# AnthonyMadia/lodestar

Hardware: AMD Instinct MI355X
Metric: verified signature sets/sec (node) at 8192-set batches (higher is better)
Workload: dtype u32 (28-bit-limb Montgomery Fp, v_mad_u64_u32)

## Files before the change

### lodestar_amd/csrc/bgv_api.cpp

```cpp
#include <hip/hip_runtime.h>
#include <stdio.h>
#include <stdlib.h>
#include <string.h>
#include <sys/mman.h>
#include <sys/random.h>

#include <algorithm>
#include <atomic>
#include <chrono>
#include <condition_variable>
#include <unordered_map>
#include <deque>
#include <map>
#include <memory>
#include <mutex>
#include <shared_mutex>
#include <unordered_set>
#include <thread>
#include <vector>

#include "../../include/blsgpu.h"
#include "bgv_launch.h"
#include "bgv_retry_plan.h"
#include "bls_field.h"

#define BGV_MAX_BATCH_SLOTS 131072
#define BGV_DISPATCHERS 2

static size_t max_batch_slots() {
  static const size_t v = env_size("BGV_MAX_BATCH_SLOTS", BGV_MAX_BATCH_SLOTS, BGV_WAVE);
  return v;
}
#define BGV_COALESCE_US 500
static size_t coalesce_us() {
  static const size_t v = env_size("BGV_COALESCE_US", BGV_COALESCE_US, 0);
  return v;
}
#define BGV_IDLE_COALESCE_US 50
static size_t idle_coalesce_us() {
  static const size_t v = env_size("BGV_IDLE_COALESCE_US", BGV_IDLE_COALESCE_US, 0);
  return v;
}
#define BGV_SPLIT_MIN_SETS 4096
static size_t split_min_env() {
  static const size_t v = env_size("BGV_SPLIT_MIN", BGV_SPLIT_MIN_SETS, 0);
  return v == 1 ? 2 : v;
}
static int dispatchers_per_device() {
  static const int v = (int)env_size("BGV_DISPATCHERS", BGV_DISPATCHERS, 1);
  return v;
}
static int execs_per_device() {
  static const int v = (int)env_size("BGV_EXECS", 2 * BGV_DISPATCHERS, 1);
  return std::max(v, dispatchers_per_device());
}

static size_t retry_hold_max() {
  static const size_t v = env_size("BGV_RETRY_HOLD", 1, 1);
  return v;
}
static int retry_threads_per_device() {
  static const int v = (int)env_size("BGV_RETRY_THREADS", 1, 1);
  return v;
}

extern "C" int bgv_device_count(void) {
  int n = 0;
  if (hipGetDeviceCount(&n) != hipSuccess) return 0;
  return n;
}

namespace {

template <class T>
struct Pinned {
  T* p = nullptr;
  size_t cap = 0;
  hipError_t reserve(size_t n) {
    if (n <= cap) return hipSuccess;
    release();
    n = std::max(n, 2 * cap);
    hipError_t e = hipHostMalloc(reinterpret_cast<void**>(&p), std::max<size_t>(n, 1) * sizeof(T), 0);
    if (e != hipSuccess) {
      p = nullptr;
      return e;
    }
    cap = n;
    return hipSuccess;
  }
  void release() {
    if (p) (void)hipHostFree(p);
    p = nullptr;
    cap = 0;
  }
};

struct Exec {
  hipStream_t main = nullptr;
  hipStream_t close = nullptr;
  hipEvent_t ev0 = nullptr, ev1 = nullptr, ev_prep = nullptr, ev_sets = nullptr;
  hipEvent_t kev[2 * BGV_NKERNELS] = {};
  void* slot_mem = nullptr;
  uint32_t slot_cap = 0;
  void* group_mem = nullptr;
  uint32_t group_cap = 0;
  bgv_dslot* d_slots = nullptr;
  bgv_dgroup* d_groups = nullptr;
  uint32_t* d_idx = nullptr;
  size_t idx_cap = 0;
  uint8_t* d_pkb = nullptr;
  size_t pkb_cap = 0;
  Pinned<bgv_dslot> h_slots;
  Pinned<bgv_dgroup> h_groups;
  Pinned<uint32_t> h_idx;
  Pinned<uint8_t> h_pkb;
  Pinned<int32_t> h_ss, h_ps, h_verdict;
  fp12_t* d_gu1 = nullptr;
  size_t gu1_cap = 0;
  void* d_pscratch = nullptr;
  size_t pscratch_cap = 0;
  uint8_t* d_pout = nullptr;
  size_t pout_cap = 0;
  uint32_t* d_lines = nullptr;
  uint32_t lines_cap = 0;
};

struct FinalScratch {
  uint8_t* din = nullptr;
  void* vals = nullptr;
  void* one = nullptr;
  bgv_dgroup* dg = nullptr;
  int32_t* dst = nullptr;
  int32_t* dv = nullptr;
  size_t cap = 0;
};

static const uint32_t kComHandles = 2 * BGV_MAX_COMMITTEES;
static const size_t kComPoolInit = size_t(1) << 20;
struct ComPool {
  std::mutex mu;
  std::vector<uint32_t> free_handles;
  std::map<uint32_t, uint32_t> free_ranges;
  size_t cap = 0;
  bool alloc(uint32_t n, uint32_t* handle, uint32_t* off) {
    if (free_handles.empty()) return false;
    for (auto it = free_ranges.begin(); it != free_ranges.end(); ++it)
      if (it->second >= n) {
        *off = it->first;
        const uint32_t rest = it->second - n;
        free_ranges.erase(it);
        if (rest) free_ranges.emplace(*off + n, rest);
        *handle = free_handles.back();
        free_handles.pop_back();
        return true;
      }
    return false;
  }
  void add_range(uint32_t off, uint32_t n) {
    auto nx = free_ranges.lower_bound(off);
    if (nx != free_ranges.begin()) {
      auto pv = std::prev(nx);
      if (pv->first + pv->second == off) {
        off = pv->first;
        n += pv->second;
        free_ranges.erase(pv);
      }
    }
    if (nx != free_ranges.end() && off + n == nx->first) {
      n += nx->second;
      free_ranges.erase(nx);
    }
    free_ranges.emplace(off, n);
  }
};
struct CommitteeRec {
  uint32_t handle = 0, off = 0;
  std::vector<uint32_t> idx;
  bool bad = false;
  std::shared_ptr<ComPool> pool;
  ~CommitteeRec() {
    if (!pool) return;
    std::lock_guard<std::mutex> lk(pool->mu);
    pool->free_handles.push_back(handle);
    pool->add_range(off, (uint32_t)idx.size());
  }
};

struct Call;
struct BatchState {
  std::chrono::steady_clock::time_point tb;
  double t_merge = 0, t_tok = 0, t_sets = 0, t_pass1 = 0, t_post = 0;
  uint32_t nslots = 0, ngroups = 0;
  std::vector<uint32_t> call_gb;
  bool want_gu = false;
  bool uniform = false;
  bool prof = false;
};
struct RetryJob {
  std::vector<Call*> calls;
  Exec* x = nullptr;
  std::shared_ptr<BatchState> st;
};
struct DevSched {
  std::mutex mu;
  std::condition_variable cv;
  std::deque<Exec*> free;
  std::deque<RetryJob> rq;
  bool stop = false;
  std::vector<std::thread> retry_threads;
  std::vector<hipStream_t> retries;
  std::vector<hipStream_t> dstreams;
};

struct Device {
  int id = 0;
  std::unique_ptr<DevSched> sched = std::make_unique<DevSched>();
  FinalScratch final_scratch;
  hipStream_t stream = nullptr;
  bgv_cache_entry* cache = nullptr;
  size_t cache_cap = 0;
  bgv_dcommittee* com_dir = nullptr;
  uint32_t* com_pool = nullptr;
  uint32_t* com_list = nullptr;
  std::vector<Exec*> execs;
  std::unique_ptr<std::mutex> compute_mu = std::make_unique<std::mutex>();
};

struct Call : CallPlan {
  const bgv_set* sets = nullptr;
  const bgv_pkbits* pkbits = nullptr;
  std::vector<SetCommittee> setcom;
  std::vector<std::shared_ptr<CommitteeRec>> com_refs;
  int32_t* out = nullptr;
  bgv_stats* stats_out = nullptr;
  bgv_done_fn done = nullptr;
  void* user = nullptr;
  bool owned = false;
  std::chrono::steady_clock::time_point t0;
  int dev = -1;
  bgv_job pjob{};
  int32_t pcode = 0;
  int rc = BGV_OK;
  std::mutex mu;
  std::condition_variable cv;
  bool finished = false;
};

}

struct bgv_ctx {
  std::vector<Device> devs;
  std::atomic<size_t> n_pubkeys{0};
  std::mutex put_mu;
  std::unordered_set<uint32_t> bad_pk;
  std::atomic<bool> closed{false};
  std::mutex rng_mu;
  uint64_t rng_seed = 0, rng_state = 0;
  std::shared_mutex cache_mu;
  std::mutex util_mu;
  std::shared_mutex com_mu;
  std::unordered_map<uint32_t, std::shared_ptr<CommitteeRec>> committees;
  std::vector<std::weak_ptr<CommitteeRec>> retired;
  std::shared_ptr<ComPool> com_pool = std::make_shared<ComPool>();
  std::mutex prof_mu;
  bool profile = false;
  bool fault_inject = false;
  std::atomic<uint32_t> max_slots{BGV_MAX_BATCH_SLOTS};
  std::atomic<uint32_t> coalesce{BGV_COALESCE_US};
  std::atomic<uint32_t> idle_coalesce{BGV_IDLE_COALESCE_US};
  std::atomic<int> running{0};
  std::atomic<uint32_t> split_min{BGV_SPLIT_MIN_SETS};
  int split_inflight = 0;
  bool split_closing = false;
  std::mutex split_mu;
  std::condition_variable split_cv;
  double kernel_ms[BGV_NKERNELS] = {};
  uint64_t kernel_launches = 0;
  std::vector<std::thread> dispatchers;
  std::mutex qmu;
  std::condition_variable qcv;
  std::deque<Call*> queue;
  bool stop = false;
};

#define HIPCHK(x)                               \
  do {                                          \
    hipError_t e_ = (x);                        \
    if (e_ != hipSuccess) return -BGV_E_DEVICE; \
  } while (0)

static uint64_t splitmix64(uint64_t* s) {
  uint64_t z = (*s += 0x9E3779B97F4A7C15ull);
  z = (z ^ (z >> 30)) * 0xBF58476D1CE4E5B9ull;
  z = (z ^ (z >> 27)) * 0x94D049BB133111EBull;
  return z ^ (z >> 31);
}

static void fill_scalars(bgv_ctx* c, uint64_t* out, size_t n) {
  {
    std::lock_guard<std::mutex> lk(c->rng_mu);
    if (c->rng_seed) {
      for (size_t i = 0; i < n; ++i) {
        uint64_t v;
        do v = splitmix64(&c->rng_state);
        while (v == 0);
        out[i] = v;
      }
      return;
    }
  }
  par_ranges(n, [out](size_t lo, size_t hi) {
    size_t got = 0;
    uint8_t* p = reinterpret_cast<uint8_t*>(out + lo);
    while (got < (hi - lo) * 8) {
      const ssize_t r = getrandom(p + got, (hi - lo) * 8 - got, 0);
      if (r > 0) got += (size_t)r;
    }
    for (size_t i = lo; i < hi; ++i)
      if (out[i] == 0) out[i] = 1;
  });
}

template <class T>
static int grow(T** p, size_t* cap, size_t want) {
  if (want <= *cap) return BGV_OK;
  size_t n = std::max(want, *cap * 2);
  if (*p) (void)hipFree(*p);
  *p = nullptr;
  HIPCHK(hipMalloc(reinterpret_cast<void**>(p), n * sizeof(T)));
  *cap = n;
  return BGV_OK;
}

static int exec_reserve_slots(Exec& x, uint32_t slots) {
  if (slots <= x.slot_cap) return BGV_OK;
  uint32_t n = std::max<uint32_t>(slots, x.slot_cap * 2);
  if (x.slot_mem) (void)hipFree(x.slot_mem);
  if (x.d_slots) (void)hipFree(x.d_slots);
  x.slot_mem = nullptr;
  x.d_slots = nullptr;
  HIPCHK(hipMalloc(&x.slot_mem, bgv_slot_mem_bytes(n)));
  HIPCHK(hipMalloc(reinterpret_cast<void**>(&x.d_slots), sizeof(bgv_dslot) * n));
  x.slot_cap = n;
  return BGV_OK;
}

static int exec_reserve_groups(Exec& x, uint32_t groups) {
  if (groups <= x.group_cap) return BGV_OK;
  uint32_t n = std::max<uint32_t>(groups, x.group_cap * 2);
  if (x.group_mem) (void)hipFree(x.group_mem);
  if (x.d_groups) (void)hipFree(x.d_groups);
  x.group_mem = nullptr;
  x.d_groups = nullptr;
  HIPCHK(hipMalloc(&x.group_mem, bgv_group_bytes() * n));
  HIPCHK(hipMalloc(reinterpret_cast<void**>(&x.d_groups), sizeof(bgv_dgroup) * n));
  x.group_cap = n;
  return BGV_OK;
}

static uint32_t lines_keep_pairs(size_t slots) {
  return (uint32_t)((slots + slots / BGV_WAVE + 16383u) & ~(size_t)16383u);
}
static void exec_trim_lines(Exec& x, size_t max_slots) {
  if (x.lines_cap <= lines_keep_pairs(max_slots)) return;
  (void)hipFree(x.d_lines);
  x.d_lines = nullptr;
  x.lines_cap = 0;
}
static int exec_reserve_lines(Exec& x, bgv_dev_batch& b) {
  const uint32_t need = bgv_lines_pairs(b);
  if (need > x.lines_cap) {
    const uint32_t cap = (need + 16383u) & ~16383u;
    if (x.d_lines) (void)hipFree(x.d_lines);
    x.d_lines = nullptr;
    x.lines_cap = 0;
    HIPCHK(hipMalloc(reinterpret_cast<void**>(&x.d_lines), bgv_line_record_bytes() * cap));
    x.lines_cap = cap;
  }
  b.lines = x.d_lines;
  b.lines_cap = x.lines_cap;
  return BGV_OK;
}

static int exec_create(Exec* x) {
  HIPCHK(hipEventCreate(&x->ev0));
  HIPCHK(hipEventCreate(&x->ev1));
  HIPCHK(hipEventCreateWithFlags(&x->ev_sets, hipEventDisableTiming));
  HIPCHK(hipEventCreateWithFlags(&x->ev_prep, hipEventDisableTiming));
  for (auto& e : x->kev) HIPCHK(hipEventCreate(&e));
  return BGV_OK;
}

static void exec_destroy(Exec* x) {
  if (x->main) (void)hipStreamSynchronize(x->main);
  void* ptrs[] = {x->slot_mem, x->group_mem, x->d_slots,    x->d_groups, x->d_idx,
                  x->d_pkb,      x->d_pscratch, x->d_pout, x->d_lines};
  for (void* p : ptrs)
    if (p) (void)hipFree(p);
  x->h_slots.release();
  x->h_groups.release();
  x->h_idx.release();
  x->h_pkb.release();
  x->h_ss.release();
  x->h_ps.release();
  x->h_verdict.release();
  if (x->d_gu1) (void)hipFree(x->d_gu1);
  if (x->ev0) (void)hipEventDestroy(x->ev0);
  if (x->ev1) (void)hipEventDestroy(x->ev1);
  if (x->ev_sets) (void)hipEventDestroy(x->ev_sets);
  if (x->ev_prep) (void)hipEventDestroy(x->ev_prep);
  for (auto& e : x->kev)
    if (e) (void)hipEventDestroy(e);
  if (x->close) (void)hipStreamSynchronize(x->close);
  delete x;
}

static void prof_add(bgv_ctx* c, Exec& x, bool sets, bool groups) {
  std::lock_guard<std::mutex> lk(c->prof_mu);
  if (!c->profile) return;
  for (int k = 0; k < BGV_NKERNELS; ++k) {
    const bool is_set_kernel = k < BGV_NSETKERNELS;
    if ((is_set_kernel && !sets) || (!is_set_kernel && !groups)) continue;
    float km = 0;
    if (hipEventElapsedTime(&km, x.kev[2 * k], x.kev[2 * k + 1]) == hipSuccess) c->kernel_ms[k] += km;
  }
  if (sets) c->kernel_launches++;
}

static bgv_dev_batch make_batch(Device& d, Exec& x, uint32_t nslots, uint32_t ngroups) {
  bgv_dev_batch b;
  memset(&b, 0, sizeof(b));
  b.nslots = nslots;
  b.ngroups = ngroups;
  b.slots = x.d_slots;
  b.groups = x.d_groups;
  b.pk_idx = x.d_idx;
  b.cache_opaque = d.cache;
  b.pk_bytes = x.d_pkb;
  b.com_dir = d.com_dir;
  b.com_pool = d.com_pool;
  bgv_carve(&b, x.slot_mem, x.slot_cap, x.group_mem, x.group_cap);
  return b;
}

static void call_finish(Call* call) {
  for (size_t j = 0; j < call->njobs; ++j) call->out[j] = call->code[j] == 2 ? -BGV_E_DEVICE : call->code[j];
  call->st.wall_ms =
      std::chrono::duration<double, std::milli>(std::chrono::steady_clock::now() - call->t0).count();
  if (call->stats_out) *call->stats_out = call->st;
  if (call->done) call->done(call->user, call->rc);
  if (call->owned) {
    delete call;
    return;
  }
  {
    std::lock_guard<std::mutex> lk(call->mu);
    call->finished = true;
  }
  call->cv.notify_all();
}

static void call_fail(Call* call, int rc) {
  call->rc = rc;
  for (auto& x : call->code)
    if (x == 2) x = -BGV_E_DEVICE;
  call_finish(call);
}

static int host_job_code(bgv_ctx* c, const bgv_job& jb, const bgv_set* sets, int32_t* code,
                         const bgv_pkbits* pkbits = nullptr, Call* call = nullptr) {
  *code = 2;
  if (jb.n_sets == 0) {
    *code = -BGV_E_EMPTY_SET;
    return BGV_OK;
  }
  for (uint32_t k = 0; k < jb.n_sets && *code == 2; ++k) {
    const bgv_set& s = sets[jb.first_set + k];
    if (pkbits && pkbits[jb.first_set + k].committee != BGV_NO_COMMITTEE) {
      const bgv_pkbits& pb = pkbits[jb.first_set + k];
      if (!s.msg || (!s.sig && s.sig_len) || (!pb.bits && pb.n_bits)) return -BGV_E_ARG;
      const auto it = c->committees.find(pb.committee);
      const CommitteeRec* rec = it != c->committees.end() ? it->second.get() : nullptr;
      CommitteeInfo ci{};
      if (rec) ci = CommitteeInfo{rec->handle, (uint32_t)rec->idx.size(), rec->bad};
      SetCommittee sc;
      *code = committee_set_check(rec ? &ci : nullptr, pb, &sc);
      if (*code == 2 && call) {
        call->setcom[jb.first_set + k] = sc;
        if (call->com_refs.empty() || call->com_refs.back().get() != rec) call->com_refs.push_back(it->second);
      }
      continue;
    }
    if (s.n_pk == 0)
      *code = -BGV_E_EMPTY_AGGREGATE;
    else if (!s.msg || (!s.sig && s.sig_len) || (!s.pk_indices && !s.pk_bytes))
      return -BGV_E_ARG;
    else if (s.pk_indices)
      for (uint32_t q = 0; q < s.n_pk; ++q)
        if (s.pk_indices[q] >= c->n_pubkeys || (!c->bad_pk.empty() && c->bad_pk.count(s.pk_indices[q]))) {
          *code = -BGV_E_BAD_INDEX;
          break;
        }
  }
  return BGV_OK;
}

static void advise_huge(void* p, size_t bytes) {
  const uintptr_t a = ((uintptr_t)p + (2u << 20) - 1) & ~(uintptr_t)((2u << 20) - 1);
  const uintptr_t e = ((uintptr_t)p + bytes) & ~(uintptr_t)((2u << 20) - 1);
  if (e > a) (void)madvise(reinterpret_cast<void*>(a), e - a, MADV_HUGEPAGE);
}

static int call_submit(bgv_ctx* c, Call* call, const bgv_job* jobs, size_t njobs, const bgv_set* sets, size_t nsets,
                       int mode, int32_t* out, bgv_stats* stats, bgv_done_fn done, void* user, int dev = -1,
                       const bgv_pkbits* pkbits = nullptr) {
  call->t0 = std::chrono::steady_clock::now();
  call->dev = dev;
  if (c->closed) return -BGV_E_CLOSED;
  if ((njobs && (!jobs || !out)) || (nsets && !sets)) return -BGV_E_ARG;
  if (mode != BGV_MODE_WORKER && mode != BGV_MODE_PER_JOB) return -BGV_E_ARG;
  call->jobs = jobs;
  call->njobs = njobs;
  call->sets = sets;
  call->nsets = nsets;
  call->mode = mode;
  call->out = out;
  call->stats_out = stats;
  call->done = done;
  call->user = user;
  call->code.assign(njobs, 2);
  call->pkbits = pkbits;
  if (pkbits) call->setcom.assign(nsets, SetCommittee{});
  {
    std::shared_lock<std::shared_mutex> clk(c->cache_mu);
    std::shared_lock<std::shared_mutex> mlk(c->com_mu, std::defer_lock);
    if (pkbits) mlk.lock();
    for (size_t j = 0; j < njobs; ++j) {
      if ((size_t)jobs[j].first_set + jobs[j].n_sets > nsets) return -BGV_E_ARG;
      if (host_job_code(c, jobs[j], sets, &call->code[j], pkbits, call) != BGV_OK) return -BGV_E_ARG;
    }
  }
  const auto is_com = [pkbits](size_t i) { return pkbits && pkbits[i].committee != BGV_NO_COMMITTEE; };
  Layout& L = call->L;
  {
    size_t npk = 0;
    for (size_t i = 0; i < nsets; ++i)
      if (is_com(i))
        npk += 1 + pkb_nwords(call->setcom[i].n);
      else if (sets[i].pk_indices)
        npk += sets[i].n_pk;
    const size_t cap = nsets + nsets / 8 + BGV_WAVE;
    L.slots.reserve(cap);
    L.slot_set.reserve(cap);
    L.idx.reserve(npk);
    if (nsets >= (1u << 17)) {
      advise_huge(L.slots.data(), sizeof(bgv_dslot) * cap);
      advise_huge(L.slot_set.data(), 4 * cap);
      advise_huge(L.idx.data(), 4 * npk);
    }
  }
  layout_call(L, call->todo, jobs, njobs, sets, mode, call->code, pkbits ? call->setcom.data() : nullptr);
  call->set_sig.assign(nsets, 0);
  call->set_pk.assign(nsets, 0);
  if (L.slots.empty()) {
    call_finish(call);
    return BGV_OK;
  }
  {
    std::lock_guard<std::mutex> lk(c->qmu);
    if (c->stop) return -BGV_E_CLOSED;
    c->queue.push_back(call);
  }
  if (dev < 0)
    c->qcv.notify_one();
  else
    c->qcv.notify_all();
  return BGV_OK;
}

static double ms_since(std::chrono::steady_clock::time_point t) {
  return std::chrono::duration<double, std::milli>(std::chrono::steady_clock::now() - t).count();
}

static bool needs_retry(const std::vector<Call*>& calls) {
  for (const Call* call : calls)
    if (!call->units.empty()) return true;
  return false;
}

static int run_pass1(bgv_ctx* c, Device& d, Exec& x, std::vector<Call*>& calls, BatchState& bs) {
  const auto tb = std::chrono::steady_clock::now();
  bs.tb = tb;
  double t_merge = 0, t_tok = 0, t_sets = 0, t_pass1 = 0, t_post = 0;
  uint32_t nslots = 0, ngroups = 0;
  size_t nidx = 0, npkb = 0, nuniq = 0, ncom_team = 0, ncom_wave = 0;
  bool any_uniform = false;
  for (Call* call : calls) {
    call->slot_base = nslots;
    nslots += (uint32_t)call->L.slots.size();
    ngroups += (uint32_t)call->L.groups.size();
    nidx += call->L.idx.size();
    npkb += call->L.pkb.size();
    nuniq += call->L.uniq.size();
    ncom_team += call->L.com_team.size();
    ncom_wave += call->L.com_wave.size();
    for (char u : call->L.group_uniform) any_uniform = any_uniform || u;
  }
  const size_t ncom = ncom_team + ncom_wave, nlist = nuniq + ncom;
  const bool bulk = nslots + ngroups > bgv_fold_pairs_max();
  const bool uniform = uniform_enabled() && any_uniform && bulk && !bgv_single_pass_miller();
  HIPCHK(hipSetDevice(d.id));
  int rc;
  if ((rc = exec_reserve_slots(x, nslots)) || (rc = exec_reserve_groups(x, ngroups)) ||
      (rc = grow(&x.d_idx, &x.idx_cap, std::max<size_t>(nidx + nlist, 1))) ||
      (rc = grow(&x.d_pkb, &x.pkb_cap, std::max<size_t>(npkb, 1))))
    return rc;
  HIPCHK(x.h_slots.reserve(nslots));
  HIPCHK(x.h_groups.reserve(std::max<size_t>(ngroups, 1)));
  HIPCHK(x.h_idx.reserve(nidx + nlist));
  HIPCHK(x.h_pkb.reserve(npkb));
  HIPCHK(x.h_ss.reserve(nslots));
  HIPCHK(x.h_ps.reserve(nslots));
  HIPCHK(x.h_verdict.reserve(std::max<size_t>(ngroups, 1)));
  bgv_dslot* slots = x.h_slots.p;
  bgv_dgroup* groups = x.h_groups.p;
  uint32_t max_npk = 0;
  {
    size_t ns = 0, ng = 0, ni = 0, npb = 0;
    for (Call* call : calls) {
      const uint32_t ib = (uint32_t)ni, pb = (uint32_t)(npb / 96), gb = (uint32_t)ng;
      if (ns == 0 && ib == 0 && pb == 0 && gb == 0) {
        const bgv_dslot* src = call->L.slots.data();
        std::atomic<uint32_t> mx{0};
        par_ranges(call->L.slots.size(), [&](size_t lo, size_t hi) {
          memcpy(slots + lo, src + lo, sizeof(bgv_dslot) * (hi - lo));
          uint32_t m = 0;
          for (size_t i = lo; i < hi; ++i)
            if (!(src[i].flags & BGV_SLOT_PK_COMMITTEE)) m = std::max(m, src[i].n_pk);
          uint32_t cur = mx.load();
          while (m > cur && !mx.compare_exchange_weak(cur, m)) {
          }
        });
        max_npk = std::max(max_npk, mx.load());
        ns = call->L.slots.size();
      } else {
        for (const bgv_dslot& s0 : call->L.slots) {
          const bgv_dslot s = rebase_slot(s0, call->slot_base, ib, pb, gb);
          if (!(s.flags & BGV_SLOT_PK_COMMITTEE)) max_npk = std::max(max_npk, s.n_pk);
          slots[ns++] = s;
        }
      }
      for (size_t gi = 0; gi < call->L.groups.size(); ++gi) {
        const bgv_dgroup& g = call->L.groups[gi];
        groups[ng++] = bgv_dgroup{g.first_slot + call->slot_base, g.n_slots, g.mask, 0,
                                  uniform && call->L.group_uniform[gi] ? BGV_GROUP_UNIFORM : 0u};
      }
      if (!call->L.idx.empty()) memcpy(x.h_idx.p + ni, call->L.idx.data(), 4 * call->L.idx.size());
      ni += call->L.idx.size();
      if (!call->L.pkb.empty()) memcpy(x.h_pkb.p + npb, call->L.pkb.data(), call->L.pkb.size());
      npb += call->L.pkb.size();
    }
    uint32_t* u = x.h_idx.p + nidx;
    for (Call* call : calls)
      for (uint32_t v : call->L.uniq) *u++ = v + call->slot_base;
    for (Call* call : calls)
      for (uint32_t v : call->L.com_team) *u++ = v + call->slot_base;
    for (Call* call : calls)
      for (uint32_t v : call->L.com_wave) *u++ = v + call->slot_base;
  }
  std::vector<uint64_t> sc(nslots);
  fill_scalars(c, sc.data(), nslots);
  par_ranges(nslots, [&](size_t lo, size_t hi) {
    for (size_t i = lo; i < hi; ++i) slots[i].scalar = sc[i];
  });

  bool prof;
  {
    std::lock_guard<std::mutex> lk(c->prof_mu);
    prof = c->profile;
  }
  t_merge = ms_since(tb);
  if (c->fault_inject) HIPCHK(hipErrorLaunchFailure);
  HIPCHK(hipMemcpyAsync(x.d_slots, slots, sizeof(bgv_dslot) * nslots, hipMemcpyHostToDevice, x.main));
  HIPCHK(hipMemcpyAsync(x.d_groups, groups, sizeof(bgv_dgroup) * ngroups, hipMemcpyHostToDevice, x.main));
  if (nidx + nlist) HIPCHK(hipMemcpyAsync(x.d_idx, x.h_idx.p, 4 * (nidx + nlist), hipMemcpyHostToDevice, x.main));
  if (npkb) HIPCHK(hipMemcpyAsync(x.d_pkb, x.h_pkb.p, npkb, hipMemcpyHostToDevice, x.main));
  bgv_dev_batch b = make_batch(d, x, nslots, ngroups);
  b.max_npk = max_npk;
  b.uniform = uniform;
  bs.uniform = uniform;
  b.uniq = x.d_idx + nidx;
  b.nuniq = (uint32_t)nuniq;
  b.com = x.d_idx + nidx + nuniq;
  b.ncom_team = (uint32_t)ncom_team;
  b.ncom_wave = (uint32_t)ncom_wave;
  if (int lrc = exec_reserve_lines(x, b)) return lrc;
  bgv_streams S{x.main, prof ? x.kev : nullptr};
  int32_t *ss = x.h_ss.p, *ps = x.h_ps.p, *verdict = x.h_verdict.p;
  {
    const auto tt = std::chrono::steady_clock::now();
    std::unique_lock<std::mutex> tok(*d.compute_mu);
    t_tok = ms_since(tt);
    HIPCHK(hipEventRecord(x.ev0, x.main));
    HIPCHK(bgv_launch_prep(b, S));
    HIPCHK(hipEventRecord(x.ev_prep, x.main));
    HIPCHK(bgv_launch_miller(b, S));
    HIPCHK(hipEventRecord(x.ev_sets, x.main));
    HIPCHK(hipEventSynchronize(x.ev_prep));
    t_sets = ms_since(tt) - t_tok;
  }
  const auto tg = std::chrono::steady_clock::now();
  HIPCHK(bgv_launch_groups(b, S, false));
  HIPCHK(hipEventRecord(x.ev1, x.main));
  HIPCHK(hipMemcpyAsync(ss, b.sig_status, 4ull * nslots, hipMemcpyDeviceToHost, x.main));
  HIPCHK(hipMemcpyAsync(ps, b.pk_status, 4ull * nslots, hipMemcpyDeviceToHost, x.main));
  HIPCHK(hipMemcpyAsync(verdict, b.verdict, 4ull * ngroups, hipMemcpyDeviceToHost, x.main));
  HIPCHK(hipStreamSynchronize(x.main));
  float ms = 0;
  HIPCHK(hipEventElapsedTime(&ms, x.ev0, x.ev1));
  exec_trim_lines(x, c->max_slots.load());
  if (prof) prof_add(c, x, true, true);
  t_pass1 = ms_since(tg);
  const auto tp = std::chrono::steady_clock::now();
  std::vector<uint32_t>& call_gb = bs.call_gb;
  bool& want_gu = bs.want_gu;
  {
    uint32_t gb = 0;
    for (Call* call : calls) {
      call->st.device_ms += ms;
      call->after_pass1(ss + call->slot_base, ps + call->slot_base, verdict + gb);
      call_gb.push_back(gb);
      gb += (uint32_t)call->L.groups.size();
      want_gu = want_gu || call->any_pattern_eligible();
    }
  }
  if (want_gu) {
    if ((rc = grow(&x.d_gu1, &x.gu1_cap, ngroups))) return rc;
    HIPCHK(hipMemcpyAsync(x.d_gu1, b.gu, sizeof(fp12_t) * ngroups, hipMemcpyDeviceToDevice, x.main));
  }
  {
    uint32_t gb = 0, np = 0, maxg = 0;
    for (Call* call : calls) {
      if (call->partial_out) {
        ++np;
        maxg = std::max<uint32_t>(maxg, (uint32_t)call->L.groups.size());
      }
    }
    if (np) {
      if ((rc = grow(reinterpret_cast<uint8_t**>(&x.d_pscratch), &x.pscratch_cap,
                     bgv_fp12_bytes() * (maxg / 32 + 4))) ||
          (rc = grow(&x.d_pout, &x.pout_cap, 576)))
        return rc;
      for (Call* call : calls) {
        const uint32_t ng = (uint32_t)call->L.groups.size();
        if (call->partial_out) {
          HIPCHK(bgv_launch_partial(b, gb, ng, x.d_pscratch, x.d_pout, x.main));
          HIPCHK(hipMemcpyAsync(call->partial_out, x.d_pout, 576, hipMemcpyDeviceToHost, x.main));
          HIPCHK(hipStreamSynchronize(x.main));
        }
        gb += ng;
      }
    }
  }
  HIPCHK(hipStreamSynchronize(x.main));
  t_post = ms_since(tp);
  bs.t_merge = t_merge;
  bs.t_tok = t_tok;
  bs.t_sets = t_sets;
  bs.t_pass1 = t_pass1;
  bs.t_post = t_post;
  bs.nslots = nslots;
  bs.ngroups = ngroups;
  bs.prof = prof;
  if (trace_on() && !needs_retry(calls))
    fprintf(stderr,
            "[bgv] dev %d calls %zu slots %u groups %u | submit..dispatch %.1f | merge %.1f tokwait %.1f sets %.1f "
            "groups %.1f post %.1f total %.1f ms\n",
            d.id, calls.size(), nslots, ngroups,
            std::chrono::duration<double, std::milli>(tb - calls.front()->t0).count(), t_merge, t_tok, t_sets,
            t_pass1, t_post, ms_since(tb));
  return BGV_OK;
}

struct RetryRun {
  RetryJob job;
  int rounds = 0;
  uint32_t nrg = 0;
  double t_build = 0;
  std::chrono::steady_clock::time_point tr;
};

static int retry_launch(Device& d, RetryRun& r, bool* more) {
  Exec& x = *r.job.x;
  std::vector<Call*>& calls = r.job.calls;
  BatchState& bs = *r.job.st;
  const auto th = std::chrono::steady_clock::now();
  std::vector<bgv_dgroup> rg;
  for (size_t k = 0; k < calls.size(); ++k)
    calls[k]->build_parts(rg, bs.want_gu ? (int64_t)bs.call_gb[k] : -1, bs.uniform);
  *more = !rg.empty();
  r.nrg = 0;
  if (rg.empty()) return BGV_OK;
  ++r.rounds;
  const uint32_t nrg = (uint32_t)rg.size();
  std::vector<uint32_t> upk;
  if (bs.uniform)
    for (uint32_t t = 0; t < nrg; ++t)
      if (rg[t].flags & BGV_GROUP_UNIFORM) upk.push_back(t);
  const uint32_t per = (uint32_t)(sizeof(bgv_dgroup) / sizeof(uint32_t));
  const uint32_t nlist = ((uint32_t)upk.size() + per - 1) / per;
  int rc;
  if ((rc = exec_reserve_groups(x, nrg + nlist))) return rc;
  HIPCHK(x.h_groups.reserve(nrg + nlist));
  HIPCHK(x.h_verdict.reserve(nrg));
  memcpy(x.h_groups.p, rg.data(), sizeof(bgv_dgroup) * nrg);
  if (!upk.empty()) memcpy(x.h_groups.p + nrg, upk.data(), 4 * upk.size());
  HIPCHK(hipMemcpyAsync(x.d_groups, x.h_groups.p, sizeof(bgv_dgroup) * (nrg + nlist), hipMemcpyHostToDevice,
                        x.close));
  bgv_dev_batch b = make_batch(d, x, bs.nslots, nrg);
  b.uniform = !upk.empty();
  b.upk = reinterpret_cast<const uint32_t*>(b.groups + nrg);
  b.npk = (uint32_t)upk.size();
  for (const bgv_dgroup& t : rg) b.weighted = b.weighted || (t.flags & BGV_GROUP_WEIGHTED);
  bool pattern = false;
  for (Call* call : calls) pattern = pattern || !call->punits.empty();
  if (pattern) b.gu1 = x.d_gu1;
  r.t_build = ms_since(th);
  bgv_streams SC{x.close, bs.prof ? x.kev : nullptr};
  HIPCHK(hipEventRecord(x.ev0, x.close));
  HIPCHK(bgv_launch_groups(b, SC, true));
  HIPCHK(hipEventRecord(x.ev1, x.close));
  HIPCHK(hipMemcpyAsync(x.h_verdict.p, b.verdict, 4ull * nrg, hipMemcpyDeviceToHost, x.close));
  r.nrg = nrg;
  return BGV_OK;
}

static int retry_complete(bgv_ctx* c, RetryRun& r, double t_wait) {
  Exec& x = *r.job.x;
  float ms = 0;
  HIPCHK(hipEventElapsedTime(&ms, x.ev0, x.ev1));
  if (r.job.st->prof) prof_add(c, x, false, true);
  if (trace_on()) {
    size_t npt = 0;
    for (Call* call : r.job.calls)
      for (const PatternUnit& pu : call->punits) npt += pu.tests.size();
    fprintf(stderr,
            "[bgv]  round %d: %u groups (%zu tests with a reference), host %.2f, launch..verdicts %.2f, device %.2f ms, "
            "since round start %.1f ms\n",
            r.rounds, r.nrg, npt, r.t_build, t_wait, ms, ms_since(r.tr));
  }
  for (Call* call : r.job.calls) {
    call->st.device_ms += ms;
    call->after_round(x.h_verdict.p);
  }
  r.nrg = 0;
  return BGV_OK;
}

static void retry_trace_done(const Device& d, const RetryRun& r) {
  if (!trace_on()) return;
  const BatchState& bs = *r.job.st;
  fprintf(stderr,
          "[bgv] dev %d calls %zu slots %u groups %u | merge %.1f tokwait %.1f sets %.1f groups %.1f post %.1f "
          "retry(%d) %.1f total %.1f ms\n",
          d.id, r.job.calls.size(), bs.nslots, bs.ngroups, bs.t_merge, bs.t_tok, bs.t_sets, bs.t_pass1, bs.t_post,
          r.rounds, ms_since(r.tr), ms_since(bs.tb));
}

static Exec* exec_acquire(Device& d) {
  DevSched& s = *d.sched;
  std::unique_lock<std::mutex> lk(s.mu);
  s.cv.wait(lk, [&s] { return !s.free.empty(); });
  Exec* x = s.free.back();
  s.free.pop_back();
  return x;
}

static void exec_release(Device& d, Exec* x) {
  DevSched& s = *d.sched;
  {
    std::lock_guard<std::mutex> lk(s.mu);
    s.free.push_back(x);
  }
  s.cv.notify_all();
}

static void finish_calls(std::vector<Call*>& calls, int rc) {
  for (Call* call : calls) {
    if (rc != BGV_OK)
      call_fail(call, rc);
    else
      call_finish(call);
  }
}

static void retry_loop(bgv_ctx* c, Device* d, int k) {
  DevSched& s = *d->sched;
  (void)hipSetDevice(d->id);
  hipStream_t st = s.retries[k];
  std::vector<RetryRun> held;
  auto leave = [&](size_t i, int rc) {
    finish_calls(held[i].job.calls, rc);
    exec_release(*d, held[i].job.x);
    c->running.fetch_sub(1);
    held.erase(held.begin() + (std::ptrdiff_t)i);
  };
  for (;;) {
    {
      std::unique_lock<std::mutex> lk(s.mu);
      if (held.empty()) s.cv.wait(lk, [&s] { return s.stop || !s.rq.empty(); });
      if (held.empty() && s.rq.empty()) return;
      while (!s.rq.empty() && held.size() < retry_hold_max()) {
        RetryRun r;
        r.job = std::move(s.rq.front());
        s.rq.pop_front();
        r.job.x->close = st;
        r.tr = std::chrono::steady_clock::now();
        c->running.fetch_add(1);
        held.push_back(std::move(r));
      }
    }
    (void)hipSetDevice(d->id);
    for (size_t i = 0; i < held.size();) {
      bool more = false;
      const int rc = retry_launch(*d, held[i], &more);
      if (rc != BGV_OK) {
        (void)hipStreamSynchronize(st);
        leave(i, rc);
      } else if (!more) {
        retry_trace_done(*d, held[i]);
        leave(i, BGV_OK);
      } else {
        ++i;
      }
    }
    if (held.empty()) continue;
    const auto tl = std::chrono::steady_clock::now();
    const hipError_t e = hipStreamSynchronize(st);
    const double t_wait = ms_since(tl);
    for (size_t i = 0; i < held.size();) {
      const int rc = e == hipSuccess ? retry_complete(c, held[i], t_wait) : -BGV_E_DEVICE;
      if (rc != BGV_OK)
        leave(i, rc);
      else
        ++i;
    }
  }
}

static void dispatcher_loop(bgv_ctx* c, Device* d, hipStream_t stream) {
  (void)hipSetDevice(d->id);
  const int di = (int)(d - c->devs.data());
  auto mine = [di](const Call* q) { return q->dev < 0 || q->dev == di; };
  auto any_mine = [c, &mine] {
    for (Call* q : c->queue)
      if (mine(q)) return true;
    return false;
  };
  for (;;) {
    std::vector<Call*> calls;
    {
      std::unique_lock<std::mutex> lk(c->qmu);
      c->qcv.wait(lk, [c, &any_mine] { return c->stop || any_mine(); });
      if (!any_mine()) return;
      auto queued_slots = [c, &mine] {
        size_t n = 0;
        for (Call* q : c->queue)
          if (mine(q)) n += q->L.slots.size();
        return n;
      };
      const size_t cap = c->max_slots.load();
      const size_t win = c->running.load() > 0 ? c->coalesce.load()
                                               : std::min<size_t>(c->coalesce.load(), c->idle_coalesce.load());
      const auto until = std::chrono::steady_clock::now() + std::chrono::microseconds(win);
      while (!c->stop && queued_slots() < cap &&
             c->qcv.wait_until(lk, until) != std::cv_status::timeout) {
      }
      if (!any_mine()) continue;
      size_t slots = 0;
      for (auto it = c->queue.begin(); it != c->queue.end();) {
        Call* call = *it;
        if (!mine(call)) {
          ++it;
          continue;
        }
        const size_t n = call->L.slots.size();
        if (!calls.empty() && slots + n > cap) break;
        calls.push_back(call);
        slots += n;
        it = c->queue.erase(it);
      }
      if (!c->queue.empty()) c->qcv.notify_all();
    }
    Exec* x = exec_acquire(*d);
    x->main = stream;
    auto bs = std::make_shared<BatchState>();
    int rc;
    {
      std::shared_lock<std::shared_mutex> clk(c->cache_mu);
      c->running.fetch_add(1);
      rc = run_pass1(c, *d, *x, calls, *bs);
      c->running.fetch_sub(1);
    }
    if (rc == BGV_OK && needs_retry(calls)) {
      DevSched& s = *d->sched;
      {
        std::lock_guard<std::mutex> lk(s.mu);
        s.rq.push_back(RetryJob{std::move(calls), x, bs});
      }
      s.cv.notify_all();
      continue;
    }
    finish_calls(calls, rc);
    exec_release(*d, x);
  }
}

extern "C" {

static void ctx_free_devices(bgv_ctx* c) {
  for (Device& d : c->devs) {
    if (!d.stream) continue;
    (void)hipSetDevice(d.id);
    for (Exec* x : d.execs) exec_destroy(x);
    d.execs.clear();
    d.sched->free.clear();
    for (hipStream_t st : d.sched->dstreams) (void)hipStreamDestroy(st);
    d.sched->dstreams.clear();
    for (hipStream_t st : d.sched->retries) (void)hipStreamDestroy(st);
    d.sched->retries.clear();
    if (d.stream) (void)hipStreamSynchronize(d.stream);
    if (d.cache) (void)hipFree(d.cache);
    d.cache = nullptr;
    {
      void* cbufs[] = {d.com_dir, d.com_pool, d.com_list};
      for (void* q : cbufs)
        if (q) (void)hipFree(q);
      d.com_dir = nullptr;
      d.com_pool = nullptr;
      d.com_list = nullptr;
    }
    {
      FinalScratch& fs = d.final_scratch;
      void* bufs[] = {fs.din, fs.vals, fs.one, fs.dg, fs.dst, fs.dv};
      for (void* q : bufs)
        if (q) (void)hipFree(q);
      fs = FinalScratch{};
    }
    if (d.stream) (void)hipStreamDestroy(d.stream);
    d.stream = nullptr;
  }
}

int bgv_init(const int* devices, int ndev, bgv_ctx** out) {
  if (!out) return -BGV_E_ARG;
  *out = nullptr;
  int avail = bgv_device_count();
  if (avail <= 0) return -BGV_E_DEVICE;
  bgv_ctx* c = new bgv_ctx();
  {
    const char* fi = getenv("BGV_FAULT_INJECT");
    c->fault_inject = fi && atoi(fi) > 0;
  }
  c->max_slots = (uint32_t)max_batch_slots();
  c->coalesce = (uint32_t)coalesce_us();
  c->idle_coalesce = (uint32_t)idle_coalesce_us();
  c->split_min = (uint32_t)split_min_env();
  const int n = (devices && ndev > 0) ? ndev : 1;
  c->devs.resize(n);
  for (int i = 0; i < n; ++i) {
    Device& d = c->devs[i];
    d.id = (devices && ndev > 0) ? devices[i] : 0;
    bool ok = d.id >= 0 && d.id < avail && hipSetDevice(d.id) == hipSuccess &&
              hipStreamCreateWithFlags(&d.stream, hipStreamNonBlocking) == hipSuccess;
    int least = 0, greatest = 0;
    ok = ok && hipDeviceGetStreamPriorityRange(&least, &greatest) == hipSuccess;
    for (int k = 0; ok && k < retry_threads_per_device(); ++k) {
      hipStream_t st = nullptr;
      ok = hipStreamCreateWithPriority(&st, hipStreamNonBlocking, greatest) == hipSuccess;
      if (ok) d.sched->retries.push_back(st);
    }
    for (int k = 0; ok && k < dispatchers_per_device(); ++k) {
      hipStream_t st = nullptr;
      ok = hipStreamCreateWithFlags(&st, hipStreamNonBlocking) == hipSuccess;
      if (ok) d.sched->dstreams.push_back(st);
    }
    ok = ok && hipMalloc(reinterpret_cast<void**>(&d.com_dir), sizeof(bgv_dcommittee) * kComHandles) == hipSuccess &&
         hipMalloc(reinterpret_cast<void**>(&d.com_pool), 4 * kComPoolInit) == hipSuccess &&
         hipMalloc(reinterpret_cast<void**>(&d.com_list), 4 * (size_t)kComHandles) == hipSuccess;
    for (int k = 0; ok && k < execs_per_device(); ++k) {
      Exec* x = new Exec();
      d.execs.push_back(x);
      ok = exec_create(x) == BGV_OK;
      if (ok) d.sched->free.push_back(x);
    }
    if (!ok) {
      ctx_free_devices(c);
      delete c;
      (void)hipGetLastError();
      return d.id < 0 || d.id >= avail ? -BGV_E_ARG : -BGV_E_DEVICE;
    }
  }
  c->com_pool->cap = kComPoolInit;
  c->com_pool->free_ranges.emplace(0u, (uint32_t)kComPoolInit);
  for (uint32_t h = kComHandles; h-- > 0;) c->com_pool->free_handles.push_back(h);
  for (Device& d : c->devs) {
    for (hipStream_t st : d.sched->dstreams) c->dispatchers.emplace_back(dispatcher_loop, c, &d, st);
    for (int k = 0; k < (int)d.sched->retries.size(); ++k) d.sched->retry_threads.emplace_back(retry_loop, c, &d, k);
  }
  *out = c;
  return BGV_OK;
}

int bgv_close(bgv_ctx* c) {
  if (!c) return -BGV_E_ARG;
  {
    std::unique_lock<std::mutex> lk(c->split_mu);
    c->split_closing = true;
    c->split_cv.wait(lk, [c] { return c->split_inflight == 0; });
  }
  {
    std::lock_guard<std::mutex> lk(c->qmu);
    c->stop = true;
  }
  c->qcv.notify_all();
  for (auto& w : c->dispatchers)
    if (w.joinable()) w.join();
  c->dispatchers.clear();
  for (Device& d : c->devs) {
    {
      std::lock_guard<std::mutex> lk(d.sched->mu);
      d.sched->stop = true;
    }
    d.sched->cv.notify_all();
    for (auto& t : d.sched->retry_threads)
      if (t.joinable()) t.join();
    d.sched->retry_threads.clear();
  }
  std::unique_lock<std::shared_mutex> lk(c->cache_mu);
  if (c->closed.exchange(true)) return BGV_OK;
  ctx_free_devices(c);
  return BGV_OK;
}

int bgv_destroy(bgv_ctx* c) {
  if (!c) return -BGV_E_ARG;
  bgv_close(c);
  delete c;
  return BGV_OK;
}

int bgv_set_batching(bgv_ctx* c, uint32_t max_batch_slots, uint32_t coalesce_us, uint32_t idle_coalesce_us) {
  if (!c) return -BGV_E_ARG;
  if (max_batch_slots) c->max_slots = std::max<uint32_t>(max_batch_slots, BGV_WAVE);
  if (coalesce_us != UINT32_MAX) c->coalesce = coalesce_us;
  if (idle_coalesce_us != UINT32_MAX) c->idle_coalesce = idle_coalesce_us;
  return BGV_OK;
}

int bgv_set_rng_seed(bgv_ctx* c, uint64_t seed) {
  if (!c) return -BGV_E_ARG;
  std::lock_guard<std::mutex> lk(c->rng_mu);
  c->rng_seed = seed;
  c->rng_state = seed;
  return BGV_OK;
}

size_t bgv_pubkeys_count(const bgv_ctx* c) { return c ? c->n_pubkeys.load() : 0; }

static int cache_reserve(bgv_ctx* c, size_t need) {
  const size_t esz = bgv_cache_entry_bytes();
  for (Device& d : c->devs) {
    HIPCHK(hipSetDevice(d.id));
    if (need <= d.cache_cap) continue;
    size_t cap = std::max(need, d.cache_cap * 2);
    void* p = nullptr;
    HIPCHK(hipMalloc(&p, esz * cap));
    if (d.cache) {
      HIPCHK(hipMemcpyAsync(p, d.cache, esz * c->n_pubkeys, hipMemcpyDeviceToDevice, d.stream));
      HIPCHK(hipStreamSynchronize(d.stream));
      HIPCHK(hipFree(d.cache));
    }
    d.cache = static_cast<bgv_cache_entry*>(p);
    d.cache_cap = cap;
  }
  return BGV_OK;
}

static int committee_totals(bgv_ctx* c, const std::vector<uint32_t>& handles) {
  if (handles.empty()) return BGV_OK;
  for (Device& d : c->devs) {
    HIPCHK(hipSetDevice(d.id));
    HIPCHK(hipMemcpyAsync(d.com_list, handles.data(), 4 * handles.size(), hipMemcpyHostToDevice, d.stream));
    HIPCHK(bgv_launch_committee_totals(d.com_dir, d.com_list, (uint32_t)handles.size(), d.com_pool, d.cache, d.stream));
    HIPCHK(hipStreamSynchronize(d.stream));
  }
  return BGV_OK;
}

static int committees_refresh(bgv_ctx* c, uint32_t first, size_t n) {
  std::vector<uint32_t> handles;
  {
    std::unique_lock<std::shared_mutex> lk(c->com_mu);
    std::vector<std::shared_ptr<CommitteeRec>> recs;
    for (auto& kv : c->committees) recs.push_back(kv.second);
    for (auto& w : c->retired)
      if (auto sp = w.lock()) recs.push_back(std::move(sp));
    for (auto& sp : recs) {
      CommitteeRec& r = *sp;
      bool touched = false, bad = false;
      for (uint32_t i : r.idx) {
        touched = touched || (i >= first && (size_t)i < (size_t)first + n);
        bad = bad || (!c->bad_pk.empty() && c->bad_pk.count(i));
      }
      if (!touched) continue;
      r.bad = bad;
      handles.push_back(r.handle);
    }
  }
  return committee_totals(c, handles);
}

static int com_pool_grow(bgv_ctx* c, size_t need) {
  ComPool& P = *c->com_pool;
  const size_t old = P.cap, cap = std::max(2 * old, old + need);
  if (cap > (size_t)UINT32_MAX) return -BGV_E_NOMEM;
  for (Device& d : c->devs) {
    HIPCHK(hipSetDevice(d.id));
    uint32_t* p = nullptr;
    HIPCHK(hipMalloc(reinterpret_cast<void**>(&p), 4 * cap));
    HIPCHK(hipMemcpyAsync(p, d.com_pool, 4 * old, hipMemcpyDeviceToDevice, d.stream));
    HIPCHK(hipStreamSynchronize(d.stream));
    HIPCHK(hipFree(d.com_pool));
    d.com_pool = p;
  }
  std::lock_guard<std::mutex> lk(P.mu);
  P.add_range((uint32_t)old, (uint32_t)(cap - old));
  P.cap = cap;
  return BGV_OK;
}

int bgv_committee_put(bgv_ctx* c, uint32_t id, const uint32_t* indices, size_t n) {
  if (!c || id >= BGV_MAX_COMMITTEES || !indices || n < 1 || n > 65536) return -BGV_E_ARG;
  std::lock_guard<std::mutex> plk(c->put_mu);
  auto rec = std::make_shared<CommitteeRec>();
  auto checks = [&]() -> int {
    if (c->closed) return -BGV_E_CLOSED;
    {
      std::shared_lock<std::shared_mutex> lk(c->com_mu);
      if (c->committees.count(id)) return -BGV_E_ARG;
    }
    for (size_t i = 0; i < n; ++i)
      if (indices[i] >= c->n_pubkeys || (!c->bad_pk.empty() && c->bad_pk.count(indices[i]))) return -BGV_E_BAD_INDEX;
    return BGV_OK;
  };
  auto take = [&]() -> bool {
    std::lock_guard<std::mutex> lk(c->com_pool->mu);
    if (!c->com_pool->alloc((uint32_t)n, &rec->handle, &rec->off)) return false;
    rec->pool = c->com_pool;
    return true;
  };
  auto upload = [&]() -> int {
    rec->idx.assign(indices, indices + n);
    const bgv_dcommittee head{rec->off, (uint32_t)n, {}};
    std::lock_guard<std::mutex> ulk(c->util_mu);
    for (Device& d : c->devs) {
      HIPCHK(hipSetDevice(d.id));
      HIPCHK(hipMemcpyAsync(d.com_pool + rec->off, indices, 4 * n, hipMemcpyHostToDevice, d.stream));
      HIPCHK(hipMemcpyAsync(d.com_dir + rec->handle, &head, sizeof(head), hipMemcpyHostToDevice, d.stream));
      HIPCHK(hipStreamSynchronize(d.stream));
    }
    const int rc = committee_totals(c, {rec->handle});
    if (rc) return rc;
    std::unique_lock<std::shared_mutex> lk(c->com_mu);
    c->committees.emplace(id, rec);
    return BGV_OK;
  };
  {
    std::shared_lock<std::shared_mutex> clk(c->cache_mu);
    if (int rc = checks()) return rc;
    if (take()) return upload();
    std::lock_guard<std::mutex> lk(c->com_pool->mu);
    if (c->com_pool->free_handles.empty()) return -BGV_E_NOMEM;
  }
  std::unique_lock<std::shared_mutex> clk(c->cache_mu);
  if (int rc = checks()) return rc;
  {
    std::lock_guard<std::mutex> ulk(c->util_mu);
    if (int rc = com_pool_grow(c, n)) return rc;
  }
  if (!take()) return -BGV_E_NOMEM;
  return upload();
}

int bgv_committee_drop(bgv_ctx* c, uint32_t id) {
  if (!c) return -BGV_E_ARG;
  std::lock_guard<std::mutex> plk(c->put_mu);
  if (c->closed) return -BGV_E_CLOSED;
  std::shared_ptr<CommitteeRec> rec;
  std::unique_lock<std::shared_mutex> lk(c->com_mu);
  auto it = c->committees.find(id);
  if (it == c->committees.end()) return -BGV_E_BAD_INDEX;
  rec = std::move(it->second);
  c->committees.erase(it);
  c->retired.erase(std::remove_if(c->retired.begin(), c->retired.end(),
                                  [](const std::weak_ptr<CommitteeRec>& w) { return w.expired(); }),
                   c->retired.end());
  c->retired.push_back(rec);
  return BGV_OK;
}

int bgv_pubkeys_put(bgv_ctx* c, uint32_t first, const uint8_t* keys, size_t n, int fmt) {
  if (!c || (n && !keys) || (fmt != BGV_PK_COMPRESSED && fmt != BGV_PK_UNCOMPRESSED)) return -BGV_E_ARG;
  std::lock_guard<std::mutex> plk(c->put_mu);
  const size_t esz = bgv_cache_entry_bytes();
  std::vector<void*> staged(c->devs.size(), nullptr);
  std::vector<int32_t> status(n, 0);
  auto free_staged = [&] {
    for (size_t di = 0; di < staged.size(); ++di)
      if (staged[di]) {
        (void)hipSetDevice(c->devs[di].id);
        (void)hipFree(staged[di]);
      }
  };
  {
    std::shared_lock<std::shared_mutex> clk(c->cache_mu);
    if (c->closed) return -BGV_E_CLOSED;
    if ((size_t)first > c->n_pubkeys) return -BGV_E_ARG;
    if (n == 0) return BGV_OK;
    std::lock_guard<std::mutex> ulk(c->util_mu);
    for (size_t di = 0; di < c->devs.size(); ++di) {
      Device& d = c->devs[di];
      if (hipSetDevice(d.id) != hipSuccess || hipMalloc(&staged[di], esz * n) != hipSuccess ||
          hipMemsetAsync(staged[di], 0, esz * n, d.stream) != hipSuccess) {
        free_staged();
        return -BGV_E_DEVICE;
      }
      const size_t chunk = 1 << 20;
      uint8_t* dk = nullptr;
      int32_t* dst = nullptr;
      int rc = BGV_OK;
      if (hipMalloc(reinterpret_cast<void**>(&dk), (size_t)fmt * std::min(n, chunk) + 1) != hipSuccess ||
          hipMalloc(reinterpret_cast<void**>(&dst), 4 * std::min(n, chunk) + 4) != hipSuccess)
        rc = -BGV_E_DEVICE;
      for (size_t off = 0; rc == BGV_OK && off < n; off += chunk) {
        const size_t m = std::min(chunk, n - off);
        bgv_cache_entry* out =
            reinterpret_cast<bgv_cache_entry*>(static_cast<uint8_t*>(staged[di]) + esz * off);
        if (hipMemcpyAsync(dk, keys + (size_t)fmt * off, (size_t)fmt * m, hipMemcpyHostToDevice, d.stream) !=
                hipSuccess ||
            bgv_launch_cache_put(dk, (uint32_t)m, fmt, out, dst, d.stream) != hipSuccess ||
            (di == 0 && hipMemcpyAsync(status.data() + off, dst, 4 * m, hipMemcpyDeviceToHost, d.stream) !=
                            hipSuccess) ||
            hipStreamSynchronize(d.stream) != hipSuccess)
          rc = -BGV_E_DEVICE;
      }
      if (dk) (void)hipFree(dk);
      if (dst) (void)hipFree(dst);
      if (rc) {
        free_staged();
        return rc;
      }
    }
  }
  int first_err = BGV_OK;
  std::vector<uint32_t> bad;
  for (size_t i = 0; i < n; ++i)
    if (status[i]) {
      if (first_err == BGV_OK) first_err = status[i];
      bad.push_back(first + (uint32_t)i);
    }
  const size_t need = (size_t)first + n;
  auto copy_in = [&]() -> int {
    for (size_t di = 0; di < c->devs.size(); ++di) {
      Device& d = c->devs[di];
      HIPCHK(hipSetDevice(d.id));
      HIPCHK(hipMemcpyAsync(reinterpret_cast<uint8_t*>(d.cache) + esz * first, staged[di], esz * n,
                            hipMemcpyDeviceToDevice, d.stream));
      HIPCHK(hipStreamSynchronize(d.stream));
    }
    return BGV_OK;
  };
  int rc = BGV_OK;
  bool done = false;
  {
    std::shared_lock<std::shared_mutex> clk(c->cache_mu);
    if (c->closed) {
      rc = -BGV_E_CLOSED;
      done = true;
    } else if (first == c->n_pubkeys && bad.empty()) {
      bool fits = true;
      for (const Device& d : c->devs) fits = fits && need <= d.cache_cap;
      if (fits) {
        std::lock_guard<std::mutex> ulk(c->util_mu);
        rc = copy_in();
        if (rc == BGV_OK) c->n_pubkeys.store(need);
        done = true;
      }
    }
  }
  if (!done) {
    std::unique_lock<std::shared_mutex> clk(c->cache_mu);
    if (c->closed) {
      rc = -BGV_E_CLOSED;
    } else {
      std::lock_guard<std::mutex> ulk(c->util_mu);
      rc = cache_reserve(c, need);
      const uint32_t old_n = (uint32_t)c->n_pubkeys.load();
      for (size_t di = 0; rc == BGV_OK && di < c->devs.size(); ++di) {
        Device& d = c->devs[di];
        if (hipSetDevice(d.id) != hipSuccess) rc = -BGV_E_DEVICE;
        for (uint32_t i : bad)
          if (rc == BGV_OK && i < old_n &&
              hipMemcpyAsync(static_cast<uint8_t*>(staged[di]) + esz * (i - first),
                             reinterpret_cast<const uint8_t*>(d.cache) + esz * i, esz, hipMemcpyDeviceToDevice,
                             d.stream) != hipSuccess)
            rc = -BGV_E_DEVICE;
      }
      if (rc == BGV_OK) rc = copy_in();
      if (rc == BGV_OK) {
        for (uint32_t i = first; i < need; ++i) c->bad_pk.erase(i);
        for (uint32_t i : bad) c->bad_pk.insert(i);
        c->n_pubkeys.store(std::max(c->n_pubkeys.load(), need));
        if (first < old_n) rc = committees_refresh(c, first, n);
      }
    }
  }
  free_staged();
  if (rc) return rc;
  return first_err ? -first_err : BGV_OK;
}

static void fp12_one_bytes(uint8_t out[576]) {
  memset(out, 0, 576);
  out[47] = 1;
}

static int partial_submit(bgv_ctx* c, Call* call, const bgv_set* sets, size_t nsets, uint8_t* out576,
                          int32_t* out_codes, int dev, const bgv_pkbits* pkbits = nullptr) {
  out_codes[0] = out_codes[1] = 0;
  fp12_one_bytes(out576);
  call->partial_out = out576;
  call->partial_codes = out_codes;
  call->pjob = bgv_job{0, (uint32_t)nsets, 0};
  return call_submit(c, call, &call->pjob, 1, sets, nsets, BGV_MODE_PER_JOB, &call->pcode, nullptr, nullptr, nullptr,
                     dev, pkbits);
}

static int call_wait(Call* call) {
  std::unique_lock<std::mutex> lk(call->mu);
  call->cv.wait(lk, [call] { return call->finished; });
  return call->rc;
}

static int partial_finish(Call* call, int rc, int32_t* out_codes) {
  if (rc == BGV_OK) rc = call_wait(call);
  if (rc == BGV_OK && call->pcode < 0 && call->pcode != -BGV_E_DEVICE) out_codes[0] = call->pcode;
  return rc;
}

static size_t split_min_sets(const bgv_ctx* c) {
  return c->split_min.load();
}

static void stats_add(bgv_stats* a, const bgv_stats& b) {
  a->batch_retries += b.batch_retries;
  a->batch_sigs_success += b.batch_sigs_success;
  a->device_groups += b.device_groups;
  a->sets_verified += b.sets_verified;
  a->device_ms = std::max(a->device_ms, b.device_ms);
}

static bool split_wanted(const bgv_ctx* c, size_t nsets) {
  return c->devs.size() > 1 && split_min_sets(c) > 0 && nsets >= split_min_sets(c);
}

static bool split_enter(bgv_ctx* c) {
  std::lock_guard<std::mutex> lk(c->split_mu);
  if (c->split_closing) return false;
  ++c->split_inflight;
  return true;
}

static void split_leave(bgv_ctx* c) {
  std::lock_guard<std::mutex> lk(c->split_mu);
  --c->split_inflight;
  c->split_cv.notify_all();
}

static int verify_split(bgv_ctx* c, const bgv_job* jobs, size_t njobs, const bgv_set* sets, size_t nsets,
                        const bgv_pkbits* pkbits, int mode, int32_t* out, bgv_stats* stats) {
  const auto t0 = std::chrono::steady_clock::now();
  const size_t K = c->devs.size(), big = split_min_sets(c);
  struct Shard {
    Call call;
    size_t job;
    uint8_t part[576];
    int32_t codes[2] = {0, 0};
    int rc = BGV_OK;
  };
  struct Child {
    Call call;
    std::vector<bgv_job> jobs;
    std::vector<int32_t> out;
    bgv_stats st{};
    size_t j0 = 0;
    int rc = BGV_OK;
  };
  std::vector<std::unique_ptr<Shard>> shards;
  std::vector<std::unique_ptr<Child>> kids;
  std::vector<size_t> small;
  size_t small_sets = 0;
  std::vector<int32_t> pre(njobs, 2);
  {
    std::shared_lock<std::shared_mutex> clk(c->cache_mu);
    std::shared_lock<std::shared_mutex> mlk(c->com_mu, std::defer_lock);
    if (pkbits) mlk.lock();
    for (size_t j = 0; j < njobs; ++j) {
      if ((size_t)jobs[j].first_set + jobs[j].n_sets > nsets) return -BGV_E_ARG;
      if (jobs[j].n_sets >= big && host_job_code(c, jobs[j], sets, &pre[j], pkbits) != BGV_OK) return -BGV_E_ARG;
    }
  }
  for (size_t j = 0; j < njobs; ++j) {
    if (jobs[j].n_sets >= big) continue;
    small.push_back(j);
    small_sets += jobs[j].n_sets;
  }
  int rc = BGV_OK;
  {
    size_t i = 0, acc = 0;
    for (size_t d = 0; d < K && i < small.size(); ++d) {
      const size_t target = (small_sets * (d + 1) + K - 1) / K;
      auto kid = std::make_unique<Child>();
      kid->j0 = i;
      while (i < small.size() && (acc < target || kid->jobs.empty())) {
        kid->jobs.push_back(jobs[small[i]]);
        acc += jobs[small[i]].n_sets;
        ++i;
      }
      if (d == K - 1)
        while (i < small.size()) {
          kid->jobs.push_back(jobs[small[i]]);
          ++i;
        }
      kid->out.assign(kid->jobs.size(), 0);
      kid->rc = call_submit(c, &kid->call, kid->jobs.data(), kid->jobs.size(), sets, nsets, mode, kid->out.data(),
                            &kid->st, nullptr, nullptr, (int)d, pkbits);
      if (kid->rc != BGV_OK && rc == BGV_OK) rc = kid->rc;
      kids.push_back(std::move(kid));
    }
  }
  for (size_t j = 0; j < njobs; ++j) {
    const uint32_t n = jobs[j].n_sets;
    if (n < big || pre[j] != 2) continue;
    for (size_t d = 0; d < K; ++d) {
      const size_t lo = n * d / K, hi = n * (d + 1) / K;
      if (hi <= lo) continue;
      auto sh = std::make_unique<Shard>();
      sh->job = j;
      sh->rc = partial_submit(c, &sh->call, sets + jobs[j].first_set + lo, hi - lo, sh->part, sh->codes, (int)d,
                              pkbits ? pkbits + jobs[j].first_set + lo : nullptr);
      if (sh->rc != BGV_OK && rc == BGV_OK) rc = sh->rc;
      shards.push_back(std::move(sh));
    }
  }
  for (auto& k : kids)
    if (k->rc == BGV_OK) {
      k->rc = call_wait(&k->call);
      if (k->rc != BGV_OK && rc == BGV_OK) rc = k->rc;
    }
  for (auto& sh : shards)
    if (sh->rc == BGV_OK) {
      sh->rc = partial_finish(&sh->call, BGV_OK, sh->codes);
      if (sh->rc != BGV_OK && rc == BGV_OK) rc = sh->rc;
    }
  if (rc != BGV_OK) return rc;
  bgv_stats st{};
  for (auto& k : kids) {
    for (size_t q = 0; q < k->jobs.size(); ++q) out[small[k->j0 + q]] = k->out[q];
    stats_add(&st, k->st);
  }
  for (size_t j = 0; j < njobs; ++j) {
    if (jobs[j].n_sets < big) continue;
    if (pre[j] != 2) {
      out[j] = pre[j];
      continue;
    }
    int32_t code = 0;
    bool decided = false;
    std::vector<uint8_t> parts;
    for (auto& sh : shards)
      if (sh->job == j && sh->codes[0] && !decided) {
        code = sh->codes[0];
        decided = true;
      }
    for (auto& sh : shards)
      if (sh->job == j && sh->codes[1] && !decided) {
        code = sh->codes[1] == 1 ? -BGV_BLST_PK_IS_INFINITY : sh->codes[1];
        decided = true;
      }
    if (!decided) {
      for (auto& sh : shards)
        if (sh->job == j) parts.insert(parts.end(), sh->part, sh->part + 576);
      int32_t v = 0;
      const int frc = bgv_final_verify(c, parts.data(), parts.size() / 576, &v);
      if (frc != BGV_OK) return frc;
      code = v ? 1 : 0;
    }
    out[j] = code;
    st.sets_verified += jobs[j].n_sets;
    st.device_groups += 1;
  }
  st.wall_ms = std::chrono::duration<double, std::milli>(std::chrono::steady_clock::now() - t0).count();
  if (stats) *stats = st;
  return BGV_OK;
}

int bgv_set_split(bgv_ctx* c, uint32_t min_sets) {
  if (!c) return -BGV_E_ARG;
  c->split_min = min_sets == 1 ? 2 : min_sets;
  return BGV_OK;
}

int bgv_verify(bgv_ctx* c, const bgv_job* jobs, size_t njobs, const bgv_set* sets, size_t nsets, int mode,
               int32_t* out, bgv_stats* stats) {
  return bgv_verify_bits(c, jobs, njobs, sets, nsets, nullptr, mode, out, stats);
}

int bgv_verify_async(bgv_ctx* c, const bgv_job* jobs, size_t njobs, const bgv_set* sets, size_t nsets, int mode,
                     int32_t* out, bgv_stats* stats, bgv_done_fn done, void* user) {
  return bgv_verify_bits_async(c, jobs, njobs, sets, nsets, nullptr, mode, out, stats, done, user);
}

int bgv_verify_bits(bgv_ctx* c, const bgv_job* jobs, size_t njobs, const bgv_set* sets, size_t nsets,
                    const bgv_pkbits* pkbits, int mode, int32_t* out, bgv_stats* stats) {
  if (!c) return -BGV_E_ARG;
  if (split_wanted(c, nsets)) {
    if (c->closed) return -BGV_E_CLOSED;
    if ((njobs && (!jobs || !out)) || (nsets && !sets)) return -BGV_E_ARG;
    if (mode != BGV_MODE_WORKER && mode != BGV_MODE_PER_JOB) return -BGV_E_ARG;
    if (!split_enter(c)) return -BGV_E_CLOSED;
    const int rc = verify_split(c, jobs, njobs, sets, nsets, pkbits, mode, out, stats);
    split_leave(c);
    return rc;
  }
  Call* call = new Call();
  int rc = call_submit(c, call, jobs, njobs, sets, nsets, mode, out, stats, nullptr, nullptr, -1, pkbits);
  if (rc == BGV_OK) {
    std::unique_lock<std::mutex> lk(call->mu);
    call->cv.wait(lk, [call] { return call->finished; });
    rc = call->rc;
  }
  delete call;
  return rc;
}

int bgv_verify_bits_async(bgv_ctx* c, const bgv_job* jobs, size_t njobs, const bgv_set* sets, size_t nsets,
                          const bgv_pkbits* pkbits, int mode, int32_t* out, bgv_stats* stats, bgv_done_fn done,
                          void* user) {
  if (!c) return -BGV_E_ARG;
  if (split_wanted(c, nsets)) {
    if (c->closed) return -BGV_E_CLOSED;
    if ((njobs && (!jobs || !out)) || (nsets && !sets)) return -BGV_E_ARG;
    if (mode != BGV_MODE_WORKER && mode != BGV_MODE_PER_JOB) return -BGV_E_ARG;
    if (!split_enter(c)) return -BGV_E_CLOSED;
    std::thread([=] {
      const int rc = verify_split(c, jobs, njobs, sets, nsets, pkbits, mode, out, stats);
      if (done) done(user, rc);
      split_leave(c);
    }).detach();
    return BGV_OK;
  }
  Call* call = new Call();
  call->owned = true;
  int rc = call_submit(c, call, jobs, njobs, sets, nsets, mode, out, stats, done, user, -1, pkbits);
  if (rc != BGV_OK) delete call;
  return rc;
}

int bgv_verify_partial(bgv_ctx* c, const bgv_set* sets, size_t nsets, uint8_t out576[576], int32_t out_codes[2]) {
  if (!c || !out576 || !out_codes || (nsets && !sets)) return -BGV_E_ARG;
  out_codes[0] = out_codes[1] = 0;
  fp12_one_bytes(out576);
  if (nsets == 0) return c->closed ? -BGV_E_CLOSED : BGV_OK;
  Call* call = new Call();
  const int rc = partial_finish(call, partial_submit(c, call, sets, nsets, out576, out_codes, -1), out_codes);
  delete call;
  return rc;
}

int bgv_final_verify(bgv_ctx* c, const uint8_t* partials, size_t n, int32_t* out_verdict) {
  if (!c || !out_verdict || (n && !partials) || n > (1u << 20)) return -BGV_E_ARG;
  std::shared_lock<std::shared_mutex> clk(c->cache_mu);
  if (c->closed) return -BGV_E_CLOSED;
  std::lock_guard<std::mutex> lk(c->util_mu);
  Device& d = c->devs[0];
  HIPCHK(hipSetDevice(d.id));
  const size_t m = std::max<size_t>(n, 1);
  std::vector<uint8_t> in(576 * m);
  if (n) memcpy(in.data(), partials, 576 * n);
  else fp12_one_bytes(in.data());
  FinalScratch& fs = d.final_scratch;
  if (m > fs.cap) {
    void* bufs[] = {fs.din, fs.vals, fs.one, fs.dg, fs.dst, fs.dv};
    for (void* q : bufs)
      if (q) (void)hipFree(q);
    fs = FinalScratch{};
    const size_t cap = std::max<size_t>(m, 8);
    HIPCHK(hipMalloc(reinterpret_cast<void**>(&fs.din), 576 * cap));
    HIPCHK(hipMalloc(&fs.vals, bgv_fp12_bytes() * cap));
    HIPCHK(hipMalloc(&fs.one, bgv_fp12_bytes()));
    HIPCHK(hipMalloc(reinterpret_cast<void**>(&fs.dg), sizeof(bgv_dgroup)));
    HIPCHK(hipMalloc(reinterpret_cast<void**>(&fs.dst), 4 * cap));
    HIPCHK(hipMalloc(reinterpret_cast<void**>(&fs.dv), 4));
    fs.cap = cap;
  }
  const bgv_dgroup g{0, (uint32_t)m, BGV_ALL_SLOTS};
  HIPCHK(hipMemcpyAsync(fs.din, in.data(), 576 * m, hipMemcpyHostToDevice, d.stream));
  HIPCHK(hipMemcpyAsync(fs.dg, &g, sizeof(g), hipMemcpyHostToDevice, d.stream));
  HIPCHK(bgv_launch_final_verify(fs.din, (uint32_t)m, fs.vals, fs.one, fs.dg, fs.dst, fs.dv, d.stream));
  std::vector<int32_t> st(m);
  int32_t v = 0;
  HIPCHK(hipMemcpyAsync(st.data(), fs.dst, 4 * m, hipMemcpyDeviceToHost, d.stream));
  HIPCHK(hipMemcpyAsync(&v, fs.dv, 4, hipMemcpyDeviceToHost, d.stream));
  HIPCHK(hipStreamSynchronize(d.stream));
  for (int32_t x : st)
    if (x) return -BGV_E_ARG;
  *out_verdict = v;
  return BGV_OK;
}

int bgv_debug_prepare(bgv_ctx* c, const bgv_set* sets, size_t nsets, int path, uint64_t seed, uint8_t* out_h192,
                      uint8_t* out_f576, int32_t* out_status) {
  if (!c || (nsets && (!sets || !out_h192 || !out_f576 || !out_status)) ||
      (path != BGV_PATH_BULK && path != BGV_PATH_LATENCY))
    return -BGV_E_ARG;
  if (nsets == 0) return BGV_OK;
  std::shared_lock<std::shared_mutex> clk(c->cache_mu);
  if (c->closed) return -BGV_E_CLOSED;
  std::vector<bgv_dslot> slots;
  std::vector<bgv_dgroup> groups;
  std::vector<uint32_t> idx;
  uint64_t state = seed;
  uint32_t max_npk = 0;
  for (size_t i = 0; i < nsets; ++i) {
    const bgv_set& st = sets[i];
    if (!st.pk_indices || st.n_pk == 0 || !st.msg || (st.sig_len && !st.sig)) return -BGV_E_ARG;
    for (uint32_t q = 0; q < st.n_pk; ++q)
      if (st.pk_indices[q] >= c->n_pubkeys || c->bad_pk.count(st.pk_indices[q])) return -BGV_E_BAD_INDEX;
    bgv_dslot s;
    memset(&s, 0, sizeof(s));
    s.flags = BGV_SLOT_PK_CACHED;
    s.n_pk = st.n_pk;
    s.sig_len = st.sig_len;
    s.pk_off = (uint32_t)idx.size();
    idx.insert(idx.end(), st.pk_indices, st.pk_indices + st.n_pk);
    memcpy(s.msg, st.msg, 32);
    if (st.sig_len == 96) memcpy(s.sig, st.sig, 96);
    s.group = (uint32_t)(i / BGV_WAVE);
    s.hsrc = (uint32_t)i;
    do s.scalar = splitmix64(&state);
    while (s.scalar == 0);
    max_npk = std::max(max_npk, st.n_pk);
    slots.push_back(s);
  }
  while (slots.size() % BGV_WAVE) {
    bgv_dslot s;
    memset(&s, 0, sizeof(s));
    s.flags = BGV_SLOT_PAD;
    s.hsrc = (uint32_t)slots.size();
    slots.push_back(s);
  }
  for (size_t g = 0; g * BGV_WAVE < nsets; ++g)
    groups.push_back(bgv_dgroup{(uint32_t)(g * BGV_WAVE), (uint32_t)std::min<size_t>(BGV_WAVE, nsets - g * BGV_WAVE),
                                BGV_ALL_SLOTS});
  const uint32_t nslots = (uint32_t)slots.size(), ngroups = (uint32_t)groups.size();
  std::lock_guard<std::mutex> lk(c->util_mu);
  Device& d = c->devs[0];
  HIPCHK(hipSetDevice(d.id));
  Exec* x = new Exec();
  uint8_t *dh = nullptr, *df = nullptr;
  int rc = exec_create(x);
  hipStream_t dstream = nullptr;
  if (!rc && hipStreamCreateWithFlags(&dstream, hipStreamNonBlocking) != hipSuccess) rc = -BGV_E_DEVICE;
  x->main = dstream;
  if (!rc) rc = exec_reserve_slots(*x, nslots);
  if (!rc) rc = exec_reserve_groups(*x, ngroups);
  if (!rc) rc = grow(&x->d_idx, &x->idx_cap, idx.size());
  if (!rc && (hipMalloc(reinterpret_cast<void**>(&dh), 192ull * nslots) != hipSuccess ||
              hipMalloc(reinterpret_cast<void**>(&df), 576ull * nslots) != hipSuccess))
    rc = -BGV_E_DEVICE;
  std::vector<int32_t> ss(nslots), ps(nslots);
  if (!rc) {
    bgv_dev_batch b = make_batch(d, *x, nslots, ngroups);
    b.max_npk = max_npk;
    b.path = path;
    rc = exec_reserve_lines(*x, b);
    bgv_streams S{x->main, nullptr};
    const bool ok = rc == BGV_OK &&
        hipMemcpyAsync(x->d_slots, slots.data(), sizeof(bgv_dslot) * nslots, hipMemcpyHostToDevice, x->main) ==
            hipSuccess &&
        hipMemcpyAsync(x->d_groups, groups.data(), sizeof(bgv_dgroup) * ngroups, hipMemcpyHostToDevice, x->main) ==
            hipSuccess &&
        hipMemcpyAsync(x->d_idx, idx.data(), 4 * idx.size(), hipMemcpyHostToDevice, x->main) == hipSuccess &&
        bgv_launch_sets(b, S) == hipSuccess && bgv_launch_debug_out(b, dh, df, x->main) == hipSuccess &&
        hipMemcpyAsync(out_h192, dh, 192 * nsets, hipMemcpyDeviceToHost, x->main) == hipSuccess &&
        hipMemcpyAsync(out_f576, df, 576 * nsets, hipMemcpyDeviceToHost, x->main) == hipSuccess &&
        hipMemcpyAsync(ss.data(), b.sig_status, 4ull * nslots, hipMemcpyDeviceToHost, x->main) == hipSuccess &&
        hipMemcpyAsync(ps.data(), b.pk_status, 4ull * nslots, hipMemcpyDeviceToHost, x->main) == hipSuccess &&
        hipStreamSynchronize(x->main) == hipSuccess;
    if (!ok) rc = -BGV_E_DEVICE;
  }
  if (dh) (void)hipFree(dh);
  if (df) (void)hipFree(df);
  exec_destroy(x);
  if (dstream) (void)hipStreamDestroy(dstream);
  if (rc) return rc;
  for (size_t i = 0; i < nsets; ++i) {
    out_status[2 * i] = ss[i];
    out_status[2 * i + 1] = ps[i];
  }
  return BGV_OK;
}

int bgv_debug_uniform(bgv_ctx* c, const bgv_set* sets, size_t nsets, uint64_t seed, const uint64_t* test_masks,
                      const uint32_t* test_weighted, size_t ntests, uint8_t* out_first576, uint8_t* out_pk576,
                      uint8_t* out_sig576) {
  if (!c || nsets < 2 || nsets > BGV_WAVE || !sets || !out_first576 || ntests > BGV_WAVE ||
      (ntests && (!test_masks || !test_weighted || !out_pk576 || !out_sig576)))
    return -BGV_E_ARG;
  std::shared_lock<std::shared_mutex> clk(c->cache_mu);
  if (c->closed) return -BGV_E_CLOSED;
  std::vector<bgv_dslot> slots;
  std::vector<uint32_t> idx;
  uint64_t state = seed;
  uint32_t max_npk = 0;
  for (size_t i = 0; i < nsets; ++i) {
    const bgv_set& st = sets[i];
    if (!st.pk_indices || st.n_pk == 0 || !st.msg || st.sig_len != 96 || !st.sig ||
        memcmp(st.msg, sets[0].msg, 32) != 0)
      return -BGV_E_ARG;
    for (uint32_t q = 0; q < st.n_pk; ++q)
      if (st.pk_indices[q] >= c->n_pubkeys || c->bad_pk.count(st.pk_indices[q])) return -BGV_E_BAD_INDEX;
    bgv_dslot s;
    memset(&s, 0, sizeof(s));
    s.flags = BGV_SLOT_PK_CACHED;
    s.n_pk = st.n_pk;
    s.sig_len = st.sig_len;
    s.pk_off = (uint32_t)idx.size();
    idx.insert(idx.end(), st.pk_indices, st.pk_indices + st.n_pk);
    memcpy(s.msg, st.msg, 32);
    memcpy(s.sig, st.sig, 96);
    s.group = 0;
    s.hsrc = 0;
    do s.scalar = splitmix64(&state);
    while (s.scalar == 0);
    max_npk = std::max(max_npk, st.n_pk);
    slots.push_back(s);
  }
  while (slots.size() % BGV_WAVE) {
    bgv_dslot s;
    memset(&s, 0, sizeof(s));
    s.flags = BGV_SLOT_PAD;
    s.hsrc = (uint32_t)slots.size();
    slots.push_back(s);
  }
  const uint32_t nslots = (uint32_t)slots.size(), nt = (uint32_t)ntests;
  const bgv_dgroup first{0u, (uint32_t)nsets, BGV_ALL_SLOTS, 0u, BGV_GROUP_UNIFORM};
  const uint32_t per = (uint32_t)(sizeof(bgv_dgroup) / sizeof(uint32_t));
  const uint32_t nlist = (nt + per - 1) / per;
  std::vector<bgv_dgroup> tg(nt + nlist);
  bool weighted = false;
  for (uint32_t t = 0; t < nt; ++t) {
    tg[t] = bgv_dgroup{0u, (uint32_t)nsets, test_masks[t], 0u,
                       BGV_GROUP_UNIFORM | (test_weighted[t] ? BGV_GROUP_WEIGHTED : 0u)};
    weighted = weighted || test_weighted[t];
    reinterpret_cast<uint32_t*>(tg.data() + nt)[t] = t;
  }
  std::lock_guard<std::mutex> lk(c->util_mu);
  Device& d = c->devs[0];
  HIPCHK(hipSetDevice(d.id));
  Exec* x = new Exec();
  uint8_t* dout = nullptr;
  int rc = exec_create(x);
  hipStream_t dstream = nullptr;
  if (!rc && hipStreamCreateWithFlags(&dstream, hipStreamNonBlocking) != hipSuccess) rc = -BGV_E_DEVICE;
  x->main = dstream;
  if (!rc) rc = exec_reserve_slots(*x, nslots);
  if (!rc) rc = exec_reserve_groups(*x, std::max<uint32_t>(1, nt + nlist));
  if (!rc) rc = grow(&x->d_idx, &x->idx_cap, idx.size());
  if (!rc && hipMalloc(reinterpret_cast<void**>(&dout), 576ull * (1 + 2 * nt)) != hipSuccess) rc = -BGV_E_DEVICE;
  if (!rc) {
    bgv_dev_batch b = make_batch(d, *x, nslots, 1);
    b.max_npk = max_npk;
    b.path = BGV_PATH_BULK;
    b.uniform = true;
    rc = exec_reserve_lines(*x, b);
    bgv_streams S{x->main, nullptr};
    bool ok = rc == BGV_OK &&
        hipMemcpyAsync(x->d_slots, slots.data(), sizeof(bgv_dslot) * nslots, hipMemcpyHostToDevice, x->main) ==
            hipSuccess &&
        hipMemcpyAsync(x->d_groups, &first, sizeof(bgv_dgroup), hipMemcpyHostToDevice, x->main) == hipSuccess &&
        hipMemcpyAsync(x->d_idx, idx.data(), 4 * idx.size(), hipMemcpyHostToDevice, x->main) == hipSuccess &&
        bgv_launch_sets(b, S) == hipSuccess &&
        bgv_launch_fp12_bytes(b.gpkp, 1, dout, x->main) == hipSuccess;
    if (ok && nt) {
      bgv_dev_batch t = make_batch(d, *x, nslots, nt);
      t.max_npk = max_npk;
      t.path = BGV_PATH_BULK;
      t.uniform = true;
      t.upk = reinterpret_cast<const uint32_t*>(t.groups + nt);
      t.npk = nt;
      t.weighted = weighted;
      ok = hipMemcpyAsync(x->d_groups, tg.data(), sizeof(bgv_dgroup) * tg.size(), hipMemcpyHostToDevice, x->main) ==
               hipSuccess &&
           bgv_launch_gpairs(t, x->main) == hipSuccess &&
           bgv_launch_fp12_bytes(t.gpkp, nt, dout + 576, x->main) == hipSuccess &&
           bgv_launch_fp12_bytes(t.gpair, nt, dout + 576ull * (1 + nt), x->main) == hipSuccess &&
           hipMemcpyAsync(out_pk576, dout + 576, 576ull * nt, hipMemcpyDeviceToHost, x->main) == hipSuccess &&
           hipMemcpyAsync(out_sig576, dout + 576ull * (1 + nt), 576ull * nt, hipMemcpyDeviceToHost, x->main) ==
               hipSuccess;
    }
    ok = ok && hipMemcpyAsync(out_first576, dout, 576, hipMemcpyDeviceToHost, x->main) == hipSuccess &&
         hipStreamSynchronize(x->main) == hipSuccess;
    if (!ok) rc = -BGV_E_DEVICE;
  }
  if (dout) (void)hipFree(dout);
  exec_destroy(x);
  if (dstream) (void)hipStreamDestroy(dstream);
  return rc;
}

int bgv_aggregate_pubkeys(bgv_ctx* c, const uint32_t* idx, size_t n, uint8_t out96[96]) {
  if (!c || !out96 || (n && !idx)) return -BGV_E_ARG;
  if (n == 0) return -BGV_E_EMPTY_AGGREGATE;
  std::shared_lock<std::shared_mutex> clk(c->cache_mu);
  if (c->closed) return -BGV_E_CLOSED;
  for (size_t i = 0; i < n; ++i)
    if (idx[i] >= c->n_pubkeys || c->bad_pk.count(idx[i])) return -BGV_E_BAD_INDEX;
  std::lock_guard<std::mutex> lk(c->util_mu);
  Device& d = c->devs[0];
  HIPCHK(hipSetDevice(d.id));
  bgv_dslot s;
  memset(&s, 0, sizeof(s));
  s.flags = BGV_SLOT_PK_CACHED;
  s.n_pk = (uint32_t)n;
  uint32_t* di = nullptr;
  uint8_t* dout = nullptr;
  bgv_dslot* ds = nullptr;
  void* dagg = nullptr;
  HIPCHK(hipMalloc(reinterpret_cast<void**>(&di), 4 * n));
  HIPCHK(hipMalloc(reinterpret_cast<void**>(&dout), 96));
  HIPCHK(hipMalloc(reinterpret_cast<void**>(&ds), sizeof(bgv_dslot)));
  HIPCHK(hipMalloc(&dagg, bgv_g1_point_bytes()));
  HIPCHK(hipMemcpyAsync(di, idx, 4 * n, hipMemcpyHostToDevice, d.stream));
  HIPCHK(hipMemcpyAsync(ds, &s, sizeof(s), hipMemcpyHostToDevice, d.stream));
  HIPCHK(bgv_launch_aggregate(ds, di, (uint32_t)n, d.cache, dagg, dout, d.stream));
  HIPCHK(hipMemcpyAsync(out96, dout, 96, hipMemcpyDeviceToHost, d.stream));
  HIPCHK(hipStreamSynchronize(d.stream));
  void* bufs[] = {di, dout, ds, dagg};
  for (void* p : bufs) (void)hipFree(p);
  return BGV_OK;
}

int bgv_aggregate_committee_bits(bgv_ctx* c, uint32_t id, const uint8_t* bits, uint32_t n_bits, uint8_t out96[96]) {
  if (!c || !out96 || (n_bits && !bits)) return -BGV_E_ARG;
  std::shared_lock<std::shared_mutex> clk(c->cache_mu);
  if (c->closed) return -BGV_E_CLOSED;
  const uint8_t zero[96] = {0};
  bgv_set st{};
  st.sig_len = 96;
  st.msg = zero;
  st.sig = zero;
  const bgv_pkbits pb{id, n_bits, bits};
  const bgv_job jb{0, 1, 0};
  Call call;
  call.setcom.assign(1, SetCommittee{});
  int32_t code = 2;
  {
    std::shared_lock<std::shared_mutex> mlk(c->com_mu);
    if (host_job_code(c, jb, &st, &code, &pb, &call) != BGV_OK) return -BGV_E_ARG;
  }
  if (code != 2) return code;
  Layout L;
  std::vector<size_t> todo;
  layout_call(L, todo, &jb, 1, &st, BGV_MODE_PER_JOB, {2}, call.setcom.data());
  const uint32_t list = 0;
  std::lock_guard<std::mutex> lk(c->util_mu);
  Device& d = c->devs[0];
  HIPCHK(hipSetDevice(d.id));
  uint32_t* di = nullptr;
  uint8_t* dout = nullptr;
  bgv_dslot* ds = nullptr;
  void* dagg = nullptr;
  const bool ok =
      hipMalloc(reinterpret_cast<void**>(&di), 4 * (L.idx.size() + 1)) == hipSuccess &&
      hipMalloc(reinterpret_cast<void**>(&dout), 96) == hipSuccess &&
      hipMalloc(reinterpret_cast<void**>(&ds), sizeof(bgv_dslot)) == hipSuccess &&
      hipMalloc(&dagg, bgv_g1_point_bytes()) == hipSuccess &&
      hipMemcpyAsync(di, L.idx.data(), 4 * L.idx.size(), hipMemcpyHostToDevice, d.stream) == hipSuccess &&
      hipMemcpyAsync(di + L.idx.size(), &list, 4, hipMemcpyHostToDevice, d.stream) == hipSuccess &&
      hipMemcpyAsync(ds, L.slots.data(), sizeof(bgv_dslot), hipMemcpyHostToDevice, d.stream) == hipSuccess &&
      bgv_launch_aggregate_bits(ds, di, di + L.idx.size(), !L.com_team.empty(), d.com_dir, d.com_pool, d.cache, dagg,
                                dout, d.stream) == hipSuccess &&
      hipMemcpyAsync(out96, dout, 96, hipMemcpyDeviceToHost, d.stream) == hipSuccess;
  const bool done = hipStreamSynchronize(d.stream) == hipSuccess;
  void* bufs[] = {di, dout, ds, dagg};
  for (void* p : bufs)
    if (p) (void)hipFree(p);
  return ok && done ? BGV_OK : -BGV_E_DEVICE;
}

int bgv_hash_to_g2(bgv_ctx* c, const uint8_t* msgs, const uint32_t* lens, size_t n, uint8_t* out192) {
  if (!c || (n && (!lens || !out192))) return -BGV_E_ARG;
  std::shared_lock<std::shared_mutex> clk(c->cache_mu);
  if (c->closed) return -BGV_E_CLOSED;
  if (n == 0) return BGV_OK;
  std::vector<uint32_t> offs(n);
  size_t tot = 0;
  for (size_t i = 0; i < n; ++i) {
    if (lens[i] > 1024) return -BGV_E_ARG;
    offs[i] = (uint32_t)tot;
    tot += lens[i];
  }
  if (tot && !msgs) return -BGV_E_ARG;
  std::lock_guard<std::mutex> lk(c->util_mu);
  Device& d = c->devs[0];
  HIPCHK(hipSetDevice(d.id));
  uint8_t *dm = nullptr, *dout = nullptr;
  uint32_t *doff = nullptr, *dlen = nullptr;
  HIPCHK(hipMalloc(reinterpret_cast<void**>(&dm), tot + 1));
  HIPCHK(hipMalloc(reinterpret_cast<void**>(&doff), 4 * n));
  HIPCHK(hipMalloc(reinterpret_cast<void**>(&dlen), 4 * n));
  HIPCHK(hipMalloc(reinterpret_cast<void**>(&dout), 192 * n));
  if (tot) HIPCHK(hipMemcpyAsync(dm, msgs, tot, hipMemcpyHostToDevice, d.stream));
  HIPCHK(hipMemcpyAsync(doff, offs.data(), 4 * n, hipMemcpyHostToDevice, d.stream));
  HIPCHK(hipMemcpyAsync(dlen, lens, 4 * n, hipMemcpyHostToDevice, d.stream));
  HIPCHK(bgv_launch_hash(dm, doff, dlen, (uint32_t)n, dout, d.stream));
  HIPCHK(hipMemcpyAsync(out192, dout, 192 * n, hipMemcpyDeviceToHost, d.stream));
  HIPCHK(hipStreamSynchronize(d.stream));
  (void)hipFree(dm);
  (void)hipFree(doff);
  (void)hipFree(dlen);
  (void)hipFree(dout);
  return BGV_OK;
}

int bgv_pubkeys_validate(bgv_ctx* c, const uint8_t* keys48, size_t n, int32_t* out_status, uint8_t* out96) {
  if (!c || (n && (!keys48 || !out_status))) return -BGV_E_ARG;
  std::shared_lock<std::shared_mutex> clk(c->cache_mu);
  if (c->closed) return -BGV_E_CLOSED;
  if (n == 0) return BGV_OK;
  std::lock_guard<std::mutex> lk(c->util_mu);
  Device& d = c->devs[0];
  HIPCHK(hipSetDevice(d.id));
  uint8_t *dk = nullptr, *dout = nullptr;
  int32_t* dst = nullptr;
  HIPCHK(hipMalloc(reinterpret_cast<void**>(&dk), 48 * n));
  HIPCHK(hipMalloc(reinterpret_cast<void**>(&dout), 96 * n));
  HIPCHK(hipMalloc(reinterpret_cast<void**>(&dst), 4 * n));
  HIPCHK(hipMemcpyAsync(dk, keys48, 48 * n, hipMemcpyHostToDevice, d.stream));
  HIPCHK(bgv_launch_pk_validate(dk, (uint32_t)n, dst, dout, d.stream));
  HIPCHK(hipMemcpyAsync(out_status, dst, 4 * n, hipMemcpyDeviceToHost, d.stream));
  if (out96) HIPCHK(hipMemcpyAsync(out96, dout, 96 * n, hipMemcpyDeviceToHost, d.stream));
  HIPCHK(hipStreamSynchronize(d.stream));
  (void)hipFree(dk);
  (void)hipFree(dout);
  (void)hipFree(dst);
  for (size_t i = 0; i < n; ++i) out_status[i] = -out_status[i];
  return BGV_OK;
}

int bgv_aggregate_signatures(bgv_ctx* c, const uint8_t* sigs96, const uint32_t* lens, const uint32_t* counts,
                             size_t naggs, uint8_t* out96, int32_t* out_status) {
  if (!c || (naggs && (!counts || !out96 || !out_status))) return -BGV_E_ARG;
  std::shared_lock<std::shared_mutex> clk(c->cache_mu);
  if (c->closed) return -BGV_E_CLOSED;
  if (naggs == 0) return BGV_OK;
  std::vector<uint32_t> first(naggs);
  size_t n = 0;
  for (size_t a = 0; a < naggs; ++a) {
    first[a] = (uint32_t)n;
    n += counts[a];
  }
  if (n && (!sigs96 || !lens)) return -BGV_E_ARG;
  std::vector<int32_t> st(n);
  std::lock_guard<std::mutex> lk(c->util_mu);
  Device& d = c->devs[0];
  HIPCHK(hipSetDevice(d.id));
  uint8_t *ds = nullptr, *dout = nullptr;
  uint32_t *dl = nullptr, *df = nullptr, *dc = nullptr;
  int32_t* dst = nullptr;
  void* pts = nullptr;
  HIPCHK(hipMalloc(reinterpret_cast<void**>(&ds), 96 * n + 1));
  HIPCHK(hipMalloc(reinterpret_cast<void**>(&dl), 4 * n + 4));
  HIPCHK(hipMalloc(reinterpret_cast<void**>(&dst), 4 * n + 4));
  HIPCHK(hipMalloc(&pts, bgv_g2_point_bytes() * n + 1));
  HIPCHK(hipMalloc(reinterpret_cast<void**>(&df), 4 * naggs));
  HIPCHK(hipMalloc(reinterpret_cast<void**>(&dc), 4 * naggs));
  HIPCHK(hipMalloc(reinterpret_cast<void**>(&dout), 96 * naggs));
  if (n) {
    HIPCHK(hipMemcpyAsync(ds, sigs96, 96 * n, hipMemcpyHostToDevice, d.stream));
    HIPCHK(hipMemcpyAsync(dl, lens, 4 * n, hipMemcpyHostToDevice, d.stream));
  }
  HIPCHK(hipMemcpyAsync(df, first.data(), 4 * naggs, hipMemcpyHostToDevice, d.stream));
  HIPCHK(hipMemcpyAsync(dc, counts, 4 * naggs, hipMemcpyHostToDevice, d.stream));
  HIPCHK(bgv_launch_sig_aggregate(ds, dl, (uint32_t)n, df, dc, (uint32_t)naggs, pts, dst, dout, d.stream));
  if (n) HIPCHK(hipMemcpyAsync(st.data(), dst, 4 * n, hipMemcpyDeviceToHost, d.stream));
  HIPCHK(hipMemcpyAsync(out96, dout, 96 * naggs, hipMemcpyDeviceToHost, d.stream));
  HIPCHK(hipStreamSynchronize(d.stream));
  void* bufs[] = {ds, dl, dst, pts, df, dc, dout};
  for (void* b : bufs) (void)hipFree(b);
  for (size_t a = 0; a < naggs; ++a) {
    int32_t code = counts[a] ? BGV_OK : -BGV_E_EMPTY_AGGREGATE;
    for (uint32_t k = 0; k < counts[a] && code == BGV_OK; ++k)
      if (st[first[a] + k] != BGV_OK) code = -st[first[a] + k];
    out_status[a] = code;
    if (code != BGV_OK) memset(out96 + 96 * a, 0, 96);
  }
  return BGV_OK;
}

int bgv_deposits_verify(bgv_ctx* c, const uint8_t* keys48, const uint8_t* msgs32, const uint8_t* sigs96, size_t n,
                        int32_t* out_valid) {
  if (!c || (n && (!keys48 || !msgs32 || !sigs96 || !out_valid))) return -BGV_E_ARG;
  if (n == 0) return BGV_OK;
  std::vector<int32_t> ks(n);
  std::vector<uint8_t> pk96(96 * n);
  int rc = bgv_pubkeys_validate(c, keys48, n, ks.data(), pk96.data());
  if (rc) return rc;
  std::vector<bgv_set> sets;
  std::vector<bgv_job> jobs;
  std::vector<size_t> which;
  for (size_t i = 0; i < n; ++i) {
    out_valid[i] = 0;
    if (ks[i] != BGV_OK) continue;
    bgv_set st{};
    st.n_pk = 1;
    st.sig_len = 96;
    st.pk_bytes = pk96.data() + 96 * i;
    st.msg = msgs32 + 32 * i;
    st.sig = sigs96 + 96 * i;
    jobs.push_back(bgv_job{(uint32_t)sets.size(), 1, 0});
    sets.push_back(st);
    which.push_back(i);
  }
  if (jobs.empty()) return BGV_OK;
  std::vector<int32_t> codes(jobs.size());
  rc = bgv_verify(c, jobs.data(), jobs.size(), sets.data(), sets.size(), BGV_MODE_PER_JOB, codes.data(), nullptr);
  if (rc) return rc;
  for (size_t k = 0; k < which.size(); ++k) out_valid[which[k]] = codes[k] == 1 ? 1 : 0;
  return BGV_OK;
}

int bgv_keygen(bgv_ctx* c, const uint8_t* sks, size_t n, int64_t cache_first, uint8_t* out48) {
  if (!c || (n && !sks)) return -BGV_E_ARG;
  std::lock_guard<std::mutex> plk(c->put_mu);
  std::unique_lock<std::shared_mutex> clk(c->cache_mu);
  if (c->closed) return -BGV_E_CLOSED;
  if (cache_first > (int64_t)c->n_pubkeys) return -BGV_E_ARG;
  if (n == 0) return BGV_OK;
  if (cache_first >= 0) {
    int rc = cache_reserve(c, (size_t)cache_first + n);
    if (rc) return rc;
  }
  const size_t esz = bgv_cache_entry_bytes();
  for (size_t di = 0; di < c->devs.size(); ++di) {
    Device& d = c->devs[di];
    if (cache_first < 0 && di > 0) break;
    HIPCHK(hipSetDevice(d.id));
    uint8_t *dsk = nullptr, *dout = nullptr;
    HIPCHK(hipMalloc(reinterpret_cast<void**>(&dsk), 32 * n));
    HIPCHK(hipMalloc(reinterpret_cast<void**>(&dout), 48 * n));
    HIPCHK(hipMemcpyAsync(dsk, sks, 32 * n, hipMemcpyHostToDevice, d.stream));
    bgv_cache_entry* dst =
        cache_first >= 0 ? reinterpret_cast<bgv_cache_entry*>(reinterpret_cast<uint8_t*>(d.cache) + esz * cache_first)
                         : nullptr;
    HIPCHK(bgv_launch_keygen(dsk, (uint32_t)n, dst, dout, d.stream));
    if (out48 && di == 0) HIPCHK(hipMemcpyAsync(out48, dout, 48 * n, hipMemcpyDeviceToHost, d.stream));
    HIPCHK(hipStreamSynchronize(d.stream));
    (void)hipFree(dsk);
    (void)hipFree(dout);
  }
  if (cache_first >= 0) {
    const size_t old_n = c->n_pubkeys.load();
    for (size_t i = 0; i < n; ++i) c->bad_pk.erase((uint32_t)(cache_first + i));
    c->n_pubkeys.store(std::max(old_n, (size_t)cache_first + n));
    if ((size_t)cache_first < old_n) return committees_refresh(c, (uint32_t)cache_first, n);
  }
  return BGV_OK;
}

int bgv_sign(bgv_ctx* c, const uint8_t* sks, const uint8_t* msgs, size_t n, uint8_t* out96) {
  if (!c || (n && (!sks || !msgs || !out96))) return -BGV_E_ARG;
  std::shared_lock<std::shared_mutex> clk(c->cache_mu);
  if (c->closed) return -BGV_E_CLOSED;
  if (n == 0) return BGV_OK;
  std::lock_guard<std::mutex> lk(c->util_mu);
  Device& d = c->devs[0];
  HIPCHK(hipSetDevice(d.id));
  uint8_t *dsk = nullptr, *dm = nullptr, *dout = nullptr;
  HIPCHK(hipMalloc(reinterpret_cast<void**>(&dsk), 32 * n));
  HIPCHK(hipMalloc(reinterpret_cast<void**>(&dm), 32 * n));
  HIPCHK(hipMalloc(reinterpret_cast<void**>(&dout), 96 * n));
  HIPCHK(hipMemcpyAsync(dsk, sks, 32 * n, hipMemcpyHostToDevice, d.stream));
  HIPCHK(hipMemcpyAsync(dm, msgs, 32 * n, hipMemcpyHostToDevice, d.stream));
  HIPCHK(bgv_launch_sign(dsk, dm, (uint32_t)n, dout, d.stream));
  HIPCHK(hipMemcpyAsync(out96, dout, 96 * n, hipMemcpyDeviceToHost, d.stream));
  HIPCHK(hipStreamSynchronize(d.stream));
  (void)hipFree(dsk);
  (void)hipFree(dm);
  (void)hipFree(dout);
  return BGV_OK;
}

int bgv_profile(bgv_ctx* c, int enable, double* kernel_ms, const char** names, int n, uint64_t* launches) {
  if (!c) return -BGV_E_ARG;
  std::lock_guard<std::mutex> lk(c->prof_mu);
  for (int k = 0; k < n && k < BGV_NKERNELS; ++k) {
    if (kernel_ms) kernel_ms[k] = c->kernel_ms[k];
    if (names) names[k] = BGV_KERNEL_NAMES[k];
  }
  if (launches) *launches = c->kernel_launches;
  if (enable >= 0) {
    c->profile = enable != 0;
    for (double& v : c->kernel_ms) v = 0;
    c->kernel_launches = 0;
  }
  return BGV_NKERNELS;
}

const char* bgv_strerror(int code) {
  if (code < 0) code = -code;
  switch (code) {
    case BGV_OK: return "BLST_SUCCESS";
    case BGV_BLST_BAD_ENCODING: return "BLST_BAD_ENCODING";
    case BGV_BLST_POINT_NOT_ON_CURVE: return "BLST_POINT_NOT_ON_CURVE";
    case BGV_BLST_POINT_NOT_IN_GROUP: return "BLST_POINT_NOT_IN_GROUP";
    case BGV_BLST_AGGR_TYPE_MISMATCH: return "BLST_AGGR_TYPE_MISMATCH";
    case BGV_BLST_VERIFY_FAIL: return "BLST_VERIFY_FAIL";
    case BGV_BLST_PK_IS_INFINITY: return "BLST_PK_IS_INFINITY";
    case BGV_BLST_BAD_SCALAR: return "BLST_BAD_SCALAR";
    case BGV_BLST_INVALID_SIZE: return "BLST_INVALID_SIZE";
    case BGV_E_EMPTY_AGGREGATE: return "EMPTY_AGGREGATE_ARRAY";
    case BGV_E_EMPTY_SET: return "Empty signature set";
    case BGV_E_BAD_INDEX: return "BGV_E_BAD_INDEX: validator index not in the device pubkey cache";
    case BGV_E_ARG: return "BGV_E_ARG: invalid argument";
    case BGV_E_DEVICE: return "BGV_E_DEVICE: HIP device error";
    case BGV_E_NOMEM: return "BGV_E_NOMEM";
    case BGV_E_CLOSED: return "QUEUE_ABORTED";
    default: return "BGV_E_UNKNOWN";
  }
}

}
```

### lodestar_amd/csrc/bgv_device.h

```cpp
#pragma once
#include <stdlib.h>
#include "bgv_layout.h"
#define BGV_KERNEL_SIDE 1
#include "bls_hash.h"
#include "bls_pairing.h"
#include "bls_team.h"

#ifndef BGV_WPE
#define BGV_WPE 1
#endif
#ifndef BGV_WPE_PREP
#define BGV_WPE_PREP 1
#endif
#ifndef BGV_PK_TREE_MIN
#define BGV_PK_TREE_MIN 16
#endif
#ifndef BGV_PK_TEAM_MAX
#define BGV_PK_TEAM_MAX 256
#endif
#define BGV_KATTR __launch_bounds__(64) __attribute__((amdgpu_waves_per_eu(BGV_WPE, BGV_WPE)))
#define BGV_KATTR_PREP __launch_bounds__(64) __attribute__((amdgpu_waves_per_eu(BGV_WPE_PREP, BGV_WPE_PREP)))

template <int M>
__device__ __forceinline__ uint32_t lane_xor(uint32_t v) {
  if constexpr (M == 32)
    return (uint32_t)__builtin_amdgcn_ds_bpermute((int)((threadIdx.x ^ 32u) << 2), (int)v);
  else
    return (uint32_t)__builtin_amdgcn_ds_swizzle((int)v, 0x1f | (M << 10));
}

template <int M, class P>
__device__ __forceinline__ P point_xor(const P& p) {
  constexpr int W = (int)(sizeof(P) / 4);
  P r;
  const uint32_t* a = reinterpret_cast<const uint32_t*>(&p);
  uint32_t* o = reinterpret_cast<uint32_t*>(&r);
  BGV_UNROLL for (int i = 0; i < W; ++i) o[i] = lane_xor<M>(a[i]);
  return r;
}



__device__ __forceinline__ bool grp_has(const bgv_dgroup& g, uint32_t k) {
  return k < g.n_slots && (k >= 64 || ((g.mask >> k) & 1));
}

__device__ __forceinline__ bool slot_live(const bgv_dslot& d, int32_t ss, int32_t ps) {
  return !(d.flags & BGV_SLOT_PAD) && (ss == BGV_ST_OK || ss == BGV_ST_INFINITY) && ps == BGV_ST_OK;
}

#include "bgv_launch.h"

static inline unsigned nblk(uint32_t n, unsigned t) { return (n + t - 1) / t; }

#define BGV_PREP_WIDE_MAX 340
#define BGV_MILLER_WIDE_MAX 1024

static inline uint32_t bgv_latency_max() {
  static const uint32_t v = [] {
    const char* e = getenv("BGV_LATENCY_MAX");
    return e ? (uint32_t)strtoul(e, nullptr, 10) : 16384u;
  }();
  return v;
}

static inline bool bgv_use_latency(const bgv_dev_batch& b, uint32_t pairs) {
  return b.path == BGV_PATH_LATENCY || (b.path == BGV_PATH_AUTO && pairs <= bgv_latency_max());
}

#define BGV_MARK(i) \
  if (s.kev) (void)hipEventRecord(s.kev[i], s.main)
```

### lodestar_amd/csrc/bgv_k_final.hip

```cpp
#include "bgv_device.h"

#include "bgv_team_dev.h"
#include "bgv_rns.h"


template <class O>
__device__ int32_t verdict_bits(O& o, const fp_t& u, const bgv_dgroup& g, const fp12_t* __restrict__ gu1, int fi) {
  int32_t v = o.is_fp6(u) ? 1 : 0;
  if (gu1) {
    const fp_t ur = g.ref1 ? reinterpret_cast<const fp_t*>(gu1 + (g.ref1 - 1))[fi] : u;
    if (o.is_fp6(o.mul(ur, o.conj(u))) && g.ref1) v |= 2;
  }
  return v;
}

extern "C" {

__global__ void BGV_KATTR k_final(const bgv_dgroup* __restrict__ groups, uint32_t ngroups,
                                  const fp12_t* __restrict__ f, const fp12_t* __restrict__ gpair,
                                  int32_t* __restrict__ verdict, fp12_t* __restrict__ gprod,
                                  fp12_t* __restrict__ gu, const fp12_t* __restrict__ gu1) {
  __shared__ fp_t lds[BGV_FINAL_TEAMS][2 * BGV_TEAM_COMPS];
  __shared__ uint32_t lens[BGV_FINAL_TEAMS];
  const int team = threadIdx.x / BGV_TEAM, c = threadIdx.x % BGV_TEAM;
  const int cc = c < BGV_TEAM_COMPS ? c : c - 4;
  const uint32_t gi = blockIdx.x * BGV_FINAL_TEAMS + team;
  const uint32_t gg = gi < ngroups ? gi : ngroups - 1;
  const bgv_dgroup g = groups[gg];
  if (c == 0) lens[team] = g.n_slots;
  __syncthreads();
  uint32_t nmax = 0;
  BGV_UNROLL for (int t = 0; t < BGV_FINAL_TEAMS; ++t) nmax = lens[t] > nmax ? lens[t] : nmax;
  const int fi = tm_fp_index(cc);
  const fp_t one_c = cc == 0 ? fp_one() : fp_zero();
  tm_dev_ops o{lds[team], lds[team] + BGV_TEAM_COMPS, c, cc};
  const fp_t* fs = reinterpret_cast<const fp_t*>(f + g.first_slot);
  constexpr int kFp12 = (int)(sizeof(fp12_t) / sizeof(fp_t));
  fp_t x = reinterpret_cast<const fp_t*>(gpair + gg)[fi];
  fp_t y = grp_has(g, 0) ? fs[fi] : one_c;
  BGV_NO_UNROLL for (uint32_t k = 0; k < nmax; ++k) {
    const fp_t yn = grp_has(g, k + 1) ? fs[kFp12 * (k + 1) + fi] : one_c;
    x = o.mul(x, y);
    y = yn;
  }
  if (gprod && gi < ngroups && c < BGV_TEAM_COMPS) reinterpret_cast<fp_t*>(gprod + gi)[fi] = x;
  const fp_t u = tm_final_exp_u(o, x);
  if (gu && gi < ngroups && c < BGV_TEAM_COMPS) reinterpret_cast<fp_t*>(gu + gi)[fi] = u;
  const int32_t v = verdict_bits(o, u, g, gu1, fi);
  if (gi < ngroups && c == 0) verdict[gi] = v;
}

#define BGV_FINAL12_TEAMS 5
#define BGV_FINAL12_ARGS                                                                                     \
  const bgv_dgroup *__restrict__ groups, uint32_t ngroups, const fp12_t *__restrict__ f,                     \
      const fp12_t *__restrict__ gpair, int32_t *__restrict__ verdict, fp12_t *__restrict__ gprod,          \
      fp12_t *__restrict__ gu, const fp12_t *__restrict__ gu1, const fp12_t *__restrict__ gpkp
}
__device__ __forceinline__ void final12_body(BGV_FINAL12_ARGS) {
  __shared__ fp_t lds[BGV_FINAL12_TEAMS + 1][2 * BGV_TEAM_COMPS];
  __shared__ uint32_t lens[BGV_FINAL12_TEAMS + 1];
  const int team = threadIdx.x / BGV_TEAM_COMPS, c = threadIdx.x % BGV_TEAM_COMPS;
  const uint32_t gi = blockIdx.x * BGV_FINAL12_TEAMS + team;
  const bool live = team < BGV_FINAL12_TEAMS && gi < ngroups;
  const bgv_dgroup g = groups[live ? gi : ngroups - 1];
  uint64_t m = live ? g.mask & (g.n_slots >= 64 ? ~0ull : ((1ull << g.n_slots) - 1)) : 0;
  const bool uni = gpkp && live && (g.flags & BGV_GROUP_UNIFORM);
  if (uni) m = 0;
  if (c == 0) lens[team] = (uint32_t)__popcll(m);
  __syncthreads();
  uint32_t nmax = 0;
  BGV_UNROLL for (int t = 0; t <= BGV_FINAL12_TEAMS; ++t) nmax = lens[t] > nmax ? lens[t] : nmax;
  const int fi = tm_fp_index(c);
  const fp_t one_c = c == 0 ? fp_one() : fp_zero();
  tm_dev_ops_t<BGV_TEAM_COMPS> o{lds[team], lds[team] + BGV_TEAM_COMPS, c, c};
  const fp_t* fs = reinterpret_cast<const fp_t*>(f + g.first_slot);
  constexpr int kFp12 = (int)(sizeof(fp12_t) / sizeof(fp_t));
  fp_t x = reinterpret_cast<const fp_t*>(gpair + (live ? gi : ngroups - 1))[fi];
  auto next = [&]() {
    if (!m) return one_c;
    const int k = __ffsll((unsigned long long)m) - 1;
    m &= m - 1;
    return fs[kFp12 * k + fi];
  };
  fp_t y = next();
  BGV_NO_UNROLL for (uint32_t k = 0; k < nmax; ++k) {
    const fp_t yn = next();
    x = o.mul(x, y);
    y = yn;
  }
  if (gpkp) x = o.mul(x, uni ? reinterpret_cast<const fp_t*>(gpkp + gi)[fi] : one_c);
  if (gprod && live) reinterpret_cast<fp_t*>(gprod + gi)[fi] = x;
  const fp_t u = tm_final_exp_u(o, x);
  if (gu && live) reinterpret_cast<fp_t*>(gu + gi)[fi] = u;
  const int32_t v = verdict_bits(o, u, g, gu1, fi);
  if (live && c == 0) verdict[gi] = v;
}

extern "C" __global__ void __launch_bounds__(64) k_final_wident(const bgv_dgroup* __restrict__ groups, uint32_t ngroups,
                                                     const fp12_t* __restrict__ gu, const fp12_t* __restrict__ gu1,
                                                     int32_t* __restrict__ verdict) {
  __shared__ fp_t lds[BGV_FINAL12_TEAMS + 1][2 * BGV_TEAM_COMPS];
  __shared__ uint32_t lens[BGV_FINAL12_TEAMS + 1];
  const int team = threadIdx.x / BGV_TEAM_COMPS, c = threadIdx.x % BGV_TEAM_COMPS;
  const uint32_t gi = blockIdx.x * BGV_FINAL12_TEAMS + team;
  const bool live = team < BGV_FINAL12_TEAMS && gi < ngroups;
  const bgv_dgroup g = groups[live ? gi : ngroups - 1];
  const bool wt = live && (g.flags & BGV_GROUP_WEIGHTED) && g.ref1;
  if (c == 0) lens[team] = wt ? g.n_slots : 0u;
  if (!__syncthreads_or(wt ? 1 : 0)) return;
  uint32_t wmax = 0;
  BGV_UNROLL for (int t = 0; t <= BGV_FINAL12_TEAMS; ++t) wmax = lens[t] > wmax ? lens[t] : wmax;
  const int fi = tm_fp_index(c);
  const fp_t one_c = c == 0 ? fp_one() : fp_zero();
  tm_dev_ops_t<BGV_TEAM_COMPS> o{lds[team], lds[team] + BGV_TEAM_COMPS, c, c};
  const fp_t u = wt ? reinterpret_cast<const fp_t*>(gu + gi)[fi] : one_c;
  const fp_t ur = wt ? reinterpret_cast<const fp_t*>(gu1 + (g.ref1 - 1))[fi] : one_c;
  const fp_t cu = o.conj(u);
  fp_t P = ur;
  int32_t found = 0;
  BGV_NO_UNROLL for (uint32_t w = 1; w <= wmax; ++w) {
    const bool hit = o.is_fp6(o.mul(P, cu));
    if (wt && hit && found == 0 && w <= g.n_slots) found = (int32_t)w;
    P = o.mul(P, ur);
  }
  if (wt && c == 0) verdict[gi] = (verdict[gi] & 1) | (found << 8);
}
extern "C" {
__global__ void __launch_bounds__(64) __attribute__((amdgpu_waves_per_eu(2, 2))) k_final12(BGV_FINAL12_ARGS) {
  final12_body(groups, ngroups, f, gpair, verdict, gprod, gu, gu1, gpkp);
}

}
template <bool LEAN>
__device__ auto bgv_fold_ops_pick() {
  if constexpr (LEAN)
    return tm_wide8_lean_ops{};
  else
    return tm_wide_ops_t<false, 8>{};
}
#ifndef BGV_FOLD_TEAMS
#define BGV_FOLD_TEAMS 16
#endif
#define BGV_FOLD_THREADS (BGV_FOLD_TEAMS * BGV_TEAM)
#define BGV_FOLD_RNS_THREADS BGV_RNS_THREADS
static_assert(BGV_FOLD_RNS_THREADS % BGV_TEAM == 0 && BGV_FOLD_RNS_THREADS >= BGV_FOLD_THREADS, "fold block");
template <int ENGINE>
__device__ __forceinline__ void final_fold_body(const bgv_dgroup* __restrict__ groups, uint32_t ngroups,
                                                const fp12_t* __restrict__ f, const fp12_t* __restrict__ gpair,
                                                int32_t* __restrict__ verdict, fp12_t* __restrict__ gprod,
                                                fp12_t* __restrict__ gu, const fp12_t* __restrict__ gu1,
                                                const fp12_t* __restrict__ fsig, const fp12_t* __restrict__ gpkp) {
  constexpr int kTeams = (ENGINE == 2 ? BGV_FOLD_RNS_THREADS : BGV_FOLD_THREADS) / BGV_TEAM;
  __shared__ fp_t lds[kTeams][2 * BGV_TEAM_COMPS];
  __shared__ fp_t part[BGV_FOLD_TEAMS][BGV_TEAM_COMPS];
  __shared__ fp_t W[BGV_TEAM_COMPS], WA[BGV_TEAM_COMPS], WB[BGV_TEAM_COMPS], WP[8 * BGV_TEAM_COMPS];
  const int team = threadIdx.x / BGV_TEAM, c = threadIdx.x % BGV_TEAM;
  const bool fold = team < BGV_FOLD_TEAMS;
  const int cc = c < BGV_TEAM_COMPS ? c : c - 4;
  const uint32_t gi = blockIdx.x;
  const bgv_dgroup g = groups[gi < ngroups ? gi : ngroups - 1];
  const int fi = tm_fp_index(cc);
  const fp_t one_c = cc == 0 ? fp_one() : fp_zero();
  tm_dev_ops o{lds[team], lds[team] + BGV_TEAM_COMPS, c, cc};
  const fp_t* fs = reinterpret_cast<const fp_t*>(f + g.first_slot);
  constexpr int kFp12 = (int)(sizeof(fp12_t) / sizeof(fp_t));
  fp_t x = team == 0 && !fsig ? reinterpret_cast<const fp_t*>(gpair + (gi < ngroups ? gi : ngroups - 1))[fi] : one_c;
  const fp_t* ss = fsig ? reinterpret_cast<const fp_t*>(fsig + g.first_slot) : nullptr;
  const bool uni = gpkp && gi < ngroups && (g.flags & BGV_GROUP_UNIFORM);
  const uint32_t nmax = uni ? 0u : (g.n_slots + BGV_FOLD_TEAMS - 1) / BGV_FOLD_TEAMS;
  BGV_NO_UNROLL for (uint32_t k = 0; k < nmax; ++k) {
    const uint32_t idx = team + BGV_FOLD_TEAMS * k;
    const bool in = fold && grp_has(g, idx);
    const fp_t y = in ? fs[kFp12 * idx + fi] : one_c;
    x = o.mul(x, y);
    if (ss) x = o.mul(x, in ? ss[kFp12 * idx + fi] : one_c);
  }
  BGV_UNROLL for (int w = BGV_FOLD_TEAMS; w > 1; w >>= 1) {
    if (fold && c < BGV_TEAM_COMPS) part[team][cc] = x;
    __syncthreads();
    const int t2 = 2 * (team % (w >> 1));
    x = o.mul(part[t2][cc], part[t2 + 1][cc]);
  }
  if (gpkp) x = o.mul(x, uni && team == 0 ? reinterpret_cast<const fp_t*>(gpkp + gi)[fi] : one_c);
  if (gprod && gi < ngroups && team == 0 && c < BGV_TEAM_COMPS) reinterpret_cast<fp_t*>(gprod + gi)[fi] = x;
  if (team == 0 && c < BGV_TEAM_COMPS) W[cc] = x;
  __syncthreads();
  if constexpr (ENGINE == 2) {
    __shared__ rns_smem RS;
    rns_ops ro;
    ro.init(&RS, threadIdx.x);
    const uint32_t u = tm_final_exp_u(ro, ro.from_fp(W[ro.c]));
    const int rfi = tm_fp_index(ro.c);
    if (gu && gi < ngroups) {
      const fp_t uf = ro.to_fp(u);
      if (ro.i == 0) reinterpret_cast<fp_t*>(gu + gi)[rfi] = uf;
    }
    int32_t v = ro.is_fp6(u) ? 1 : 0;
    if (gu1 && g.ref1) {
      const uint32_t ur = ro.from_fp(reinterpret_cast<const fp_t*>(gu1 + (g.ref1 - 1))[rfi]);
      if (ro.is_fp6(ro.mul(ur, ro.conj(u)))) v |= 2;
    }
    if (gi < ngroups && threadIdx.x == 0) verdict[gi] = v;
  } else {
    const int wc = threadIdx.x % BGV_TEAM_COMPS, wq = threadIdx.x / BGV_TEAM_COMPS;
    using OW = decltype(bgv_fold_ops_pick<ENGINE == 1>());
    OW ow;
    ow.A = WA;
    ow.B = WB;
    ow.P = WP;
    ow.c = wc;
    ow.q = wq;
    if constexpr (ENGINE == 1) tm_sqr_rec8(wc, wq, &ow.rx, &ow.ry);
    const fp_t xw = W[wc];
    const int wfi = tm_fp_index(wc);
    const fp_t u = tm_final_exp_u(ow, xw);
    if (gu && gi < ngroups && wq == 0) reinterpret_cast<fp_t*>(gu + gi)[wfi] = u;
    const int32_t v = verdict_bits(ow, u, g, gu1, wfi);
    if (gi < ngroups && threadIdx.x == 0) verdict[gi] = v;
  }
}
extern "C" {
#define BGV_FOLD_ARGS                                                                                         \
  const bgv_dgroup *__restrict__ groups, uint32_t ngroups, const fp12_t *__restrict__ f,                     \
      const fp12_t *__restrict__ gpair, int32_t *__restrict__ verdict, fp12_t *__restrict__ gprod,          \
      fp12_t *__restrict__ gu, const fp12_t *__restrict__ gu1, const fp12_t *__restrict__ fsig,                \
      const fp12_t *__restrict__ gpkp
__global__ void __launch_bounds__(BGV_FOLD_RNS_THREADS) k_final_fold(BGV_FOLD_ARGS) {
  final_fold_body<2>(groups, ngroups, f, gpair, verdict, gprod, gu, gu1, fsig, gpkp);
}
__global__ void __launch_bounds__(BGV_FOLD_THREADS) k_final_fold_p8(BGV_FOLD_ARGS) {
  final_fold_body<1>(groups, ngroups, f, gpair, verdict, gprod, gu, gu1, fsig, gpkp);
}
__global__ void __launch_bounds__(BGV_FOLD_THREADS) k_final_fold_sel(BGV_FOLD_ARGS) {
  final_fold_body<0>(groups, ngroups, f, gpair, verdict, gprod, gu, gu1, fsig, gpkp);
}

__global__ void BGV_KATTR k_fp12_prod(const fp12_t* __restrict__ in, uint32_t n, uint32_t chunk,
                                      fp12_t* __restrict__ out, uint32_t nout) {
  __shared__ fp_t lds[BGV_FINAL_TEAMS][2 * BGV_TEAM_COMPS];
  const int team = threadIdx.x / BGV_TEAM, c = threadIdx.x % BGV_TEAM;
  const int cc = c < BGV_TEAM_COMPS ? c : c - 4;
  const uint32_t t = blockIdx.x * BGV_FINAL_TEAMS + team;
  const uint32_t lo = t * chunk;
  const uint32_t len = lo < n ? (n - lo < chunk ? n - lo : chunk) : 0;
  const int fi = tm_fp_index(cc);
  const fp_t one_c = cc == 0 ? fp_one() : fp_zero();
  tm_dev_ops o{lds[team], lds[team] + BGV_TEAM_COMPS, c, cc};
  fp_t x = one_c;
  for (uint32_t k = 0; k < chunk; ++k) {
    const fp_t y = k < len ? reinterpret_cast<const fp_t*>(in + lo + k)[fi] : one_c;
    x = o.mul(x, y);
  }
  if (t < nout && c < BGV_TEAM_COMPS) reinterpret_cast<fp_t*>(out + t)[fi] = x;
}

__global__ void k_fp12_to_bytes(const fp12_t* __restrict__ in, uint8_t* __restrict__ out576) {
  if (blockIdx.x != 0 || threadIdx.x != 0) return;
  const fp_t* v = reinterpret_cast<const fp_t*>(in);
  for (int i = 0; i < 12; ++i) {
    uint8_t b[48];
    fp_to_be48(b, fp_from_mont(v[i]));
    for (int q = 0; q < 48; ++q) out576[48 * i + q] = b[q];
  }
}

__global__ void k_fp12_n_to_bytes(const fp12_t* __restrict__ in, uint32_t n, uint8_t* __restrict__ out) {
  const uint32_t i = blockIdx.x * blockDim.x + threadIdx.x;
  if (i >= n) return;
  const fp_t* v = reinterpret_cast<const fp_t*>(in + i);
  for (int k = 0; k < 12; ++k) {
    uint8_t b[48];
    fp_to_be48(b, fp_from_mont(v[k]));
    for (int q = 0; q < 48; ++q) out[576ull * i + 48 * k + q] = b[q];
  }
}

__global__ void k_fp12_from_bytes(const uint8_t* __restrict__ in, uint32_t n, fp12_t* __restrict__ out,
                                  int32_t* __restrict__ status, fp12_t* __restrict__ one) {
  const uint32_t i = blockIdx.x * blockDim.x + threadIdx.x;
  if (i == 0) *one = fp12_one();
  if (i >= n) return;
  fp_t* v = reinterpret_cast<fp_t*>(out + i);
  int32_t st = BGV_OK;
  for (int k = 0; k < 12; ++k) {
    uint8_t b[48];
    for (int q = 0; q < 48; ++q) b[q] = in[576ull * i + 48 * k + q];
    const fp_t r = fp_from_be48(b);
    if (!fp_raw_lt_p(r)) st = BGV_BAD_ENCODING;
    v[k] = fp_to_mont(r);
  }
  status[i] = st;
}

}

uint32_t bgv_fold_pairs_max() { return bgv_latency_max(); }
#ifndef BGV_RETRY_FOLD_MAX
#define BGV_RETRY_FOLD_MAX 512
#endif

hipError_t bgv_launch_groups(const bgv_dev_batch& b, const bgv_streams& s, bool pairs) {
  if (b.ngroups == 0) return hipSuccess;
  BGV_MARK(4);
  if (pairs) {
    const hipError_t e = bgv_launch_gpairs(b, s.main);
    if (e != hipSuccess) return e;
  }
  static const bool lean = [] {
    const char* e = getenv("BGV_FOLD_LEAN");
    return !(e && atoi(e) == 0);
  }();
  static const bool rns = [] {
    const char* e = getenv("BGV_FOLD_RNS");
    return !(e && atoi(e) == 0);
  }();
  if (b.weighted && !b.gu) return hipErrorInvalidValue;
  static const uint32_t retry_fold_max = [] {
    const char* e = getenv("BGV_RETRY_FOLD_MAX");
    return e ? (uint32_t)atoi(e) : (uint32_t)BGV_RETRY_FOLD_MAX;
  }();
  const bool small_retry = pairs && b.uniform && b.ngroups <= retry_fold_max;
  if ((!b.uniform && b.nslots + b.ngroups <= bgv_latency_max()) || small_retry)
    hipLaunchKernelGGL(rns ? k_final_fold : (lean ? k_final_fold_p8 : k_final_fold_sel), dim3(b.ngroups),
                       dim3(rns ? BGV_FOLD_RNS_THREADS : BGV_FOLD_THREADS), 0, s.main, b.groups,
                       b.ngroups, b.f, b.gpair,
                       b.verdict, b.gprod, b.gu, b.gu1,
                       !pairs && bgv_sig_pairs(b) ? static_cast<const fp12_t*>(b.fsig) : nullptr,
                       b.uniform ? static_cast<const fp12_t*>(b.gpkp) : nullptr);
  else
    hipLaunchKernelGGL(k_final12, dim3(nblk(b.ngroups, BGV_FINAL12_TEAMS)), dim3(64), 0, s.main, b.groups,
                       b.ngroups, b.f, b.gpair, b.verdict, b.gprod, b.gu, b.gu1,
                       b.uniform ? static_cast<const fp12_t*>(b.gpkp) : nullptr);
  if (b.weighted)
    hipLaunchKernelGGL(k_final_wident, dim3(nblk(b.ngroups, BGV_FINAL12_TEAMS)), dim3(64), 0, s.main, b.groups,
                       b.ngroups, static_cast<const fp12_t*>(b.gu), b.gu1, b.verdict);
  BGV_MARK(5);
  return hipGetLastError();
}
hipError_t bgv_launch_partial(const bgv_dev_batch& b, uint32_t g0, uint32_t ng, void* scratch, uint8_t* out576,
                              hipStream_t st) {
  fp12_t* tmp = reinterpret_cast<fp12_t*>(scratch);
  const uint32_t chunk = 32, n1 = (ng + chunk - 1) / chunk;
  hipLaunchKernelGGL(k_fp12_prod, dim3(nblk(n1 ? n1 : 1, BGV_FINAL_TEAMS)), dim3(64), 0, st, b.gprod + g0, ng, chunk,
                     tmp + 1, n1);
  hipLaunchKernelGGL(k_fp12_prod, dim3(1), dim3(64), 0, st, tmp + 1, n1, n1 ? n1 : 1, tmp, 1u);
  hipLaunchKernelGGL(k_fp12_to_bytes, dim3(1), dim3(64), 0, st, tmp, out576);
  return hipGetLastError();
}
size_t bgv_fp12_bytes() { return sizeof(fp12_t); }
hipError_t bgv_launch_fp12_bytes(const fp12_t* in, uint32_t n, uint8_t* out576, hipStream_t st) {
  if (n == 0) return hipSuccess;
  hipLaunchKernelGGL(k_fp12_n_to_bytes, dim3(nblk(n, 64)), dim3(64), 0, st, in, n, out576);
  return hipGetLastError();
}

hipError_t bgv_launch_final_verify(const uint8_t* in, uint32_t n, void* vals, void* one, const bgv_dgroup* group,
                                   int32_t* status, int32_t* verdict, hipStream_t st) {
  hipLaunchKernelGGL(k_fp12_from_bytes, dim3(nblk(n, 64)), dim3(64), 0, st, in, n, reinterpret_cast<fp12_t*>(vals),
                     status, reinterpret_cast<fp12_t*>(one));
  hipLaunchKernelGGL(k_final, dim3(1), dim3(64), 0, st, group, 1u, reinterpret_cast<const fp12_t*>(vals),
                     reinterpret_cast<const fp12_t*>(one), verdict, static_cast<fp12_t*>(nullptr),
                     static_cast<fp12_t*>(nullptr), static_cast<const fp12_t*>(nullptr));
  return hipGetLastError();
}
```

### lodestar_amd/csrc/bgv_k_lat.h

```cpp
#pragma once
#include "bgv_k_tasks.h"

static __device__ __forceinline__ g2_jac* split_q1(fp12_t* f, uint32_t s) { return reinterpret_cast<g2_jac*>(f + s); }
static __device__ __forceinline__ g2_aff* split_sig(fp12_t* f, uint32_t s) {
  return reinterpret_cast<g2_aff*>(reinterpret_cast<uint8_t*>(f + s) + sizeof(g2_jac));
}
static_assert(sizeof(g2_jac) + sizeof(g2_aff) <= sizeof(fp12_t), "split intermediates fit in f[s]");

template <class PW>
__device__ __noinline__ void task_map_t(uint32_t s, int which, const bgv_dslot* __restrict__ slots, g2_jac* out,
                                        bool writer) {
  const bgv_dslot& d = slots[s];
  if (d.flags & BGV_SLOT_PAD) return;
  uint8_t msg[32];
  for (int i = 0; i < 32; ++i) msg[i] = d.msg[i];
  fp2_t u0, u1;
  hash_to_field_fp2(&u0, &u1, msg, 32);
  const g2_jac q = sswu_g2_jac_t<PW>(which ? u1 : u0, fp_sqrt_minus5());
  if (writer) *out = q;
}

template <class PW>
__device__ __noinline__ void task_sig_decode_t(uint32_t s, const bgv_dslot* __restrict__ slots, g2_aff* out,
                                               int32_t* __restrict__ sig_status, bool writer) {
  const bgv_dslot& d = slots[s];
  int32_t st = BGV_ST_OK;
  g2_aff a;
  bool fin = false;
  if (d.flags & BGV_SLOT_PAD) {
    st = BGV_ST_INFINITY;
  } else if (d.sig_len != 96) {
    st = BGV_INVALID_SIZE;
  } else {
    uint8_t b[96];
    for (int i = 0; i < 96; ++i) b[i] = d.sig[i];
    bool inf;
    st = g2_decompress_t<PW>(&a, &inf, b);
    if (st == BGV_OK) {
      if (inf)
        st = BGV_ST_INFINITY;
      else
        fin = true;
    }
  }
  if (writer) {
    if (fin) *out = a;
    sig_status[s] = st;
  }
}
```

### lodestar_amd/csrc/bgv_k_prep.hip

```cpp
#include "bgv_k_lat.h"
#include "bgv_pk_bits.h"
#include "bgv_team_dev.h"
#include "bgv_tcurve.h"
#include "bgv_tg1.h"
#include "bgv_tround_dev.h"

static __constant__ uint8_t kTcProg[TCP_TABLE_BYTES] = TCP_TABLE_INIT;
static __constant__ uint8_t kTg1Prog[TG1_TABLE_BYTES] = TG1_TABLE_INIT;

struct tc_dev_engine {
  const uint8_t* prog;
  fp_t* S;
  int c;
  bool bad;
  __device__ void run(int off) {
    int pos = off;
    const int nr = prog[pos++];
    for (int r = 0; r < nr; ++r) {
      const int T = prog[pos], M = prog[pos + 1];
      pos += 2;
      const int rb = tmp_rec_bytes(T, M);
      int out;
      const fp_t v = tmp_lane_any(S, prog + pos + c * rb, T, M, &out);
      S[out] = v;
      __syncthreads();
      pos += BGV_TEAM * rb;
    }
  }
  __device__ void copy(int dst, int src) {
    if (c < 6 && dst != src) S[TCP_BANK(dst) + c] = S[TCP_BANK(src) + c];
    __syncthreads();
  }
  __device__ void neg_y(int b) {
    if (c == 2 || c == 3) S[TCP_BANK(b) + c] = fp_neg(S[TCP_BANK(b) + c]);
    __syncthreads();
  }
  __device__ void check_add() {
    if (c == 0) {
      const auto z2 = [&](int s) { return fp_is_zero(S[s]) && fp_is_zero(S[s + 1]); };
      bad = bad || z2(TC_CHK_A) || z2(TC_CHK_B);
    }
  }
};

#ifndef BGV_WPE_AGG
#define BGV_WPE_AGG 2
#endif

static_assert(sizeof(g1_jac) == sizeof(bgv_dcommittee::total), "bgv_dcommittee keeps a Jacobian G1 point");
template <int T>
__device__ __forceinline__ g1_jac pk_bits_sum(bool act, uint32_t l, const uint32_t* __restrict__ words,
                                              const uint32_t* __restrict__ members, uint32_t n, bool comp,
                                              const g1_aff* __restrict__ cache) {
  g1_jac acc = jac_infinity<fp_t>();
  if (act) {
    pkb_cursor c = pkb_begin(l);
    uint32_t pos;
    if (pkb_next(c, words, n, comp, T, &pos)) {
      acc = jac_from_aff(cache[members[pos]]);
      bool have = pkb_next(c, words, n, comp, T, &pos);
      g1_aff cur = cache[members[have ? pos : 0]];
      while (have) {
        uint32_t pn;
        const bool hn = pkb_next(c, words, n, comp, T, &pn);
        const g1_aff nxt = cache[members[hn ? pn : pos]];
        acc = jac_add_aff(acc, cur);
        cur = nxt;
        pos = hn ? pn : pos;
        have = hn;
      }
    }
  }
  if constexpr (T == 64) {
    acc = jac_add(acc, point_xor<32>(acc));
    acc = jac_add(acc, point_xor<16>(acc));
  }
  acc = jac_add(acc, point_xor<8>(acc));
  acc = jac_add(acc, point_xor<4>(acc));
  acc = jac_add(acc, point_xor<2>(acc));
  acc = jac_add(acc, point_xor<1>(acc));
  return acc;
}

template <int T>
__device__ __forceinline__ void pk_bits_slot(bool act, uint32_t s, uint32_t l, const bgv_dslot* __restrict__ slots,
                                             const uint32_t* __restrict__ pk_idx,
                                             const bgv_dcommittee* __restrict__ dir,
                                             const uint32_t* __restrict__ pool, const g1_aff* __restrict__ cache,
                                             g1_jac* __restrict__ pk_agg, bool writer) {
  const uint32_t* words = nullptr;
  const uint32_t* members = nullptr;
  const bgv_dcommittee* cm = nullptr;
  uint32_t n = 0;
  bool comp = false;
  if (act) {
    const bgv_dslot& d = slots[s];
    cm = dir + pk_idx[d.pk_off];
    words = pk_idx + d.pk_off + 1;
    members = pool + cm->off;
    n = cm->n;
    comp = (d.flags & BGV_SLOT_PK_COMPLEMENT) != 0;
  }
  g1_jac acc = pk_bits_sum<T>(act, l, words, members, n, comp, cache);
  if (act && writer) {
    if (comp) acc = jac_add(*reinterpret_cast<const g1_jac*>(cm->total), jac_neg(acc));
    pk_agg[s] = acc;
  }
}

extern "C" {

__device__ __forceinline__ void pk_aggw_body(const bgv_dslot* __restrict__ slots, uint32_t s,
                                             const uint32_t* __restrict__ pk_idx, const g1_aff* __restrict__ cache,
                                             g1_jac* __restrict__ pk_agg) {
  const bgv_dslot& d = slots[s];
  if ((d.flags & BGV_SLOT_PAD) || !(d.flags & BGV_SLOT_PK_CACHED) || d.n_pk <= BGV_PK_TEAM_MAX) return;
  const uint32_t l = threadIdx.x;
  g1_jac acc = jac_infinity<fp_t>();
  for (uint32_t k = l; k < d.n_pk; k += 64) acc = jac_add_aff(acc, cache[pk_idx[d.pk_off + k]]);
  acc = jac_add(acc, point_xor<32>(acc));
  acc = jac_add(acc, point_xor<16>(acc));
  acc = jac_add(acc, point_xor<8>(acc));
  acc = jac_add(acc, point_xor<4>(acc));
  acc = jac_add(acc, point_xor<2>(acc));
  acc = jac_add(acc, point_xor<1>(acc));
  if (l == 0) pk_agg[s] = acc;
}

__device__ __forceinline__ void pk_agg16_body(const bgv_dslot* __restrict__ slots, uint32_t nslots, uint32_t blk,
                                              const uint32_t* __restrict__ pk_idx, const g1_aff* __restrict__ cache,
                                              g1_jac* __restrict__ pk_agg) {
  const uint32_t s = blk * (64 / 16) + threadIdx.x / 16;
  const uint32_t l = threadIdx.x % 16;
  const bgv_dslot* d = s < nslots ? &slots[s] : nullptr;
  const bool act = d && !(d->flags & BGV_SLOT_PAD) && (d->flags & BGV_SLOT_PK_CACHED) &&
                   d->n_pk >= BGV_PK_TREE_MIN && d->n_pk <= BGV_PK_TEAM_MAX;
  g1_jac acc = jac_infinity<fp_t>();
  if (act) {
    const uint32_t* idx = pk_idx + d->pk_off;
    const uint32_t n = d->n_pk;
    acc = jac_from_aff(cache[idx[l]]);
    uint32_t k = l + 16;
    g1_aff cur = cache[idx[k < n ? k : l]];
    for (; k < n; k += 16) {
      const uint32_t kn = k + 16 < n ? k + 16 : k;
      const g1_aff nxt = cache[idx[kn]];
      acc = jac_add_aff(acc, cur);
      cur = nxt;
    }
  }
  acc = jac_add(acc, point_xor<8>(acc));
  acc = jac_add(acc, point_xor<4>(acc));
  acc = jac_add(acc, point_xor<2>(acc));
  acc = jac_add(acc, point_xor<1>(acc));
  if (act && l == 0) pk_agg[s] = acc;
}

__device__ __forceinline__ void pk_agg_one(const bgv_dslot* __restrict__ slots, uint32_t s,
                                           const uint32_t* __restrict__ pk_idx, const g1_aff* __restrict__ cache,
                                           g1_jac* __restrict__ pk_agg) {
  const bgv_dslot& d = slots[s];
  if ((d.flags & BGV_SLOT_PAD) || !(d.flags & BGV_SLOT_PK_CACHED) || d.n_pk < BGV_PK_TREE_MIN) return;
  if (d.n_pk > BGV_PK_TEAM_MAX) {
    pk_aggw_body(slots, s, pk_idx, cache, pk_agg);
    return;
  }
  const uint32_t l = threadIdx.x % 16;
  const uint32_t* idx = pk_idx + d.pk_off;
  const uint32_t n = d.n_pk;
  g1_jac acc = jac_from_aff(cache[idx[l]]);
  for (uint32_t k = l + 16; k < n; k += 16) acc = jac_add_aff(acc, cache[idx[k]]);
  acc = jac_add(acc, point_xor<8>(acc));
  acc = jac_add(acc, point_xor<4>(acc));
  acc = jac_add(acc, point_xor<2>(acc));
  acc = jac_add(acc, point_xor<1>(acc));
  if (threadIdx.x == 0) pk_agg[s] = acc;
}

#ifndef BGV_WPE_BITS
#define BGV_WPE_BITS 1
#endif
__global__ void __launch_bounds__(64) __attribute__((amdgpu_waves_per_eu(BGV_WPE_BITS, BGV_WPE_BITS)))
k_pk_agg_bits(const bgv_dslot* __restrict__ slots, const uint32_t* __restrict__ com, uint32_t nteam, uint32_t nwave,
              const uint32_t* __restrict__ pk_idx, const bgv_dcommittee* __restrict__ dir,
              const uint32_t* __restrict__ pool, const g1_aff* __restrict__ cache, g1_jac* __restrict__ pk_agg) {
  const uint32_t nb_team = (nteam + 3) / 4;
  if (blockIdx.x < nb_team) {
    const uint32_t q = blockIdx.x * 4 + threadIdx.x / 16, l = threadIdx.x % 16;
    const bool act = q < nteam;
    pk_bits_slot<16>(act, act ? com[q] : 0u, l, slots, pk_idx, dir, pool, cache, pk_agg, l == 0);
  } else {
    const uint32_t q = nteam + (blockIdx.x - nb_team);
    const bool act = q < nteam + nwave;
    pk_bits_slot<64>(act, act ? com[q] : 0u, threadIdx.x, slots, pk_idx, dir, pool, cache, pk_agg, threadIdx.x == 0);
  }
}

#define BGV_PK_ONE_WAVE_MIN 49
__device__ __noinline__ void pk_bits_one(const bgv_dslot* __restrict__ slots, uint32_t s,
                                            const uint32_t* __restrict__ pk_idx,
                                            const bgv_dcommittee* __restrict__ dir,
                                            const uint32_t* __restrict__ pool, const g1_aff* __restrict__ cache,
                                            g1_jac* __restrict__ pk_agg) {
  const bgv_dslot& d = slots[s];
  if ((d.flags & BGV_SLOT_PAD) || !(d.flags & BGV_SLOT_PK_COMMITTEE)) return;
  const uint32_t n = dir[pk_idx[d.pk_off]].n;
  if (pkb_terms(n, d.n_pk, (d.flags & BGV_SLOT_PK_COMPLEMENT) != 0) < BGV_PK_ONE_WAVE_MIN)
    pk_bits_slot<16>(true, s, threadIdx.x % 16, slots, pk_idx, dir, pool, cache, pk_agg, threadIdx.x == 0);
  else
    pk_bits_slot<64>(true, s, threadIdx.x, slots, pk_idx, dir, pool, cache, pk_agg, threadIdx.x == 0);
}

__global__ void __launch_bounds__(64) k_committee_total(bgv_dcommittee* __restrict__ dir,
                                                        const uint32_t* __restrict__ handles, uint32_t nh,
                                                        const uint32_t* __restrict__ pool,
                                                        const g1_aff* __restrict__ cache) {
  if (blockIdx.x >= nh) return;
  bgv_dcommittee* cm = dir + handles[blockIdx.x];
  const g1_jac acc = pk_bits_sum<64>(true, threadIdx.x, nullptr, pool + cm->off, cm->n, false, cache);
  if (threadIdx.x == 0) *reinterpret_cast<g1_jac*>(cm->total) = acc;
}

__global__ void __launch_bounds__(64) k_pk_agg(const bgv_dslot* __restrict__ slots, uint32_t nslots,
                                               const uint32_t* __restrict__ pk_idx,
                                               const g1_aff* __restrict__ cache, g1_jac* __restrict__ pk_agg) {
  if (blockIdx.x < nslots) pk_aggw_body(slots, blockIdx.x, pk_idx, cache, pk_agg);
}

__global__ void BGV_KATTR_PREP k_prep_a(const bgv_dslot* __restrict__ slots, uint32_t nslots, g2_jac* __restrict__ h,
                                        fp12_t* __restrict__ f, int32_t* __restrict__ sig_status,
                                        const uint32_t* __restrict__ pk_idx, const g1_aff* __restrict__ cache,
                                        const uint8_t* __restrict__ pk_bytes, g1_jac* __restrict__ rpk,
                                        int32_t* __restrict__ pk_status, g1_jac* __restrict__ pk_agg) {
  const uint32_t s = blockIdx.x * blockDim.x + threadIdx.x;
  if (s >= nslots) return;
  if (blockIdx.y == 0)
    task_map_t<bgv_pow_lane>(s, 0, slots, h + s, true);
  else if (blockIdx.y == 1)
    task_map_t<bgv_pow_lane>(s, 1, slots, split_q1(f, s), true);
  else if (blockIdx.y == 2)
    task_sig_decode_t<bgv_pow_lane>(s, slots, split_sig(f, s), sig_status, true);
  else
    task_pk(s, slots, pk_idx, cache, pk_bytes, rpk, pk_status, pk_agg);
}

__global__ void __launch_bounds__(64) k_prep_team(const bgv_dslot* __restrict__ slots, uint32_t nslots,
                                                  g2_jac* __restrict__ h, fp12_t* __restrict__ f,
                                                  g2_jac* __restrict__ rsig, int32_t* __restrict__ sig_status) {
  if (blockIdx.y == 2) {
    const uint32_t s = blockIdx.x * blockDim.x + threadIdx.x;
    if (s >= nslots || (slots[s].flags & BGV_SLOT_PAD) || sig_status[s] != BGV_ST_OK) return;
    if (!g2_in_subgroup(jac_from_aff(*split_sig(f, s)))) sig_status[s] = BGV_POINT_NOT_IN_GROUP;
    return;
  }
  __shared__ uint8_t prog[TCP_TABLE_BYTES];
  __shared__ fp_t Sall[BGV_FINAL_TEAMS][TCP_NSLOT];
  __shared__ int flags[BGV_FINAL_TEAMS];
  for (int i = threadIdx.x; i < TCP_TABLE_BYTES; i += 64) prog[i] = kTcProg[i];
  const int team = threadIdx.x / BGV_TEAM, c = threadIdx.x % BGV_TEAM;
  const uint32_t u = blockIdx.x * BGV_FINAL_TEAMS + team;
  const uint32_t uu = u < nslots ? u : nslots - 1;
  const bgv_dslot& d = slots[uu];
  const bool real = u < nslots && !(d.flags & BGV_SLOT_PAD);
  fp_t* S = Sall[team];
  if (c == 6) {
    S[TCP_S_ONE] = fp_one();
  } else if (c >= 7 && c < 11) {
    const fp2_t cx = BGV_PSI_CX, cy = BGV_PSI_CY;
    const fp2_t& v = c < 9 ? cx : cy;
    S[c < 9 ? TCP_S_PSI_CX + (c - 7) : TCP_S_PSI_CY + (c - 9)] = (c & 1) ? v.c0 : v.c1;
  } else if (c == 11) {
    S[TCP_S_PSI2_CX] = fp_t{BGV_PSI2_CX};
  } else if (c == 12) {
    S[TCP_S_PSI2_CY] = fp_t{BGV_PSI2_CY};
  }
  for (int i = c; i < TC_ISO_NCONST; i += BGV_TEAM) S[TCP_S_ISO + i] = tc_iso_const(i);
  tc_dev_engine e{prog, S, c, false};
  if (blockIdx.y == 0) {
    if (c < 6) {
      S[TCP_BANK(1) + c] = reinterpret_cast<const fp_t*>(h + uu)[c];
      S[TCP_BANK(2) + c] = reinterpret_cast<const fp_t*>(split_q1(f, uu))[c];
    }
    __syncthreads();
    tc_clear_cofactor(e);
    if (c == 0) flags[team] = e.bad ? 1 : 0;
    __syncthreads();
    if (real) {
      if (!flags[team]) {
        if (c < 6) reinterpret_cast<fp_t*>(h + uu)[c] = S[TCP_BANK(3) + c];
      } else if (c == 0) {
        h[uu] = g2_clear_cofactor(jac_add(iso_map_g2_jac(h[uu]), iso_map_g2_jac(*split_q1(f, uu))));
      }
    }
  } else {
    const bool ok = sig_status[uu] == BGV_ST_OK;
    if (c < 4)
      S[TCP_BANK(1) + c] = reinterpret_cast<const fp_t*>(split_sig(f, uu))[c];
    else if (c < 6)
      S[TCP_BANK(1) + c] = c == 4 ? fp_one() : fp_zero();
    __syncthreads();
    tc_mul_glv(e, d.scalar);
    if (real && ok && c < 6) reinterpret_cast<fp_t*>(rsig + uu)[c] = S[TCP_BANK(4) + c];
  }
}

struct tc_wide_engine : tr_wide_engine {
  __device__ void copy(int dst, int src) {
    if (q == 0 && c < 6 && dst != src) S[TCP_BANK(dst) + c] = S[TCP_BANK(src) + c];
    __syncthreads();
  }
  __device__ void neg_y(int b) {
    if (q == 0 && (c == 2 || c == 3)) S[TCP_BANK(b) + c] = fp_neg(S[TCP_BANK(b) + c]);
    __syncthreads();
  }
  __device__ void check_add() {
    if (q == 0 && c == 0) {
      const auto z2 = [&](int s) { return fp_is_zero(S[s]) && fp_is_zero(S[s + 1]); };
      bad = bad || z2(TC_CHK_A) || z2(TC_CHK_B);
    }
  }
};

struct tg1_wide_engine : tr_wide_engine {
  __device__ void copy(int dst, int src) {
    if (q == 0 && c < 3 && dst != src) S[TG1_BANK(dst) + c] = S[TG1_BANK(src) + c];
    __syncthreads();
  }
};

__global__ void __launch_bounds__(64) k_prep_wide(const bgv_dslot* __restrict__ slots, uint32_t nslots,
                                                  g2_jac* __restrict__ h, fp12_t* __restrict__ f,
                                                  g2_jac* __restrict__ rsig, int32_t* __restrict__ sig_status,
                                                  const uint32_t* __restrict__ pk_idx,
                                                  const g1_aff* __restrict__ cache, const uint8_t* __restrict__ pk_bytes,
                                                  g1_jac* __restrict__ rpk, int32_t* __restrict__ pk_status,
                                                  g1_jac* __restrict__ pk_agg,
                                                  const bgv_dcommittee* __restrict__ com_dir,
                                                  const uint32_t* __restrict__ com_pool) {
  static_assert(TG1_TABLE_BYTES <= TCP_TABLE_BYTES && TG1_NSLOT <= TCP_NSLOT, "plane 3 reuses the G2 buffers");
  __shared__ uint8_t prog[TCP_TABLE_BYTES];
  __shared__ fp_t S[TCP_NSLOT];
  __shared__ fp_t RP[64];
  __shared__ int flag;
  if (blockIdx.y == 3) {
    const uint32_t s = blockIdx.x;
    if (pk_agg) pk_agg_one(slots, s, pk_idx, cache, pk_agg);
    if (pk_agg) pk_bits_one(slots, s, pk_idx, com_dir, com_pool, cache, pk_agg);
    if (threadIdx.x == 0) {
      g1_jac acc;
      const bool go = task_pk_sum(s, slots, pk_idx, cache, pk_bytes, pk_status, pk_agg, &acc);
      flag = go ? 1 : 0;
      if (go) {
        S[TG1_BANK(1)] = acc.x;
        S[TG1_BANK(1) + 1] = acc.y;
        S[TG1_BANK(1) + 2] = acc.z;
      }
      S[TG1_S_ONE] = fp_one();
      S[TG1_S_BETA] = fp_t{BGV_BETA_MX2};
    }
    for (int i = threadIdx.x; i < TG1_TABLE_BYTES; i += 64) prog[i] = kTg1Prog[i];
    __syncthreads();
    if (!flag) return;
    const int lane = threadIdx.x;
    tg1_wide_engine e{{prog, S, RP, tr_wide_lane_c(lane), tr_wide_lane_q(lane), false}};
    tg1_mul_glv(e, slots[s].scalar);
    if (lane < 3) reinterpret_cast<fp_t*>(rpk + s)[lane] = S[TG1_BANK(4) + lane];
    if (lane == 0) pk_status[s] = BGV_ST_OK;
    return;
  }
  const uint32_t uu = blockIdx.x;
  const int lane = threadIdx.x, c = lane % BGV_TEAM, q = lane / BGV_TEAM;
  const bgv_dslot& d = slots[uu];
  const bool real = !(d.flags & BGV_SLOT_PAD);
  if (blockIdx.y == 2 && (!real || sig_status[uu] != BGV_ST_OK)) return;
  for (int i = lane; i < TCP_TABLE_BYTES; i += 64) prog[i] = kTcProg[i];
  if (q == 0) {
    if (c == 6) {
      S[TCP_S_ONE] = fp_one();
    } else if (c >= 7 && c < 11) {
      const fp2_t cx = BGV_PSI_CX, cy = BGV_PSI_CY;
      const fp2_t& v = c < 9 ? cx : cy;
      S[c < 9 ? TCP_S_PSI_CX + (c - 7) : TCP_S_PSI_CY + (c - 9)] = (c & 1) ? v.c0 : v.c1;
    } else if (c == 11) {
      S[TCP_S_PSI2_CX] = fp_t{BGV_PSI2_CX};
    } else if (c == 12) {
      S[TCP_S_PSI2_CY] = fp_t{BGV_PSI2_CY};
    }
  }
  for (int i = lane; i < TC_ISO_NCONST; i += 64) S[TCP_S_ISO + i] = tc_iso_const(i);
  tc_wide_engine e{{prog, S, RP, tr_wide_lane_c(lane), tr_wide_lane_q(lane), false}};
  if (blockIdx.y == 0) {
    if (q == 0 && c < 6) {
      S[TCP_BANK(1) + c] = reinterpret_cast<const fp_t*>(h + uu)[c];
      S[TCP_BANK(2) + c] = reinterpret_cast<const fp_t*>(split_q1(f, uu))[c];
    }
    __syncthreads();
    tc_clear_cofactor(e);
    if (lane == 0) flag = e.bad ? 1 : 0;
    __syncthreads();
    if (real) {
      if (!flag) {
        if (q == 0 && c < 6) reinterpret_cast<fp_t*>(h + uu)[c] = S[TCP_BANK(3) + c];
      } else if (lane == 0) {
        h[uu] = g2_clear_cofactor(jac_add(iso_map_g2_jac(h[uu]), iso_map_g2_jac(*split_q1(f, uu))));
      }
    }
  } else if (blockIdx.y == 1) {
    const bool ok = sig_status[uu] == BGV_ST_OK;
    if (q == 0) {
      if (c < 4)
        S[TCP_BANK(1) + c] = reinterpret_cast<const fp_t*>(split_sig(f, uu))[c];
      else if (c < 6)
        S[TCP_BANK(1) + c] = c == 4 ? fp_one() : fp_zero();
    }
    __syncthreads();
    tc_mul_glv(e, d.scalar);
    if (real && ok && q == 0 && c < 6) reinterpret_cast<fp_t*>(rsig + uu)[c] = S[TCP_BANK(4) + c];
  } else {
    if (q == 0 && c < 6) {
      const fp_t v = c < 4 ? reinterpret_cast<const fp_t*>(split_sig(f, uu))[c] : (c == 4 ? fp_one() : fp_zero());
      S[TCP_BANK(0) + c] = v;
      S[TCP_BANK(4) + c] = v;
    }
    __syncthreads();
    const int a = tc_to_jac(e, tc_mul_x_abs(e));
    if (lane == 0) {
      const g2_jac p = jac_from_aff(*split_sig(f, uu));
      bool in;
      if (e.bad) {
        in = g2_in_subgroup(p);
      } else {
        const fp_t* B = S + TCP_BANK(a);
        const g2_jac xp = {{B[0], B[1]}, {B[2], B[3]}, {B[4], B[5]}};
        in = jac_eq(g2_psi(p), jac_neg(xp));
      }
      if (!in) sig_status[uu] = BGV_POINT_NOT_IN_GROUP;
    }
  }
}

__global__ void __launch_bounds__(64) __attribute__((amdgpu_waves_per_eu(BGV_WPE_AGG, BGV_WPE_AGG)))
k_pk_agg16(const bgv_dslot* __restrict__ slots, uint32_t nslots, const uint32_t* __restrict__ pk_idx,
           const g1_aff* __restrict__ cache, g1_jac* __restrict__ pk_agg) {
  pk_agg16_body(slots, nslots, blockIdx.x, pk_idx, cache, pk_agg);
}

__global__ void k_pk_sum_out(const bgv_dslot* __restrict__ slot, const uint32_t* __restrict__ idx,
                             const g1_aff* __restrict__ cache, const g1_jac* __restrict__ pk_agg,
                             uint8_t* __restrict__ out96) {
  if (blockIdx.x != 0 || threadIdx.x != 0) return;
  int32_t st = BGV_OK;
  const g1_jac acc = pk_sum(slot[0], idx, cache, nullptr, pk_agg, 0, &st);
  g1_aff a;
  const bool fin = jac_to_aff(&a, acc);
  uint8_t b[96];
  g1_serialize(b, a, !fin);
  for (int i = 0; i < 96; ++i) out96[i] = b[i];
}

}

hipError_t bgv_launch_prep(const bgv_dev_batch& b, const bgv_streams& s) {
  const uint32_t n = b.nslots;
  if (n == 0) return hipSuccess;
  BGV_MARK(0);
  const bool tree = b.max_npk >= BGV_PK_TREE_MIN;
  const uint32_t ncom = b.ncom_team + b.ncom_wave;
  const bool agg = tree || ncom > 0;
  const bool wide = bgv_use_latency(b, n + b.ngroups) && n <= BGV_PREP_WIDE_MAX;
  if (wide) {
    const g1_aff* cache = reinterpret_cast<const g1_aff*>(b.cache_opaque);
    const hipError_t e = bgv_launch_prep_wave(b, s.main);
    if (e != hipSuccess) return e;
    hipLaunchKernelGGL(k_prep_wide, dim3(n, 4), dim3(64), 0, s.main, b.slots, n, b.h, b.f, b.rsig, b.sig_status,
                       b.pk_idx, cache, b.pk_bytes, b.rpk, b.pk_status, agg ? b.pk_agg : nullptr, b.com_dir, b.com_pool);
    BGV_MARK(1);
    return hipGetLastError();
  }
  if (ncom)
    hipLaunchKernelGGL(k_pk_agg_bits, dim3(nblk(b.ncom_team, 4) + b.ncom_wave), dim3(64), 0, s.main, b.slots, b.com,
                       b.ncom_team, b.ncom_wave, b.pk_idx, b.com_dir, b.com_pool,
                       reinterpret_cast<const g1_aff*>(b.cache_opaque), b.pk_agg);
  if (tree)
    hipLaunchKernelGGL(k_pk_agg16, dim3(nblk(n, 4)), dim3(64), 0, s.main, b.slots, n, b.pk_idx,
                       reinterpret_cast<const g1_aff*>(b.cache_opaque), b.pk_agg);
  if (b.max_npk > BGV_PK_TEAM_MAX)
    hipLaunchKernelGGL(k_pk_agg, dim3(n), dim3(64), 0, s.main, b.slots, n, b.pk_idx,
                       reinterpret_cast<const g1_aff*>(b.cache_opaque), b.pk_agg);
  if (bgv_use_latency(b, n + b.ngroups)) {
    hipLaunchKernelGGL(k_prep_a, dim3(nblk(n, 64), 4), dim3(64), 0, s.main, b.slots, n, b.h, b.f, b.sig_status,
                       b.pk_idx, reinterpret_cast<const g1_aff*>(b.cache_opaque), b.pk_bytes, b.rpk, b.pk_status,
                       agg ? b.pk_agg : nullptr);
    hipLaunchKernelGGL(k_prep_team, dim3(nblk(n, BGV_FINAL_TEAMS), 3), dim3(64), 0, s.main, b.slots, n, b.h, b.f,
                       b.rsig, b.sig_status);
  } else {
    const hipError_t e = bgv_launch_prep_bulk(b, s, agg);
    if (e != hipSuccess) return e;
  }
  BGV_MARK(1);
  return hipGetLastError();
}

hipError_t bgv_launch_aggregate(const bgv_dslot* slot, const uint32_t* idx, uint32_t n, const bgv_cache_entry* cache,
                                void* agg, uint8_t* out96, hipStream_t st) {
  const g1_aff* c = reinterpret_cast<const g1_aff*>(cache);
  g1_jac* a = reinterpret_cast<g1_jac*>(agg);
  const bool tree = n >= BGV_PK_TREE_MIN;
  if (tree && n <= BGV_PK_TEAM_MAX) hipLaunchKernelGGL(k_pk_agg16, dim3(1), dim3(64), 0, st, slot, 1u, idx, c, a);
  if (tree && n > BGV_PK_TEAM_MAX) hipLaunchKernelGGL(k_pk_agg, dim3(1), dim3(64), 0, st, slot, 1u, idx, c, a);
  hipLaunchKernelGGL(k_pk_sum_out, dim3(1), dim3(64), 0, st, slot, idx, c, tree ? a : nullptr, out96);
  return hipGetLastError();
}

hipError_t bgv_launch_aggregate_bits(const bgv_dslot* slot, const uint32_t* idx, const uint32_t* list, bool team,
                                     const bgv_dcommittee* dir, const uint32_t* pool, const bgv_cache_entry* cache,
                                     void* agg, uint8_t* out96, hipStream_t st) {
  const g1_aff* c = reinterpret_cast<const g1_aff*>(cache);
  g1_jac* a = reinterpret_cast<g1_jac*>(agg);
  hipLaunchKernelGGL(k_pk_agg_bits, dim3(1), dim3(64), 0, st, slot, list, team ? 1u : 0u, team ? 0u : 1u, idx, dir, pool,
                     c, a);
  hipLaunchKernelGGL(k_pk_sum_out, dim3(1), dim3(64), 0, st, slot, idx, c, a, out96);
  return hipGetLastError();
}

hipError_t bgv_launch_committee_totals(bgv_dcommittee* dir, const uint32_t* handles, uint32_t nh, const uint32_t* pool,
                                       const bgv_cache_entry* cache, hipStream_t st) {
  if (nh == 0) return hipSuccess;
  hipLaunchKernelGGL(k_committee_total, dim3(nh), dim3(64), 0, st, dir, handles, nh, pool,
                     reinterpret_cast<const g1_aff*>(cache));
  return hipGetLastError();
}
```

### lodestar_amd/csrc/bgv_k_prep_bulk.hip

```cpp
#ifndef BGV_LZ2_CLASSIC
#define BGV_LZ2_WIDE 1
#define BGV_LZ2_WIDE_STRICT 1
#endif
#include "bgv_k_tasks.h"

#ifndef BGV_WPE_BULK
#define BGV_WPE_BULK 1
#endif
#define BGV_KATTR_BULK __launch_bounds__(64) __attribute__((amdgpu_waves_per_eu(BGV_WPE_BULK, BGV_WPE_BULK)))

extern "C" {

__global__ void BGV_KATTR_BULK k_prep(const bgv_dslot* __restrict__ slots, uint32_t nslots, g2_jac* __restrict__ rsig,
                                      int32_t* __restrict__ sig_status, g2_jac* __restrict__ h,
                                      const uint32_t* __restrict__ pk_idx, const g1_aff* __restrict__ cache,
                                      const uint8_t* __restrict__ pk_bytes, g1_jac* __restrict__ rpk,
                                      int32_t* __restrict__ pk_status, const g1_jac* __restrict__ pk_agg,
                                      const uint32_t* __restrict__ uniq, uint32_t nuniq, uint32_t task0) {
  const uint32_t s = blockIdx.x * blockDim.x + threadIdx.x;
  const uint32_t task = blockIdx.y + task0;
  if (task == 0) {
    if (uniq) {
      if (s < nuniq) task_hash(uniq[s], slots, h);
    } else if (s < nslots) {
      task_hash(s, slots, h);
    }
    return;
  }
  if (s >= nslots) return;
  if (task == 1)
    task_sig(s, slots, rsig, sig_status);
  else
    task_pk(s, slots, pk_idx, cache, pk_bytes, rpk, pk_status, pk_agg);
}

}

hipError_t bgv_launch_prep_bulk(const bgv_dev_batch& b, const bgv_streams& s, bool tree) {
  static const bool split = [] {
    const char* e = getenv("BGV_PREP_SPLIT");
    return e && atoi(e) > 0;
  }();
  for (uint32_t t0 = 0; t0 < 3; t0 += split ? 1 : 3) {
    hipLaunchKernelGGL(k_prep, dim3(nblk(b.nslots, 64), split ? 1 : 3), dim3(64), 0, s.main, b.slots, b.nslots, b.rsig,
                       b.sig_status, b.h, b.pk_idx, reinterpret_cast<const g1_aff*>(b.cache_opaque), b.pk_bytes, b.rpk,
                       b.pk_status, tree ? b.pk_agg : nullptr, b.uniq, b.nuniq, t0);
  }
  return hipGetLastError();
}
```

### lodestar_amd/csrc/bgv_k_prep_wave.hip

```cpp
#ifndef BGV_PREP_WAVE_LANE_MUL
#define BGV_WAVE_UNIFORM_MUL 1
#endif
#include "bgv_k_lat.h"
#include "bgv_wfp.h"

extern "C" __global__ void __launch_bounds__(64) k_prep_a_wave(const bgv_dslot* __restrict__ slots, uint32_t nslots,
                                                               g2_jac* __restrict__ h, fp12_t* __restrict__ f,
                                                               int32_t* __restrict__ sig_status) {
  const uint32_t s = blockIdx.x;
  const bool w = threadIdx.x == 0;
  if (blockIdx.y == 0)
    task_map_t<bgv_pow_wave>(s, 0, slots, h + s, w);
  else if (blockIdx.y == 1)
    task_map_t<bgv_pow_wave>(s, 1, slots, split_q1(f, s), w);
  else
    task_sig_decode_t<bgv_pow_wave>(s, slots, split_sig(f, s), sig_status, w);
}

hipError_t bgv_launch_prep_wave(const bgv_dev_batch& b, hipStream_t st) {
  if (b.nslots == 0) return hipSuccess;
  hipLaunchKernelGGL(k_prep_a_wave, dim3(b.nslots, 3), dim3(64), 0, st, b.slots, b.nslots, b.h, b.f, b.sig_status);
  return hipGetLastError();
}
```

### lodestar_amd/csrc/bgv_k_tasks.h

```cpp
#pragma once
#include "bgv_device.h"

static __device__ __noinline__ void task_sig(uint32_t s, const bgv_dslot* __restrict__ slots, g2_jac* __restrict__ rsig,
                                      int32_t* __restrict__ sig_status) {
  const bgv_dslot& d = slots[s];
  int32_t st = BGV_ST_OK;
  if (d.flags & BGV_SLOT_PAD) {
    st = BGV_ST_INFINITY;
  } else if (d.sig_len != 96) {
    st = BGV_INVALID_SIZE;
  } else {
    uint8_t b[96];
    for (int i = 0; i < 96; ++i) b[i] = d.sig[i];
    g2_aff a;
    bool inf;
    st = g2_decompress(&a, &inf, b);
    if (st == BGV_OK) {
      if (inf) {
        st = BGV_ST_INFINITY;
      } else {
        const g2_jac j = jac_from_aff(a);
        if (!g2_in_subgroup(j))
          st = BGV_POINT_NOT_IN_GROUP;
        else
          rsig[s] = jac_mul_glv(j, d.scalar);
      }
    }
  }
  sig_status[s] = st;
}

static __device__ __noinline__ void task_hash(uint32_t s, const bgv_dslot* __restrict__ slots, g2_jac* __restrict__ h) {
  const bgv_dslot& d = slots[s];
  if (d.flags & BGV_SLOT_PAD) return;
  uint8_t msg[32];
  for (int i = 0; i < 32; ++i) msg[i] = d.msg[i];
  h[s] = hash_to_g2(msg, 32);
}

__device__ __noinline__ static g1_jac pk_sum(const bgv_dslot& d, const uint32_t* __restrict__ pk_idx,
                                      const g1_aff* __restrict__ cache, const uint8_t* __restrict__ pk_bytes,
                                      const g1_jac* __restrict__ pk_agg, uint32_t s, int32_t* st) {
  if (d.flags & BGV_SLOT_PK_COMMITTEE) return pk_agg[s];
  g1_jac acc = jac_infinity<fp_t>();
  const bool cached = (d.flags & BGV_SLOT_PK_CACHED) != 0;
  const bool tree = pk_agg != nullptr && cached && d.n_pk >= BGV_PK_TREE_MIN;
  if (tree) return pk_agg[s];
  for (uint32_t k = 0; k < d.n_pk; ++k) {
    g1_aff a;
    if (cached) {
      a = cache[pk_idx[d.pk_off + k]];
    } else {
      uint8_t b[96];
      const uint8_t* src = pk_bytes + 96ull * (d.pk_off + k);
      for (int i = 0; i < 96; ++i) b[i] = src[i];
      bool inf;
      const int rc = g1_deserialize(&a, &inf, b);
      if (rc != BGV_OK) {
        *st = rc;
        break;
      }
      if (inf) continue;
    }
    acc = jac_add_aff(acc, a);
  }
  return acc;
}

static __device__ __noinline__ bool task_pk_sum(uint32_t s, const bgv_dslot* __restrict__ slots,
                                                const uint32_t* __restrict__ pk_idx, const g1_aff* __restrict__ cache,
                                                const uint8_t* __restrict__ pk_bytes, int32_t* __restrict__ pk_status,
                                                const g1_jac* __restrict__ pk_agg, g1_jac* acc) {
  const bgv_dslot& d = slots[s];
  if (d.flags & BGV_SLOT_PAD) {
    pk_status[s] = BGV_ST_INFINITY;
    return false;
  }
  int32_t st = BGV_ST_OK;
  const g1_jac a = pk_sum(d, pk_idx, cache, pk_bytes, pk_agg, s, &st);
  if (st != BGV_OK || jac_is_inf(a)) {
    pk_status[s] = st != BGV_OK ? st : BGV_ST_INFINITY;
    return false;
  }
  *acc = a;
  return true;
}

static __device__ __noinline__ void task_pk(uint32_t s, const bgv_dslot* __restrict__ slots,
                                     const uint32_t* __restrict__ pk_idx, const g1_aff* __restrict__ cache,
                                     const uint8_t* __restrict__ pk_bytes, g1_jac* __restrict__ rpk,
                                     int32_t* __restrict__ pk_status, const g1_jac* __restrict__ pk_agg) {
  const bgv_dslot& d = slots[s];
  int32_t st = BGV_ST_OK;
  if (d.flags & BGV_SLOT_PAD) {
    pk_status[s] = BGV_ST_INFINITY;
    return;
  }
  const g1_jac acc = pk_sum(d, pk_idx, cache, pk_bytes, pk_agg, s, &st);
  if (st == BGV_OK) {
    const g1_jac rp = jac_mul_glv(acc, d.scalar);
    if (jac_is_inf(rp))
      st = BGV_ST_INFINITY;
    else
      rpk[s] = rp;
  }
  pk_status[s] = st;
}
```

### lodestar_amd/csrc/bgv_launch.h

```cpp
#pragma once
#include <hip/hip_runtime.h>
#include <stddef.h>
#include <stdint.h>

#include "bgv_layout.h"

struct fp12_t;
template <class F>
struct jac_t;
template <class F>
struct aff_t;
struct fp_t;
struct fp2_t;

struct bgv_cache_entry;

#define BGV_PATH_AUTO 0
#ifndef BGV_PATH_BULK
#define BGV_PATH_BULK 1
#define BGV_PATH_LATENCY 2
#endif

struct bgv_dev_batch {
  uint32_t nslots, ngroups;
  uint32_t max_npk;
  bool uniform;
  int path;
  const uint32_t* uniq;
  uint32_t nuniq;
  const bgv_dslot* slots;
  const bgv_dgroup* groups;
  const uint32_t* pk_idx;
  const bgv_cache_entry* cache_opaque;
  const uint8_t* pk_bytes;
  const uint32_t* com;
  uint32_t ncom_team, ncom_wave;
  const bgv_dcommittee* com_dir;
  const uint32_t* com_pool;
  jac_t<fp2_t>* rsig;
  jac_t<fp2_t>* h;
  jac_t<fp_t>* rpk;
  fp12_t* f;
  fp12_t* fsig;
  jac_t<fp_t>* pk_agg;
  int32_t* sig_status;
  int32_t* pk_status;
  jac_t<fp2_t>* gsum;
  fp12_t* gpair;
  jac_t<fp_t>* gpk;
  fp12_t* gpkp;
  const uint32_t* upk;
  uint32_t npk;
  bool weighted;
  fp12_t* gprod;
  fp12_t* gu;
  const fp12_t* gu1;
  int32_t* verdict;
  uint32_t* lines;
  uint32_t lines_cap;
#ifdef BGV_KERNEL_SIDE
  const aff_t<fp_t>* cache_ptr() const { return reinterpret_cast<const aff_t<fp_t>*>(cache_opaque); }
#endif
};

#define BGV_NKERNELS 3
#define BGV_NSETKERNELS 2
static const char* const BGV_KERNEL_NAMES[BGV_NKERNELS] = {"k_prep", "k_miller", "k_final"};
struct bgv_streams {
  hipStream_t main;
  hipEvent_t* kev;
};
hipError_t bgv_launch_sets(const bgv_dev_batch& b, const bgv_streams& s);
bool bgv_sig_pairs(const bgv_dev_batch& b);
hipError_t bgv_launch_prep(const bgv_dev_batch& b, const bgv_streams& s);
hipError_t bgv_launch_prep_bulk(const bgv_dev_batch& b, const bgv_streams& s, bool tree);
hipError_t bgv_launch_prep_wave(const bgv_dev_batch& b, hipStream_t st);
hipError_t bgv_launch_miller(const bgv_dev_batch& b, const bgv_streams& s);
hipError_t bgv_launch_miller_bulk(const bgv_dev_batch& b, uint32_t ngroups, hipStream_t st);
uint32_t bgv_lines_pairs(const bgv_dev_batch& b);
bool bgv_single_pass_miller();
size_t bgv_line_record_bytes();
hipError_t bgv_launch_groups(const bgv_dev_batch& b, const bgv_streams& s, bool pairs);
uint32_t bgv_fold_pairs_max();
hipError_t bgv_launch_gpairs(const bgv_dev_batch& b, hipStream_t st);
size_t bgv_slot_bytes();
size_t bgv_slot_mem_bytes(uint32_t cap_slots);
size_t bgv_group_bytes();
size_t bgv_cache_entry_bytes();
void bgv_carve(bgv_dev_batch* b, void* slot_mem, uint32_t cap_slots, void* group_mem, uint32_t cap_groups);
hipError_t bgv_launch_cache_put(const uint8_t* keys, uint32_t n, int fmt, bgv_cache_entry* cache, int32_t* status,
                                hipStream_t st);
hipError_t bgv_launch_aggregate(const bgv_dslot* slot, const uint32_t* idx, uint32_t n, const bgv_cache_entry* cache,
                                void* agg, uint8_t* out96, hipStream_t st);
hipError_t bgv_launch_aggregate_bits(const bgv_dslot* slot, const uint32_t* idx, const uint32_t* list, bool team,
                                     const bgv_dcommittee* dir, const uint32_t* pool, const bgv_cache_entry* cache,
                                     void* agg, uint8_t* out96, hipStream_t st);
hipError_t bgv_launch_committee_totals(bgv_dcommittee* dir, const uint32_t* handles, uint32_t nh, const uint32_t* pool,
                                       const bgv_cache_entry* cache, hipStream_t st);
size_t bgv_g1_point_bytes();
hipError_t bgv_launch_debug_out(const bgv_dev_batch& b, uint8_t* out_h192, uint8_t* out_f576, hipStream_t st);
hipError_t bgv_launch_hash(const uint8_t* msgs, const uint32_t* offs, const uint32_t* lens, uint32_t n,
                           uint8_t* out192, hipStream_t st);
hipError_t bgv_launch_keygen(const uint8_t* sks, uint32_t n, bgv_cache_entry* cache, uint8_t* out48, hipStream_t st);
hipError_t bgv_launch_sign(const uint8_t* sks, const uint8_t* msgs, uint32_t n, uint8_t* out96, hipStream_t st);
hipError_t bgv_launch_pk_validate(const uint8_t* keys48, uint32_t n, int32_t* status, uint8_t* out96,
                                  hipStream_t st);
hipError_t bgv_launch_sig_aggregate(const uint8_t* sigs96, const uint32_t* lens, uint32_t n, const uint32_t* first,
                                    const uint32_t* count, uint32_t naggs, void* pts, int32_t* status,
                                    uint8_t* out96, hipStream_t st);
size_t bgv_g2_point_bytes();
size_t bgv_fp12_bytes();
hipError_t bgv_launch_fp12_bytes(const fp12_t* in, uint32_t n, uint8_t* out576, hipStream_t st);
hipError_t bgv_launch_partial(const bgv_dev_batch& b, uint32_t g0, uint32_t ng, void* scratch, uint8_t* out576,
                              hipStream_t st);
hipError_t bgv_launch_final_verify(const uint8_t* in, uint32_t n, void* vals, void* one, const bgv_dgroup* group,
                                   int32_t* status, int32_t* verdict, hipStream_t st);
```

Baseline: 2.712 million.

## Use mapped pinned host memory for batch inputs and status outputs, dropping memcpys

Pinned host buffers are now allocated as mapped and coherent, and the prep kernels read slot, group, index and pubkey data straight from host memory. They also publish copies into device buffers so later kernels can use them. Status and verdict results are written directly to host-mapped arrays, which removes the explicit H2D and D2H memcpys and one stream sync. The gu copy is replaced by a kernel-side write into a kept buffer when a call might need it. The risk is slower reads over PCIe/Infinity Fabric from kernels and coherence costs on small scattered writes.

```diff
diff --git a/lodestar_amd/csrc/bgv_api.cpp b/lodestar_amd/csrc/bgv_api.cpp
--- a/lodestar_amd/csrc/bgv_api.cpp
+++ b/lodestar_amd/csrc/bgv_api.cpp
@@ -75,14 +75,21 @@
 template <class T>
 struct Pinned {
   T* p = nullptr;
+  T* d = nullptr;
   size_t cap = 0;
   hipError_t reserve(size_t n) {
     if (n <= cap) return hipSuccess;
     release();
     n = std::max(n, 2 * cap);
-    hipError_t e = hipHostMalloc(reinterpret_cast<void**>(&p), std::max<size_t>(n, 1) * sizeof(T), 0);
+    hipError_t e = hipHostMalloc(reinterpret_cast<void**>(&p), std::max<size_t>(n, 1) * sizeof(T),
+                                 hipHostMallocMapped | hipHostMallocCoherent);
+    if (e == hipSuccess) {
+      e = hipHostGetDevicePointer(reinterpret_cast<void**>(&d), p, 0);
+      if (e != hipSuccess) (void)hipHostFree(p);
+    }
     if (e != hipSuccess) {
       p = nullptr;
+      d = nullptr;
       return e;
     }
     cap = n;
@@ -91,6 +98,7 @@
   void release() {
     if (p) (void)hipHostFree(p);
     p = nullptr;
+    d = nullptr;
     cap = 0;
   }
 };
@@ -580,6 +588,13 @@
 
 static double ms_since(std::chrono::steady_clock::time_point t) {
   return std::chrono::duration<double, std::milli>(std::chrono::steady_clock::now() - t).count();
+}
+
+static bool call_may_need_gu(const Call& call) {
+  if (call.partial_out || call.todo.size() < 2) return false;
+  for (char shared : call.L.group_shared)
+    if (shared) return true;
+  return false;
 }
 
 static bool needs_retry(const std::vector<Call*>& calls) {
@@ -681,11 +696,20 @@
   }
   t_merge = ms_since(tb);
   if (c->fault_inject) HIPCHK(hipErrorLaunchFailure);
-  HIPCHK(hipMemcpyAsync(x.d_slots, slots, sizeof(bgv_dslot) * nslots, hipMemcpyHostToDevice, x.main));
-  HIPCHK(hipMemcpyAsync(x.d_groups, groups, sizeof(bgv_dgroup) * ngroups, hipMemcpyHostToDevice, x.main));
-  if (nidx + nlist) HIPCHK(hipMemcpyAsync(x.d_idx, x.h_idx.p, 4 * (nidx + nlist), hipMemcpyHostToDevice, x.main));
-  if (npkb) HIPCHK(hipMemcpyAsync(x.d_pkb, x.h_pkb.p, npkb, hipMemcpyHostToDevice, x.main));
   bgv_dev_batch b = make_batch(d, x, nslots, ngroups);
+  b.slots_in = x.h_slots.d;
+  b.groups_in = x.h_groups.d;
+  b.idx_in = x.h_idx.d;
+  b.pkb_in = x.h_pkb.d;
+  b.sig_status_out = x.h_ss.d;
+  b.pk_status_out = x.h_ps.d;
+  b.verdict_out = x.h_verdict.d;
+  bool keep_gu = false;
+  for (const Call* call : calls) keep_gu = keep_gu || call_may_need_gu(*call);
+  if (keep_gu) {
+    if ((rc = grow(&x.d_gu1, &x.gu1_cap, ngroups))) return rc;
+    b.gu_keep = x.d_gu1;
+  }
   b.max_npk = max_npk;
   b.uniform = uniform;
   bs.uniform = uniform;
@@ -712,9 +736,6 @@
   const auto tg = std::chrono::steady_clock::now();
   HIPCHK(bgv_launch_groups(b, S, false));
   HIPCHK(hipEventRecord(x.ev1, x.main));
-  HIPCHK(hipMemcpyAsync(ss, b.sig_status, 4ull * nslots, hipMemcpyDeviceToHost, x.main));
-  HIPCHK(hipMemcpyAsync(ps, b.pk_status, 4ull * nslots, hipMemcpyDeviceToHost, x.main));
-  HIPCHK(hipMemcpyAsync(verdict, b.verdict, 4ull * ngroups, hipMemcpyDeviceToHost, x.main));
   HIPCHK(hipStreamSynchronize(x.main));
   float ms = 0;
   HIPCHK(hipEventElapsedTime(&ms, x.ev0, x.ev1));
@@ -734,10 +755,7 @@
       want_gu = want_gu || call->any_pattern_eligible();
     }
   }
-  if (want_gu) {
-    if ((rc = grow(&x.d_gu1, &x.gu1_cap, ngroups))) return rc;
-    HIPCHK(hipMemcpyAsync(x.d_gu1, b.gu, sizeof(fp12_t) * ngroups, hipMemcpyDeviceToDevice, x.main));
-  }
+  if (want_gu && !keep_gu) return -BGV_E_DEVICE;
   {
     uint32_t gb = 0, np = 0, maxg = 0;
     for (Call* call : calls) {
@@ -762,7 +780,6 @@
       }
     }
   }
-  HIPCHK(hipStreamSynchronize(x.main));
   t_post = ms_since(tp);
   bs.t_merge = t_merge;
   bs.t_tok = t_tok;
@@ -825,12 +842,12 @@
   bool pattern = false;
   for (Call* call : calls) pattern = pattern || !call->punits.empty();
   if (pattern) b.gu1 = x.d_gu1;
+  b.verdict_out = x.h_verdict.d;
   r.t_build = ms_since(th);
   bgv_streams SC{x.close, bs.prof ? x.kev : nullptr};
   HIPCHK(hipEventRecord(x.ev0, x.close));
   HIPCHK(bgv_launch_groups(b, SC, true));
   HIPCHK(hipEventRecord(x.ev1, x.close));
-  HIPCHK(hipMemcpyAsync(x.h_verdict.p, b.verdict, 4ull * nrg, hipMemcpyDeviceToHost, x.close));
   r.nrg = nrg;
   return BGV_OK;
 }
diff --git a/lodestar_amd/csrc/bgv_device.h b/lodestar_amd/csrc/bgv_device.h
--- a/lodestar_amd/csrc/bgv_device.h
+++ b/lodestar_amd/csrc/bgv_device.h
@@ -51,6 +51,95 @@
 
 #include "bgv_launch.h"
 
+struct bgv_prep_io {
+  const bgv_dslot* slots;
+  const uint32_t* pk_idx;
+  const uint8_t* pk_bytes;
+  const uint32_t* uniq;
+  const uint32_t* com;
+  const bgv_dgroup* groups;
+  bgv_dslot* slots_pub;
+  bgv_dgroup* groups_pub;
+  uint32_t* uniq_pub;
+  uint32_t ngroups, nuniq;
+  int32_t* sig_status_out;
+  int32_t* pk_status_out;
+};
+static inline bgv_prep_io bgv_prep_io_of(const bgv_dev_batch& b) {
+  bgv_prep_io io;
+  const bool m = b.slots_in != nullptr;
+  io.slots = m ? b.slots_in : b.slots;
+  io.pk_idx = m ? b.idx_in : b.pk_idx;
+  io.pk_bytes = m ? b.pkb_in : b.pk_bytes;
+  io.uniq = m && b.uniq ? b.idx_in + (b.uniq - b.pk_idx) : b.uniq;
+  io.com = m && b.com ? b.idx_in + (b.com - b.pk_idx) : b.com;
+  io.groups = m ? b.groups_in : b.groups;
+  io.slots_pub = m ? const_cast<bgv_dslot*>(b.slots) : nullptr;
+  io.groups_pub = m ? const_cast<bgv_dgroup*>(b.groups) : nullptr;
+  io.uniq_pub = m ? const_cast<uint32_t*>(b.uniq) : nullptr;
+  io.ngroups = b.ngroups;
+  io.nuniq = b.uniq ? b.nuniq : 0;
+  io.sig_status_out = b.sig_status_out;
+  io.pk_status_out = b.pk_status_out;
+  return io;
+}
+
+template <int N>
+__device__ __forceinline__ void load_field16(uint8_t* dst, const uint8_t* src) {
+  static_assert(N % 16 == 0 && offsetof(bgv_dslot, msg) % 16 == 0 && offsetof(bgv_dslot, sig) % 16 == 0,
+                "16-byte fields");
+  const uint4* q = reinterpret_cast<const uint4*>(src);
+  BGV_UNROLL for (int i = 0; i < N / 16; ++i) {
+    const uint4 v = q[i];
+    __builtin_memcpy(dst + 16 * i, &v, 16);
+  }
+}
+
+#define BGV_PREP_IO_PARAMS                                                                                       \
+  const bgv_dslot *__restrict__ slots, const uint32_t *__restrict__ pk_idx, const uint8_t *__restrict__ pk_bytes, \
+      const uint32_t *__restrict__ uniq, const uint32_t *__restrict__ com, const bgv_dgroup *__restrict__ groups, \
+      bgv_dslot *__restrict__ slots_pub, bgv_dgroup *__restrict__ groups_pub, uint32_t *__restrict__ uniq_pub,    \
+      uint32_t ngroups, uint32_t nuniq, int32_t *__restrict__ sig_status_out, int32_t *__restrict__ pk_status_out
+#define BGV_PREP_IO_ARGS(io)                                                                                  \
+  (io).slots, (io).pk_idx, (io).pk_bytes, (io).uniq, (io).com, (io).groups, (io).slots_pub, (io).groups_pub, \
+      (io).uniq_pub, (io).ngroups, (io).nuniq, (io).sig_status_out, (io).pk_status_out
+#define BGV_PREP_IO_LOCAL                                                                                   \
+  bgv_prep_io {                                                                                             \
+    slots, pk_idx, pk_bytes, uniq, com, groups, slots_pub, groups_pub, uniq_pub, ngroups, nuniq,           \
+        sig_status_out, pk_status_out                                                                       \
+  }
+
+__device__ __forceinline__ void put_status(int32_t* __restrict__ dev, int32_t* __restrict__ out, uint32_t s,
+                                           int32_t v) {
+  dev[s] = v;
+  if (out) out[s] = v;
+}
+
+struct bgv_slot_pk {
+  uint32_t flags, n_pk, pk_off;
+  uint32_t scalar_lo, scalar_hi;
+  __device__ uint64_t scalar() const { return (uint64_t)scalar_lo | ((uint64_t)scalar_hi << 32); }
+};
+static_assert(sizeof(bgv_dslot) == 160 && offsetof(bgv_dslot, scalar) == 16, "slot record layout");
+
+__device__ __forceinline__ bgv_slot_pk slot_pk(const bgv_dslot& d) {
+  return bgv_slot_pk{d.flags, d.n_pk, d.pk_off, (uint32_t)d.scalar, (uint32_t)(d.scalar >> 32)};
+}
+
+__device__ __forceinline__ bgv_slot_pk slot_take(uint32_t s, const bgv_prep_io& io) {
+  const uint4* __restrict__ src = reinterpret_cast<const uint4*>(io.slots + s);
+  const uint4 w0 = src[0], w1 = src[1];
+  if (io.slots_pub) {
+    uint4* __restrict__ dst = reinterpret_cast<uint4*>(io.slots_pub + s);
+    dst[0] = w0;
+    dst[1] = w1;
+    BGV_UNROLL for (int i = 2; i < 10; ++i) dst[i] = src[i];
+    if (s < io.ngroups) io.groups_pub[s] = io.groups[s];
+    if (s < io.nuniq) io.uniq_pub[s] = io.uniq[s];
+  }
+  return bgv_slot_pk{w0.x, w0.y, w0.z, w1.x, w1.y};
+}
+
 static inline unsigned nblk(uint32_t n, unsigned t) { return (n + t - 1) / t; }
 
 #define BGV_PREP_WIDE_MAX 340
diff --git a/lodestar_amd/csrc/bgv_k_final.hip b/lodestar_amd/csrc/bgv_k_final.hip
--- a/lodestar_amd/csrc/bgv_k_final.hip
+++ b/lodestar_amd/csrc/bgv_k_final.hip
@@ -54,7 +54,8 @@
 #define BGV_FINAL12_ARGS                                                                                     \
   const bgv_dgroup *__restrict__ groups, uint32_t ngroups, const fp12_t *__restrict__ f,                     \
       const fp12_t *__restrict__ gpair, int32_t *__restrict__ verdict, fp12_t *__restrict__ gprod,          \
-      fp12_t *__restrict__ gu, const fp12_t *__restrict__ gu1, const fp12_t *__restrict__ gpkp
+      fp12_t *__restrict__ gu, const fp12_t *__restrict__ gu1, const fp12_t *__restrict__ gpkp,              \
+      int32_t *__restrict__ verdict_out, fp12_t *__restrict__ gu_keep
 }
 __device__ __forceinline__ void final12_body(BGV_FINAL12_ARGS) {
   __shared__ fp_t lds[BGV_FINAL12_TEAMS + 1][2 * BGV_TEAM_COMPS];
@@ -92,13 +93,15 @@
   if (gprod && live) reinterpret_cast<fp_t*>(gprod + gi)[fi] = x;
   const fp_t u = tm_final_exp_u(o, x);
   if (gu && live) reinterpret_cast<fp_t*>(gu + gi)[fi] = u;
+  if (gu_keep && live) reinterpret_cast<fp_t*>(gu_keep + gi)[fi] = u;
   const int32_t v = verdict_bits(o, u, g, gu1, fi);
-  if (live && c == 0) verdict[gi] = v;
+  if (live && c == 0) put_status(verdict, verdict_out, gi, v);
 }
 
 extern "C" __global__ void __launch_bounds__(64) k_final_wident(const bgv_dgroup* __restrict__ groups, uint32_t ngroups,
                                                      const fp12_t* __restrict__ gu, const fp12_t* __restrict__ gu1,
-                                                     int32_t* __restrict__ verdict) {
+                                                     int32_t* __restrict__ verdict,
+                                                     int32_t* __restrict__ verdict_out) {
   __shared__ fp_t lds[BGV_FINAL12_TEAMS + 1][2 * BGV_TEAM_COMPS];
   __shared__ uint32_t lens[BGV_FINAL12_TEAMS + 1];
   const int team = threadIdx.x / BGV_TEAM_COMPS, c = threadIdx.x % BGV_TEAM_COMPS;
@@ -123,11 +126,11 @@
     if (wt && hit && found == 0 && w <= g.n_slots) found = (int32_t)w;
     P = o.mul(P, ur);
   }
-  if (wt && c == 0) verdict[gi] = (verdict[gi] & 1) | (found << 8);
+  if (wt && c == 0) put_status(verdict, verdict_out, gi, (verdict[gi] & 1) | (found << 8));
 }
 extern "C" {
 __global__ void __launch_bounds__(64) __attribute__((amdgpu_waves_per_eu(2, 2))) k_final12(BGV_FINAL12_ARGS) {
-  final12_body(groups, ngroups, f, gpair, verdict, gprod, gu, gu1, gpkp);
+  final12_body(groups, ngroups, f, gpair, verdict, gprod, gu, gu1, gpkp, verdict_out, gu_keep);
 }
 
 }
@@ -149,7 +152,8 @@
                                                 const fp12_t* __restrict__ f, const fp12_t* __restrict__ gpair,
                                                 int32_t* __restrict__ verdict, fp12_t* __restrict__ gprod,
                                                 fp12_t* __restrict__ gu, const fp12_t* __restrict__ gu1,
-                                                const fp12_t* __restrict__ fsig, const fp12_t* __restrict__ gpkp) {
+                                                const fp12_t* __restrict__ fsig, const fp12_t* __restrict__ gpkp,
+                                                int32_t* __restrict__ verdict_out, fp12_t* __restrict__ gu_keep) {
   constexpr int kTeams = (ENGINE == 2 ? BGV_FOLD_RNS_THREADS : BGV_FOLD_THREADS) / BGV_TEAM;
   __shared__ fp_t lds[kTeams][2 * BGV_TEAM_COMPS];
   __shared__ fp_t part[BGV_FOLD_TEAMS][BGV_TEAM_COMPS];
@@ -194,13 +198,14 @@
     if (gu && gi < ngroups) {
       const fp_t uf = ro.to_fp(u);
       if (ro.i == 0) reinterpret_cast<fp_t*>(gu + gi)[rfi] = uf;
+      if (ro.i == 0 && gu_keep) reinterpret_cast<fp_t*>(gu_keep + gi)[rfi] = uf;
     }
     int32_t v = ro.is_fp6(u) ? 1 : 0;
     if (gu1 && g.ref1) {
       const uint32_t ur = ro.from_fp(reinterpret_cast<const fp_t*>(gu1 + (g.ref1 - 1))[rfi]);
       if (ro.is_fp6(ro.mul(ur, ro.conj(u)))) v |= 2;
     }
-    if (gi < ngroups && threadIdx.x == 0) verdict[gi] = v;
+    if (gi < ngroups && threadIdx.x == 0) put_status(verdict, verdict_out, gi, v);
   } else {
     const int wc = threadIdx.x % BGV_TEAM_COMPS, wq = threadIdx.x / BGV_TEAM_COMPS;
     using OW = decltype(bgv_fold_ops_pick<ENGINE == 1>());
@@ -215,8 +220,9 @@
     const int wfi = tm_fp_index(wc);
     const fp_t u = tm_final_exp_u(ow, xw);
     if (gu && gi < ngroups && wq == 0) reinterpret_cast<fp_t*>(gu + gi)[wfi] = u;
+    if (gu_keep && gi < ngroups && wq == 0) reinterpret_cast<fp_t*>(gu_keep + gi)[wfi] = u;
     const int32_t v = verdict_bits(ow, u, g, gu1, wfi);
-    if (gi < ngroups && threadIdx.x == 0) verdict[gi] = v;
+    if (gi < ngroups && threadIdx.x == 0) put_status(verdict, verdict_out, gi, v);
   }
 }
 extern "C" {
@@ -224,15 +230,15 @@
   const bgv_dgroup *__restrict__ groups, uint32_t ngroups, const fp12_t *__restrict__ f,                     \
       const fp12_t *__restrict__ gpair, int32_t *__restrict__ verdict, fp12_t *__restrict__ gprod,          \
       fp12_t *__restrict__ gu, const fp12_t *__restrict__ gu1, const fp12_t *__restrict__ fsig,                \
-      const fp12_t *__restrict__ gpkp
+      const fp12_t *__restrict__ gpkp, int32_t *__restrict__ verdict_out, fp12_t *__restrict__ gu_keep
 __global__ void __launch_bounds__(BGV_FOLD_RNS_THREADS) k_final_fold(BGV_FOLD_ARGS) {
-  final_fold_body<2>(groups, ngroups, f, gpair, verdict, gprod, gu, gu1, fsig, gpkp);
+  final_fold_body<2>(groups, ngroups, f, gpair, verdict, gprod, gu, gu1, fsig, gpkp, verdict_out, gu_keep);
 }
 __global__ void __launch_bounds__(BGV_FOLD_THREADS) k_final_fold_p8(BGV_FOLD_ARGS) {
-  final_fold_body<1>(groups, ngroups, f, gpair, verdict, gprod, gu, gu1, fsig, gpkp);
+  final_fold_body<1>(groups, ngroups, f, gpair, verdict, gprod, gu, gu1, fsig, gpkp, verdict_out, gu_keep);
 }
 __global__ void __launch_bounds__(BGV_FOLD_THREADS) k_final_fold_sel(BGV_FOLD_ARGS) {
-  final_fold_body<0>(groups, ngroups, f, gpair, verdict, gprod, gu, gu1, fsig, gpkp);
+  final_fold_body<0>(groups, ngroups, f, gpair, verdict, gprod, gu, gu1, fsig, gpkp, verdict_out, gu_keep);
 }
 
 __global__ void BGV_KATTR k_fp12_prod(const fp12_t* __restrict__ in, uint32_t n, uint32_t chunk,
@@ -326,14 +332,14 @@
                        b.ngroups, b.f, b.gpair,
                        b.verdict, b.gprod, b.gu, b.gu1,
                        !pairs && bgv_sig_pairs(b) ? static_cast<const fp12_t*>(b.fsig) : nullptr,
-                       b.uniform ? static_cast<const fp12_t*>(b.gpkp) : nullptr);
+                       b.uniform ? static_cast<const fp12_t*>(b.gpkp) : nullptr, b.verdict_out, b.gu_keep);
   else
     hipLaunchKernelGGL(k_final12, dim3(nblk(b.ngroups, BGV_FINAL12_TEAMS)), dim3(64), 0, s.main, b.groups,
                        b.ngroups, b.f, b.gpair, b.verdict, b.gprod, b.gu, b.gu1,
-                       b.uniform ? static_cast<const fp12_t*>(b.gpkp) : nullptr);
+                       b.uniform ? static_cast<const fp12_t*>(b.gpkp) : nullptr, b.verdict_out, b.gu_keep);
   if (b.weighted)
     hipLaunchKernelGGL(k_final_wident, dim3(nblk(b.ngroups, BGV_FINAL12_TEAMS)), dim3(64), 0, s.main, b.groups,
-                       b.ngroups, static_cast<const fp12_t*>(b.gu), b.gu1, b.verdict);
+                       b.ngroups, static_cast<const fp12_t*>(b.gu), b.gu1, b.verdict, b.verdict_out);
   BGV_MARK(5);
   return hipGetLastError();
 }
diff --git a/lodestar_amd/csrc/bgv_k_lat.h b/lodestar_amd/csrc/bgv_k_lat.h
--- a/lodestar_amd/csrc/bgv_k_lat.h
+++ b/lodestar_amd/csrc/bgv_k_lat.h
@@ -13,7 +13,7 @@
   const bgv_dslot& d = slots[s];
   if (d.flags & BGV_SLOT_PAD) return;
   uint8_t msg[32];
-  for (int i = 0; i < 32; ++i) msg[i] = d.msg[i];
+  load_field16<32>(msg, d.msg);
   fp2_t u0, u1;
   hash_to_field_fp2(&u0, &u1, msg, 32);
   const g2_jac q = sswu_g2_jac_t<PW>(which ? u1 : u0, fp_sqrt_minus5());
@@ -22,18 +22,20 @@
 
 template <class PW>
 __device__ __noinline__ void task_sig_decode_t(uint32_t s, const bgv_dslot* __restrict__ slots, g2_aff* out,
-                                               int32_t* __restrict__ sig_status, bool writer) {
+                                               int32_t* __restrict__ sig_status,
+                                               int32_t* __restrict__ sig_status_out, bool writer) {
   const bgv_dslot& d = slots[s];
   int32_t st = BGV_ST_OK;
   g2_aff a;
   bool fin = false;
-  if (d.flags & BGV_SLOT_PAD) {
+  const uint4 w0 = *reinterpret_cast<const uint4*>(&d);
+  if (w0.x & BGV_SLOT_PAD) {
     st = BGV_ST_INFINITY;
-  } else if (d.sig_len != 96) {
+  } else if (w0.w != 96) {
     st = BGV_INVALID_SIZE;
   } else {
     uint8_t b[96];
-    for (int i = 0; i < 96; ++i) b[i] = d.sig[i];
+    load_field16<96>(b, d.sig);
     bool inf;
     st = g2_decompress_t<PW>(&a, &inf, b);
     if (st == BGV_OK) {
@@ -45,6 +47,6 @@
   }
   if (writer) {
     if (fin) *out = a;
-    sig_status[s] = st;
+    put_status(sig_status, sig_status_out, s, st);
   }
 }
diff --git a/lodestar_amd/csrc/bgv_k_prep.hip b/lodestar_amd/csrc/bgv_k_prep.hip
--- a/lodestar_amd/csrc/bgv_k_prep.hip
+++ b/lodestar_amd/csrc/bgv_k_prep.hip
@@ -227,30 +227,32 @@
   if (blockIdx.x < nslots) pk_aggw_body(slots, blockIdx.x, pk_idx, cache, pk_agg);
 }
 
-__global__ void BGV_KATTR_PREP k_prep_a(const bgv_dslot* __restrict__ slots, uint32_t nslots, g2_jac* __restrict__ h,
+__global__ void BGV_KATTR_PREP k_prep_a(BGV_PREP_IO_PARAMS, uint32_t nslots, g2_jac* __restrict__ h,
                                         fp12_t* __restrict__ f, int32_t* __restrict__ sig_status,
-                                        const uint32_t* __restrict__ pk_idx, const g1_aff* __restrict__ cache,
-                                        const uint8_t* __restrict__ pk_bytes, g1_jac* __restrict__ rpk,
+                                        const g1_aff* __restrict__ cache, g1_jac* __restrict__ rpk,
                                         int32_t* __restrict__ pk_status, g1_jac* __restrict__ pk_agg) {
+  const bgv_prep_io io = BGV_PREP_IO_LOCAL;
   const uint32_t s = blockIdx.x * blockDim.x + threadIdx.x;
   if (s >= nslots) return;
   if (blockIdx.y == 0)
-    task_map_t<bgv_pow_lane>(s, 0, slots, h + s, true);
+    task_map_t<bgv_pow_lane>(s, 0, io.slots, h + s, true);
   else if (blockIdx.y == 1)
-    task_map_t<bgv_pow_lane>(s, 1, slots, split_q1(f, s), true);
+    task_map_t<bgv_pow_lane>(s, 1, io.slots, split_q1(f, s), true);
   else if (blockIdx.y == 2)
-    task_sig_decode_t<bgv_pow_lane>(s, slots, split_sig(f, s), sig_status, true);
+    task_sig_decode_t<bgv_pow_lane>(s, io.slots, split_sig(f, s), sig_status, io.sig_status_out, true);
   else
-    task_pk(s, slots, pk_idx, cache, pk_bytes, rpk, pk_status, pk_agg);
+    task_pk(s, slot_take(s, io), io.pk_idx, cache, io.pk_bytes, rpk, pk_status, io.pk_status_out, pk_agg);
 }
 
 __global__ void __launch_bounds__(64) k_prep_team(const bgv_dslot* __restrict__ slots, uint32_t nslots,
                                                   g2_jac* __restrict__ h, fp12_t* __restrict__ f,
-                                                  g2_jac* __restrict__ rsig, int32_t* __restrict__ sig_status) {
+                                                  g2_jac* __restrict__ rsig, int32_t* __restrict__ sig_status,
+                                                  int32_t* __restrict__ sig_status_out) {
   if (blockIdx.y == 2) {
     const uint32_t s = blockIdx.x * blockDim.x + threadIdx.x;
     if (s >= nslots || (slots[s].flags & BGV_SLOT_PAD) || sig_status[s] != BGV_ST_OK) return;
-    if (!g2_in_subgroup(jac_from_aff(*split_sig(f, s)))) sig_status[s] = BGV_POINT_NOT_IN_GROUP;
+    if (!g2_in_subgroup(jac_from_aff(*split_sig(f, s))))
+      put_status(sig_status, sig_status_out, s, BGV_POINT_NOT_IN_GROUP);
     return;
   }
   __shared__ uint8_t prog[TCP_TABLE_BYTES];
@@ -336,7 +338,9 @@
                                                   g1_jac* __restrict__ rpk, int32_t* __restrict__ pk_status,
                                                   g1_jac* __restrict__ pk_agg,
                                                   const bgv_dcommittee* __restrict__ com_dir,
-                                                  const uint32_t* __restrict__ com_pool) {
+                                                  const uint32_t* __restrict__ com_pool,
+                                                  int32_t* __restrict__ sig_status_out,
+                                                  int32_t* __restrict__ pk_status_out) {
   static_assert(TG1_TABLE_BYTES <= TCP_TABLE_BYTES && TG1_NSLOT <= TCP_NSLOT, "plane 3 reuses the G2 buffers");
   __shared__ uint8_t prog[TCP_TABLE_BYTES];
   __shared__ fp_t S[TCP_NSLOT];
@@ -348,7 +352,7 @@
     if (pk_agg) pk_bits_one(slots, s, pk_idx, com_dir, com_pool, cache, pk_agg);
     if (threadIdx.x == 0) {
       g1_jac acc;
-      const bool go = task_pk_sum(s, slots, pk_idx, cache, pk_bytes, pk_status, pk_agg, &acc);
+      const bool go = task_pk_sum(s, slots, pk_idx, cache, pk_bytes, pk_status, pk_status_out, pk_agg, &acc);
       flag = go ? 1 : 0;
       if (go) {
         S[TG1_BANK(1)] = acc.x;
@@ -365,7 +369,7 @@
     tg1_wide_engine e{{prog, S, RP, tr_wide_lane_c(lane), tr_wide_lane_q(lane), false}};
     tg1_mul_glv(e, slots[s].scalar);
     if (lane < 3) reinterpret_cast<fp_t*>(rpk + s)[lane] = S[TG1_BANK(4) + lane];
-    if (lane == 0) pk_status[s] = BGV_ST_OK;
+    if (lane == 0) put_status(pk_status, pk_status_out, s, BGV_ST_OK);
     return;
   }
   const uint32_t uu = blockIdx.x;
@@ -434,7 +438,7 @@
         const g2_jac xp = {{B[0], B[1]}, {B[2], B[3]}, {B[4], B[5]}};
         in = jac_eq(g2_psi(p), jac_neg(xp));
       }
-      if (!in) sig_status[uu] = BGV_POINT_NOT_IN_GROUP;
+      if (!in) put_status(sig_status, sig_status_out, uu, BGV_POINT_NOT_IN_GROUP);
     }
   }
 }
@@ -450,7 +454,7 @@
                              uint8_t* __restrict__ out96) {
   if (blockIdx.x != 0 || threadIdx.x != 0) return;
   int32_t st = BGV_OK;
-  const g1_jac acc = pk_sum(slot[0], idx, cache, nullptr, pk_agg, 0, &st);
+  const g1_jac acc = pk_sum(slot[0].flags, slot[0].n_pk, slot[0].pk_off, idx, cache, nullptr, pk_agg, 0, &st);
   g1_aff a;
   const bool fin = jac_to_aff(&a, acc);
   uint8_t b[96];
@@ -468,31 +472,30 @@
   const uint32_t ncom = b.ncom_team + b.ncom_wave;
   const bool agg = tree || ncom > 0;
   const bool wide = bgv_use_latency(b, n + b.ngroups) && n <= BGV_PREP_WIDE_MAX;
+  const g1_aff* cache = reinterpret_cast<const g1_aff*>(b.cache_opaque);
+  const bgv_prep_io io = bgv_prep_io_of(b);
   if (wide) {
-    const g1_aff* cache = reinterpret_cast<const g1_aff*>(b.cache_opaque);
     const hipError_t e = bgv_launch_prep_wave(b, s.main);
     if (e != hipSuccess) return e;
     hipLaunchKernelGGL(k_prep_wide, dim3(n, 4), dim3(64), 0, s.main, b.slots, n, b.h, b.f, b.rsig, b.sig_status,
-                       b.pk_idx, cache, b.pk_bytes, b.rpk, b.pk_status, agg ? b.pk_agg : nullptr, b.com_dir, b.com_pool);
+                       io.pk_idx, cache, io.pk_bytes, b.rpk, b.pk_status, agg ? b.pk_agg : nullptr, b.com_dir,
+                       b.com_pool, b.sig_status_out, b.pk_status_out);
     BGV_MARK(1);
     return hipGetLastError();
   }
   if (ncom)
-    hipLaunchKernelGGL(k_pk_agg_bits, dim3(nblk(b.ncom_team, 4) + b.ncom_wave), dim3(64), 0, s.main, b.slots, b.com,
-                       b.ncom_team, b.ncom_wave, b.pk_idx, b.com_dir, b.com_pool,
-                       reinterpret_cast<const g1_aff*>(b.cache_opaque), b.pk_agg);
+    hipLaunchKernelGGL(k_pk_agg_bits, dim3(nblk(b.ncom_team, 4) + b.ncom_wave), dim3(64), 0, s.main, io.slots, io.com,
+                       b.ncom_team, b.ncom_wave, io.pk_idx, b.com_dir, b.com_pool, cache, b.pk_agg);
   if (tree)
-    hipLaunchKernelGGL(k_pk_agg16, dim3(nblk(n, 4)), dim3(64), 0, s.main, b.slots, n, b.pk_idx,
-                       reinterpret_cast<const g1_aff*>(b.cache_opaque), b.pk_agg);
+    hipLaunchKernelGGL(k_pk_agg16, dim3(nblk(n, 4)), dim3(64), 0, s.main, io.slots, n, io.pk_idx, cache, b.pk_agg);
   if (b.max_npk > BGV_PK_TEAM_MAX)
-    hipLaunchKernelGGL(k_pk_agg, dim3(n), dim3(64), 0, s.main, b.slots, n, b.pk_idx,
-                       reinterpret_cast<const g1_aff*>(b.cache_opaque), b.pk_agg);
+    hipLaunchKernelGGL(k_pk_agg, dim3(n), dim3(64), 0, s.main, io.slots, n, io.pk_idx, cache, b.pk_agg);
   if (bgv_use_latency(b, n + b.ngroups)) {
-    hipLaunchKernelGGL(k_prep_a, dim3(nblk(n, 64), 4), dim3(64), 0, s.main, b.slots, n, b.h, b.f, b.sig_status,
-                       b.pk_idx, reinterpret_cast<const g1_aff*>(b.cache_opaque), b.pk_bytes, b.rpk, b.pk_status,
-                       agg ? b.pk_agg : nullptr);
+    hipLaunchKernelGGL(k_prep_a, dim3(nblk(n, 64), 4), dim3(64), 0, s.main, BGV_PREP_IO_ARGS(io), n, b.h, b.f,
+                       b.sig_status, cache,
+                       b.rpk, b.pk_status, agg ? b.pk_agg : nullptr);
     hipLaunchKernelGGL(k_prep_team, dim3(nblk(n, BGV_FINAL_TEAMS), 3), dim3(64), 0, s.main, b.slots, n, b.h, b.f,
-                       b.rsig, b.sig_status);
+                       b.rsig, b.sig_status, b.sig_status_out);
   } else {
     const hipError_t e = bgv_launch_prep_bulk(b, s, agg);
     if (e != hipSuccess) return e;
diff --git a/lodestar_amd/csrc/bgv_k_prep_bulk.hip b/lodestar_amd/csrc/bgv_k_prep_bulk.hip
--- a/lodestar_amd/csrc/bgv_k_prep_bulk.hip
+++ b/lodestar_amd/csrc/bgv_k_prep_bulk.hip
@@ -11,27 +11,27 @@
 
 extern "C" {
 
-__global__ void BGV_KATTR_BULK k_prep(const bgv_dslot* __restrict__ slots, uint32_t nslots, g2_jac* __restrict__ rsig,
+__global__ void BGV_KATTR_BULK k_prep(BGV_PREP_IO_PARAMS, uint32_t nslots, g2_jac* __restrict__ rsig,
                                       int32_t* __restrict__ sig_status, g2_jac* __restrict__ h,
-                                      const uint32_t* __restrict__ pk_idx, const g1_aff* __restrict__ cache,
-                                      const uint8_t* __restrict__ pk_bytes, g1_jac* __restrict__ rpk,
+                                      const g1_aff* __restrict__ cache, g1_jac* __restrict__ rpk,
                                       int32_t* __restrict__ pk_status, const g1_jac* __restrict__ pk_agg,
-                                      const uint32_t* __restrict__ uniq, uint32_t nuniq, uint32_t task0) {
+                                      uint32_t task0) {
+  const bgv_prep_io io = BGV_PREP_IO_LOCAL;
   const uint32_t s = blockIdx.x * blockDim.x + threadIdx.x;
   const uint32_t task = blockIdx.y + task0;
   if (task == 0) {
-    if (uniq) {
-      if (s < nuniq) task_hash(uniq[s], slots, h);
+    if (io.uniq) {
+      if (s < io.nuniq) task_hash(io.uniq[s], io.slots, h);
     } else if (s < nslots) {
-      task_hash(s, slots, h);
+      task_hash(s, io.slots, h);
     }
     return;
   }
   if (s >= nslots) return;
   if (task == 1)
-    task_sig(s, slots, rsig, sig_status);
+    task_sig(s, io.slots, rsig, sig_status, io.sig_status_out);
   else
-    task_pk(s, slots, pk_idx, cache, pk_bytes, rpk, pk_status, pk_agg);
+    task_pk(s, slot_take(s, io), io.pk_idx, cache, io.pk_bytes, rpk, pk_status, io.pk_status_out, pk_agg);
 }
 
 }
@@ -41,10 +41,12 @@
     const char* e = getenv("BGV_PREP_SPLIT");
     return e && atoi(e) > 0;
   }();
+  const bgv_prep_io io = bgv_prep_io_of(b);
   for (uint32_t t0 = 0; t0 < 3; t0 += split ? 1 : 3) {
-    hipLaunchKernelGGL(k_prep, dim3(nblk(b.nslots, 64), split ? 1 : 3), dim3(64), 0, s.main, b.slots, b.nslots, b.rsig,
-                       b.sig_status, b.h, b.pk_idx, reinterpret_cast<const g1_aff*>(b.cache_opaque), b.pk_bytes, b.rpk,
-                       b.pk_status, tree ? b.pk_agg : nullptr, b.uniq, b.nuniq, t0);
+    hipLaunchKernelGGL(k_prep, dim3(nblk(b.nslots, 64), split ? 1 : 3), dim3(64), 0, s.main, BGV_PREP_IO_ARGS(io),
+                       b.nslots, b.rsig,
+                       b.sig_status, b.h, reinterpret_cast<const g1_aff*>(b.cache_opaque), b.rpk, b.pk_status,
+                       tree ? b.pk_agg : nullptr, t0);
   }
   return hipGetLastError();
 }
diff --git a/lodestar_amd/csrc/bgv_k_prep_wave.hip b/lodestar_amd/csrc/bgv_k_prep_wave.hip
--- a/lodestar_amd/csrc/bgv_k_prep_wave.hip
+++ b/lodestar_amd/csrc/bgv_k_prep_wave.hip
@@ -4,21 +4,34 @@
 #include "bgv_k_lat.h"
 #include "bgv_wfp.h"
 
-extern "C" __global__ void __launch_bounds__(64) k_prep_a_wave(const bgv_dslot* __restrict__ slots, uint32_t nslots,
+extern "C" __global__ void __launch_bounds__(64) k_prep_a_wave(BGV_PREP_IO_PARAMS, uint32_t nslots,
                                                                g2_jac* __restrict__ h, fp12_t* __restrict__ f,
                                                                int32_t* __restrict__ sig_status) {
+  const bgv_prep_io io = BGV_PREP_IO_LOCAL;
   const uint32_t s = blockIdx.x;
   const bool w = threadIdx.x == 0;
-  if (blockIdx.y == 0)
-    task_map_t<bgv_pow_wave>(s, 0, slots, h + s, w);
-  else if (blockIdx.y == 1)
-    task_map_t<bgv_pow_wave>(s, 1, slots, split_q1(f, s), w);
-  else
-    task_sig_decode_t<bgv_pow_wave>(s, slots, split_sig(f, s), sig_status, w);
+  if (blockIdx.y == 0) {
+    task_map_t<bgv_pow_wave>(s, 0, io.slots, h + s, w);
+  } else if (blockIdx.y == 1) {
+    task_map_t<bgv_pow_wave>(s, 1, io.slots, split_q1(f, s), w);
+  } else {
+    if (io.slots_pub) {
+      const uint32_t l = threadIdx.x;
+      if (l < 10)
+        reinterpret_cast<uint4*>(io.slots_pub + s)[l] = reinterpret_cast<const uint4*>(io.slots + s)[l];
+      else if (l == 10 && s < io.ngroups)
+        io.groups_pub[s] = io.groups[s];
+      else if (l == 11 && s < io.nuniq)
+        io.uniq_pub[s] = io.uniq[s];
+    }
+    task_sig_decode_t<bgv_pow_wave>(s, io.slots, split_sig(f, s), sig_status, io.sig_status_out, w);
+  }
 }
 
 hipError_t bgv_launch_prep_wave(const bgv_dev_batch& b, hipStream_t st) {
   if (b.nslots == 0) return hipSuccess;
-  hipLaunchKernelGGL(k_prep_a_wave, dim3(b.nslots, 3), dim3(64), 0, st, b.slots, b.nslots, b.h, b.f, b.sig_status);
+  hipLaunchKernelGGL(k_prep_a_wave, dim3(b.nslots, 3), dim3(64), 0, st, BGV_PREP_IO_ARGS(bgv_prep_io_of(b)), b.nslots,
+                     b.h, b.f,
+                     b.sig_status);
   return hipGetLastError();
 }
diff --git a/lodestar_amd/csrc/bgv_k_tasks.h b/lodestar_amd/csrc/bgv_k_tasks.h
--- a/lodestar_amd/csrc/bgv_k_tasks.h
+++ b/lodestar_amd/csrc/bgv_k_tasks.h
@@ -2,16 +2,17 @@
 #include "bgv_device.h"
 
 static __device__ __noinline__ void task_sig(uint32_t s, const bgv_dslot* __restrict__ slots, g2_jac* __restrict__ rsig,
-                                      int32_t* __restrict__ sig_status) {
+                                      int32_t* __restrict__ sig_status, int32_t* __restrict__ sig_status_out) {
   const bgv_dslot& d = slots[s];
   int32_t st = BGV_ST_OK;
-  if (d.flags & BGV_SLOT_PAD) {
+  const uint4 w0 = *reinterpret_cast<const uint4*>(&d);
+  if (w0.x & BGV_SLOT_PAD) {
     st = BGV_ST_INFINITY;
-  } else if (d.sig_len != 96) {
+  } else if (w0.w != 96) {
     st = BGV_INVALID_SIZE;
   } else {
     uint8_t b[96];
-    for (int i = 0; i < 96; ++i) b[i] = d.sig[i];
+    load_field16<96>(b, d.sig);
     g2_aff a;
     bool inf;
     st = g2_decompress(&a, &inf, b);
@@ -27,33 +28,34 @@
       }
     }
   }
-  sig_status[s] = st;
+  put_status(sig_status, sig_status_out, s, st);
 }
 
 static __device__ __noinline__ void task_hash(uint32_t s, const bgv_dslot* __restrict__ slots, g2_jac* __restrict__ h) {
   const bgv_dslot& d = slots[s];
   if (d.flags & BGV_SLOT_PAD) return;
   uint8_t msg[32];
-  for (int i = 0; i < 32; ++i) msg[i] = d.msg[i];
+  load_field16<32>(msg, d.msg);
   h[s] = hash_to_g2(msg, 32);
 }
 
-__device__ __noinline__ static g1_jac pk_sum(const bgv_dslot& d, const uint32_t* __restrict__ pk_idx,
-                                      const g1_aff* __restrict__ cache, const uint8_t* __restrict__ pk_bytes,
-                                      const g1_jac* __restrict__ pk_agg, uint32_t s, int32_t* st) {
-  if (d.flags & BGV_SLOT_PK_COMMITTEE) return pk_agg[s];
+__device__ __noinline__ static g1_jac pk_sum(uint32_t flags, uint32_t n_pk, uint32_t pk_off,
+                                      const uint32_t* __restrict__ pk_idx, const g1_aff* __restrict__ cache,
+                                      const uint8_t* __restrict__ pk_bytes, const g1_jac* __restrict__ pk_agg,
+                                      uint32_t s, int32_t* st) {
+  if (flags & BGV_SLOT_PK_COMMITTEE) return pk_agg[s];
   g1_jac acc = jac_infinity<fp_t>();
-  const bool cached = (d.flags & BGV_SLOT_PK_CACHED) != 0;
-  const bool tree = pk_agg != nullptr && cached && d.n_pk >= BGV_PK_TREE_MIN;
+  const bool cached = (flags & BGV_SLOT_PK_CACHED) != 0;
+  const bool tree = pk_agg != nullptr && cached && n_pk >= BGV_PK_TREE_MIN;
   if (tree) return pk_agg[s];
-  for (uint32_t k = 0; k < d.n_pk; ++k) {
+  for (uint32_t k = 0; k < n_pk; ++k) {
     g1_aff a;
     if (cached) {
-      a = cache[pk_idx[d.pk_off + k]];
+      a = cache[pk_idx[pk_off + k]];
     } else {
       uint8_t b[96];
-      const uint8_t* src = pk_bytes + 96ull * (d.pk_off + k);
-      for (int i = 0; i < 96; ++i) b[i] = src[i];
+      const uint8_t* src = pk_bytes + 96ull * (pk_off + k);
+      load_field16<96>(b, src);
       bool inf;
       const int rc = g1_deserialize(&a, &inf, b);
       if (rc != BGV_OK) {
@@ -70,39 +72,40 @@
 static __device__ __noinline__ bool task_pk_sum(uint32_t s, const bgv_dslot* __restrict__ slots,
                                                 const uint32_t* __restrict__ pk_idx, const g1_aff* __restrict__ cache,
                                                 const uint8_t* __restrict__ pk_bytes, int32_t* __restrict__ pk_status,
+                                                int32_t* __restrict__ pk_status_out,
                                                 const g1_jac* __restrict__ pk_agg, g1_jac* acc) {
-  const bgv_dslot& d = slots[s];
+  const bgv_slot_pk d = slot_pk(slots[s]);
   if (d.flags & BGV_SLOT_PAD) {
-    pk_status[s] = BGV_ST_INFINITY;
+    put_status(pk_status, pk_status_out, s, BGV_ST_INFINITY);
     return false;
   }
   int32_t st = BGV_ST_OK;
-  const g1_jac a = pk_sum(d, pk_idx, cache, pk_bytes, pk_agg, s, &st);
+  const g1_jac a = pk_sum(d.flags, d.n_pk, d.pk_off, pk_idx, cache, pk_bytes, pk_agg, s, &st);
   if (st != BGV_OK || jac_is_inf(a)) {
-    pk_status[s] = st != BGV_OK ? st : BGV_ST_INFINITY;
+    put_status(pk_status, pk_status_out, s, st != BGV_OK ? st : BGV_ST_INFINITY);
     return false;
   }
   *acc = a;
   return true;
 }
 
-static __device__ __noinline__ void task_pk(uint32_t s, const bgv_dslot* __restrict__ slots,
+static __device__ __noinline__ void task_pk(uint32_t s, bgv_slot_pk d,
                                      const uint32_t* __restrict__ pk_idx, const g1_aff* __restrict__ cache,
                                      const uint8_t* __restrict__ pk_bytes, g1_jac* __restrict__ rpk,
-                                     int32_t* __restrict__ pk_status, const g1_jac* __restrict__ pk_agg) {
-  const bgv_dslot& d = slots[s];
+                                     int32_t* __restrict__ pk_status, int32_t* __restrict__ pk_status_out,
+                                     const g1_jac* __restrict__ pk_agg) {
   int32_t st = BGV_ST_OK;
   if (d.flags & BGV_SLOT_PAD) {
-    pk_status[s] = BGV_ST_INFINITY;
+    put_status(pk_status, pk_status_out, s, BGV_ST_INFINITY);
     return;
   }
-  const g1_jac acc = pk_sum(d, pk_idx, cache, pk_bytes, pk_agg, s, &st);
+  const g1_jac acc = pk_sum(d.flags, d.n_pk, d.pk_off, pk_idx, cache, pk_bytes, pk_agg, s, &st);
   if (st == BGV_OK) {
-    const g1_jac rp = jac_mul_glv(acc, d.scalar);
+    const g1_jac rp = jac_mul_glv(acc, d.scalar());
     if (jac_is_inf(rp))
       st = BGV_ST_INFINITY;
     else
       rpk[s] = rp;
   }
-  pk_status[s] = st;
+  put_status(pk_status, pk_status_out, s, st);
 }
diff --git a/lodestar_amd/csrc/bgv_launch.h b/lodestar_amd/csrc/bgv_launch.h
--- a/lodestar_amd/csrc/bgv_launch.h
+++ b/lodestar_amd/csrc/bgv_launch.h
@@ -37,6 +37,14 @@
   uint32_t ncom_team, ncom_wave;
   const bgv_dcommittee* com_dir;
   const uint32_t* com_pool;
+  const bgv_dslot* slots_in;
+  const bgv_dgroup* groups_in;
+  const uint32_t* idx_in;
+  const uint8_t* pkb_in;
+  int32_t* sig_status_out;
+  int32_t* pk_status_out;
+  int32_t* verdict_out;
+  fp12_t* gu_keep;
   jac_t<fp2_t>* rsig;
   jac_t<fp2_t>* h;
   jac_t<fp_t>* rpk;
```

Result: no change. 2.714 million, median of 5 (+0.1%).
